# jayleicn/TVRetrieval

Hardware: AMD Instinct MI355X
Metric: queries/sec VCMR over 21.8K-video corpus (higher is better)
Workload: dtype bf16

## Files before the change

### tvretrieval_amd/csrc/convse.hip

```cpp
#include "band.h"
#include "gemm.h"

static constexpr int TM = dispatch::CONVSE_TM;
static constexpr int LP = 128 + 8;
static constexpr int LH = 4;

using dispatch::CONVSE_SUB_MAX;
using dispatch::convse_sub;

struct ConvseWs {
  int32_t* counts;
  int32_t* offsets;
  int32_t* pos;
  int32_t* chunk_off;
  int32_t* bucket;
  int32_t* chunk_vid;
};

static size_t convse_ws_layout(const xml_convse_desc* d, ConvseWs* w, char* base) {
  size_t off = 0;
  auto take = [&](size_t bytes) {
    char* p = base ? base + off : nullptr;
    off += align_up(bytes, 256);
    return p;
  };
  const size_t nv = (size_t)d->nv, P = (size_t)d->nq * d->kpairs;
  char* counts = take(nv * CONVSE_SUB_MAX * 4);
  char* offsets = take((nv * CONVSE_SUB_MAX + 1) * 4);
  char* chunk_off = take((nv + 1) * 4);
  char* bucket = take(P * 4);
  char* pos = take(P * 4);
  char* chunk_vid = take(((size_t)dispatch::convse_max_chunks((int64_t)P, (int)nv, TM) + 1) * 4);
  if (w) {
    w->chunk_vid = (int32_t*)chunk_vid;
    w->counts = (int32_t*)counts; w->pos = (int32_t*)pos; w->offsets = (int32_t*)offsets;
    w->chunk_off = (int32_t*)chunk_off; w->bucket = (int32_t*)bucket;
  }
  return off;
}

extern "C" size_t xml_convse_rerank_workspace_bytes(const xml_convse_desc* d) {
  if (!d) return 0;
  return convse_ws_layout(d, nullptr, nullptr);
}

__global__ void convse_count_kernel(const int32_t* __restrict__ pair_vid, int32_t* __restrict__ counts,
                                    int32_t* __restrict__ pos, int64_t P, int nv, int sub) {
  const int64_t p = (int64_t)blockIdx.x * blockDim.x + threadIdx.x;
  if (p >= P) return;
  const int v = pair_vid[p];
  pos[p] = (v >= 0 && v < nv) ? atomicAdd(&counts[(int64_t)v * sub + (int)(p & (sub - 1))], 1) : -1;
}

__global__ void convse_zero_skipped_kernel(const int32_t* __restrict__ pair_vid, float* __restrict__ st_out,
                                           float* __restrict__ ed_out, int64_t P, int nv, int lpad4) {
  const int64_t p = (int64_t)blockIdx.x * blockDim.x + threadIdx.x;
  if (p >= P) return;
  const int v = pair_vid[p];
  if (v >= 0 && v < nv) return;
  const float4 z = make_float4(0.f, 0.f, 0.f, 0.f);
  float4* s4 = reinterpret_cast<float4*>(st_out) + p * lpad4;
  float4* e4 = reinterpret_cast<float4*>(ed_out) + p * lpad4;
  for (int i = 0; i < lpad4; ++i) { s4[i] = z; e4[i] = z; }
}

__global__ __launch_bounds__(1024) void convse_scan_kernel(const int32_t* __restrict__ counts,
                                                           int32_t* __restrict__ offsets,
                                                           int32_t* __restrict__ chunk_off,
                                                           int32_t* __restrict__ chunk_vid, int nv, int TM, int sub) {
  __shared__ int32_t wa[16], wb[16];
  const int tid = threadIdx.x, lane = tid & 63, wave = tid >> 6;
  const int per = (nv + 1023) / 1024;
  const int r0 = min(nv, tid * per), r1 = min(nv, r0 + per);
  int sa = 0, sb = 0;
  for (int i = r0; i < r1; ++i) {
    int c = 0;
    for (int j = 0; j < sub; ++j) c += counts[(int64_t)i * sub + j];
    sa += c; sb += (c + TM - 1) / TM;
  }
  int ia = sa, ib = sb;
#pragma unroll
  for (int o = 1; o < 64; o <<= 1) {
    const int va = __shfl_up(ia, o, 64), vb = __shfl_up(ib, o, 64);
    if (lane >= o) { ia += va; ib += vb; }
  }
  if (lane == 63) { wa[wave] = ia; wb[wave] = ib; }
  __syncthreads();
  int a = ia - sa, b = ib - sb;
  for (int w = 0; w < wave; ++w) { a += wa[w]; b += wb[w]; }
  for (int i = r0; i < r1; ++i) {
    int c = 0;
    for (int j = 0; j < sub; ++j) {
      const int cj = counts[(int64_t)i * sub + j];
      offsets[(int64_t)i * sub + j] = a + c;
      c += cj;
    }
    const int ch = (c + TM - 1) / TM;
    chunk_off[i] = b;
    for (int j = 0; j < ch; ++j) chunk_vid[b + j] = i;
    a += c; b += ch;
  }
  if (tid == 1023) { offsets[(int64_t)nv * sub] = a; chunk_off[nv] = b; }
}

__global__ void convse_fill_kernel(const int32_t* __restrict__ pair_vid, const int32_t* __restrict__ offsets,
                                   const int32_t* __restrict__ pos, int32_t* __restrict__ bucket, int64_t P, int sub) {
  const int64_t p = (int64_t)blockIdx.x * blockDim.x + threadIdx.x;
  if (p >= P) return;
  const int r = pos[p];
  if (r >= 0) bucket[offsets[(int64_t)pair_vid[p] * sub + (int)(p & (sub - 1))] + r] = (int32_t)p;
}

using dispatch::CONVSE_SMALL_NV;
__global__ __launch_bounds__(1024) void convse_invert_small_kernel(const int32_t* __restrict__ pair_vid,
                                                                   int32_t* __restrict__ offsets, int32_t* __restrict__ chunk_off,
                                                                   int32_t* __restrict__ chunk_vid, int32_t* __restrict__ pos,
                                                                   int32_t* __restrict__ bucket, float* __restrict__ st_out,
                                                                   float* __restrict__ ed_out, int P, int nv, int TM, int lpad4,
                                                                   int zero_skipped) {
  __shared__ int32_t s_cnt[CONVSE_SMALL_NV], s_off[CONVSE_SMALL_NV];
  __shared__ int32_t wa[16], wb[16];
  const int tid = threadIdx.x, lane = tid & 63, wave = tid >> 6;
  for (int i = tid; i < nv; i += 1024) s_cnt[i] = 0;
  const bool in_regs = P <= 8 * 1024;
  int v_r[8], pos_r[8];
#pragma unroll
  for (int j = 0; j < 8; ++j) {
    const int p = tid + j * 1024;
    v_r[j] = (in_regs && p < P) ? pair_vid[p] : -1;
  }
  __syncthreads();
  if (in_regs) {
#pragma unroll
    for (int j = 0; j < 8; ++j) {
      const int p = tid + j * 1024;
      const bool ok = v_r[j] >= 0 && v_r[j] < nv;
      pos_r[j] = ok ? atomicAdd(&s_cnt[v_r[j]], 1) : -1;
      if (p < P && !ok && zero_skipped) {
        const float4 z = make_float4(0.f, 0.f, 0.f, 0.f);
        float4* s4 = reinterpret_cast<float4*>(st_out) + (int64_t)p * lpad4;
        float4* e4 = reinterpret_cast<float4*>(ed_out) + (int64_t)p * lpad4;
        for (int i = 0; i < lpad4; ++i) { s4[i] = z; e4[i] = z; }
      }
    }
  } else {
  for (int p = tid; p < P; p += 1024) {
    const int v = pair_vid[p];
    const bool ok = v >= 0 && v < nv;
    pos[p] = ok ? atomicAdd(&s_cnt[v], 1) : -1;
    if (!ok && zero_skipped) {
      const float4 z = make_float4(0.f, 0.f, 0.f, 0.f);
      float4* s4 = reinterpret_cast<float4*>(st_out) + (int64_t)p * lpad4;
      float4* e4 = reinterpret_cast<float4*>(ed_out) + (int64_t)p * lpad4;
      for (int i = 0; i < lpad4; ++i) { s4[i] = z; e4[i] = z; }
    }
  }
  }
  __syncthreads();
  const int per = (nv + 1023) / 1024;
  const int r0 = min(nv, tid * per), r1 = min(nv, r0 + per);
  int sa = 0, sb = 0;
  for (int i = r0; i < r1; ++i) { const int c = s_cnt[i]; sa += c; sb += (c + TM - 1) / TM; }
  int ia = sa, ib = sb;
#pragma unroll
  for (int o = 1; o < 64; o <<= 1) {
    const int va = __shfl_up(ia, o, 64), vb = __shfl_up(ib, o, 64);
    if (lane >= o) { ia += va; ib += vb; }
  }
  if (lane == 63) { wa[wave] = ia; wb[wave] = ib; }
  __syncthreads();
  int a = ia - sa, b = ib - sb;
  for (int w = 0; w < wave; ++w) { a += wa[w]; b += wb[w]; }
  for (int i = r0; i < r1; ++i) {
    const int c = s_cnt[i], ch = (c + TM - 1) / TM;
    offsets[i] = a; s_off[i] = a;
    chunk_off[i] = b;
    for (int j = 0; j < ch; ++j) chunk_vid[b + j] = i;
    a += c; b += ch;
  }
  if (tid == 1023) { offsets[nv] = a; chunk_off[nv] = b; }
  __syncthreads();
  if (in_regs) {
#pragma unroll
    for (int j = 0; j < 8; ++j)
      if (pos_r[j] >= 0) bucket[s_off[v_r[j]] + pos_r[j]] = tid + j * 1024;
    return;
  }
  for (int p = tid; p < P; p += 1024) {
    const int r = pos[p];
    if (r >= 0) bucket[s_off[pair_vid[p]] + r] = p;
  }
}

struct ConvseArgs {
  const void* q_lin[2];
  const void* feat2[2];
  const float* mask[2];
  const float* conv_w;
  float* st_out;
  float* ed_out;
  const int32_t* offsets;
  const int32_t* chunk_off;
  const int32_t* bucket;
  const int32_t* chunk_vid;
  int nv, kpairs, lpad, l_ref, hidden, n_mod, merged, ksize, softmax;
  int sub;
  int dbg;
  int dma;
  const float* q_inv[2];
  const float* c_inv[2];
  const float* pair_w;
  float* summ;
  int min_l, max_l;
  const int32_t* vid_len;
  const int32_t* pair_q;
  float* ev_sim[2];
  float* ev_merged;
};

template <typename T, bool EV = false>
__global__ __launch_bounds__(256, IsSplit16<T>::value ? 2 : 3) void convse_kernel(ConvseArgs a) {
  using Cfg = GemmCfg<T, TM, 128, 1, 4>;
  extern __shared__ __attribute__((aligned(16))) char smem[];
  __shared__ int32_t s_pair[TM];
  const int n_sim_l = a.merged ? 1 : a.n_mod;
  float (*sim)[TM][LP] = reinterpret_cast<float (*)[TM][LP]>(n_sim_l == 1 ? smem : smem + Cfg::LDS_BYTES);
  const int tid = threadIdx.x;
  const int chunk = blockIdx.x;
  if (chunk >= a.chunk_off[a.nv]) return;
  const int v = a.chunk_vid[chunk];
  const int first = a.offsets[(int64_t)v * a.sub] + (chunk - a.chunk_off[v]) * TM;
  const int cnt = min(TM, a.offsets[(int64_t)(v + 1) * a.sub] - first);
  const int vlen = a.vid_len ? max(0, min(a.vid_len[v], a.l_ref)) : a.l_ref;
  const int b_rows = a.vid_len ? max(1, min(a.lpad, vlen + (a.ksize >> 1))) : a.lpad;
  constexpr bool SPLIT = IsSplit16<T>::value;
  __shared__ float s_qinv[SPLIT ? 2 : 1][SPLIT ? TM : 1];
  auto q_of = [&](int p) -> int {
    if constexpr (EV) return a.pair_q[p];
    else return p / a.kpairs;
  };
  if (tid < TM) {
    const int p = tid < cnt ? a.bucket[first + tid] : -1;
    s_pair[tid] = p;
    if constexpr (SPLIT) {
#pragma unroll
      for (int m = 0; m < 2; ++m) s_qinv[m][tid] = (p >= 0 && m < a.n_mod) ? a.q_inv[m][q_of(p)] : 1.f;
    }
  }
  __syncthreads();

  const int lane = tid & 63, wn = tid >> 6;
  const int fr = lane & 15, fg = lane >> 4;
  const int n_sim = a.merged ? 1 : a.n_mod;
  const int mt_used = (cnt + 15) >> 4;
  f32x4 acc[Cfg::MT][Cfg::NT];
  auto ev_store = [&](float* dst, int mt, int nt, int r, float x) {
    const int row = mt * 16 + fg * 4 + r, col = wn * 32 + nt * 16 + fr;
    if (row < cnt && col < a.lpad) dst[(int64_t)s_pair[row] * a.lpad + col] = col < a.l_ref ? x : 0.f;
  };
  for (int pass = (EV && a.merged) ? -1 : 0; pass < a.n_mod; ++pass) {
    const bool pre = EV && pass < 0;
    const int m = pre ? 1 : pass;
    float cinv[Cfg::NT];
#pragma unroll
    for (int nt = 0; nt < Cfg::NT; ++nt) {
      cinv[nt] = 1.f;
      if constexpr (SPLIT) cinv[nt] = a.c_inv[m][(int64_t)v * a.lpad + min(wn * 32 + nt * 16 + fr, a.lpad - 1)];
    }
    const T* ql = reinterpret_cast<const T*>(a.q_lin[m]);
    const T* f2 = reinterpret_cast<const T*>(a.feat2[m]);
    auto a_row = [&](int r) -> const char* {
      const int p = s_pair[r];
      return p >= 0 ? reinterpret_cast<const char*>(ql + (int64_t)q_of(p) * a.hidden) : nullptr;
    };
    auto b_row = [&](int r) -> const char* {
      return r < b_rows ? reinterpret_cast<const char*>(f2 + ((int64_t)v * a.lpad + r) * a.hidden) : nullptr;
    };
    const int k_bytes = a.hidden * (int)sizeof(T);
    auto a_off = [&](int r) -> uint32_t {
      const int p = s_pair[r] >= 0 ? s_pair[r] : s_pair[0];
      return (uint32_t)q_of(p) * (uint32_t)k_bytes;
    };
    auto b_off = [&](int r) -> uint32_t { return (uint32_t)min(r, b_rows - 1) * (uint32_t)k_bytes; };
    const char* b_base = reinterpret_cast<const char*>(f2 + (int64_t)v * a.lpad * a.hidden);
    if (a.dbg == 1) {
#pragma unroll
      for (int mt = 0; mt < Cfg::MT; ++mt)
#pragma unroll
        for (int nt = 0; nt < Cfg::NT; ++nt) acc[mt][nt] = f32x4{0.f, 0.f, 0.f, 0.f};
    } else if (a.dma) {
      if (m > 0) __syncthreads();
      if (a.merged && m > 0 && !pre)
        gemm_mainloop_dma<T, Cfg, false, 2>(acc, reinterpret_cast<const char*>(ql), a_off, b_base, b_off, k_bytes, smem, mt_used);
      else
        gemm_mainloop_dma<T, Cfg, true, 2>(acc, reinterpret_cast<const char*>(ql), a_off, b_base, b_off, k_bytes, smem, mt_used);
    } else if (a.merged && m > 0 && !pre)
      gemm_mainloop<T, Cfg, false>(acc, a_row, b_row, a.hidden * (int)sizeof(T), smem, mt_used);
    else
      gemm_mainloop<T, Cfg, true>(acc, a_row, b_row, a.hidden * (int)sizeof(T), smem, mt_used);
    if constexpr (EV) {
      if (a.merged && (pre || m == 0)) {
#pragma unroll
        for (int mt = 0; mt < Cfg::MT; ++mt)
#pragma unroll
          for (int nt = 0; nt < Cfg::NT; ++nt)
#pragma unroll
            for (int r = 0; r < 4; ++r) {
              float x = acc[mt][nt][r];
              if constexpr (SPLIT) x *= s_qinv[m][mt * 16 + fg * 4 + r] * cinv[nt];
              ev_store(a.ev_sim[m], mt, nt, r, x);
            }
      }
      if (pre) {
        __syncthreads();
        continue;
      }
    }
    if constexpr (SPLIT) {
      if (a.merged && m + 1 < a.n_mod) {
        float cnext[Cfg::NT];
#pragma unroll
        for (int nt = 0; nt < Cfg::NT; ++nt)
          cnext[nt] = cinv[nt] / a.c_inv[m + 1][(int64_t)v * a.lpad + min(wn * 32 + nt * 16 + fr, a.lpad - 1)];
#pragma unroll
        for (int mt = 0; mt < Cfg::MT; ++mt)
#pragma unroll
          for (int r = 0; r < 4; ++r) {
            const int row = mt * 16 + fg * 4 + r;
            const float qr = s_qinv[m][row] / s_qinv[m + 1][row];
#pragma unroll
            for (int nt = 0; nt < Cfg::NT; ++nt) acc[mt][nt][r] *= qr * cnext[nt];
          }
      }
    }
    if (!a.merged || m == a.n_mod - 1) {
      const float scale = (a.merged && a.n_mod == 2) ? 0.5f : 1.f;
      const int si = a.merged ? 0 : m;
      if (n_sim_l == 1) __syncthreads();
#pragma unroll
      for (int mt = 0; mt < Cfg::MT; ++mt)
#pragma unroll
        for (int nt = 0; nt < Cfg::NT; ++nt)
#pragma unroll
          for (int r = 0; r < 4; ++r) {
            float x = acc[mt][nt][r] * scale;
            if constexpr (SPLIT) x *= s_qinv[m][mt * 16 + fg * 4 + r] * cinv[nt];
            sim[si][mt * 16 + fg * 4 + r][LH + wn * 32 + nt * 16 + fr] = x;
            if constexpr (EV) {
              if (a.merged) {
                ev_store(a.ev_merged, mt, nt, r, x);
              } else {
                ev_store(a.ev_sim[m], mt, nt, r, x);
                if (m == a.n_mod - 1)
                  ev_store(a.ev_merged, mt, nt, r,
                           m ? (sim[0][mt * 16 + fg * 4 + r][LH + wn * 32 + nt * 16 + fr] + x) * 0.5f : x);
              }
            }
          }
    }
  }
  __syncthreads();

  if (a.dbg == 2) return;
  const int half = a.ksize >> 1;
  const float inv_mod = 1.f / (float)n_sim;
  __shared__ float s_taps[2 * 2 * 16];
  if (tid < 2 * n_sim * a.ksize) {
    const int which = tid / (n_sim * a.ksize), rest = tid - which * n_sim * a.ksize;
    const int si = rest / a.ksize, t = rest - si * a.ksize;
    s_taps[(which * 2 + si) * 16 + t] = a.conv_w[(which * n_sim + si) * a.ksize + t];
  }
  float mk_r[2][2];
#pragma unroll
  for (int si = 0; si < 2; ++si)
#pragma unroll
    for (int h = 0; h < 2; ++h) {
      const int l = lane + h * 64;
      mk_r[si][h] = (si < n_sim && l < a.l_ref) ? a.mask[a.merged ? 0 : si][(int64_t)v * a.lpad + l] : 0.f;
    }
  __syncthreads();
  if (XML_CONVSE_FAST_EPILOGUE(a.ksize, a.summ)) {
    const int hsel = lane >> 5, l4 = (lane & 31) * 4;
    float tw[2][2][5];
#pragma unroll
    for (int w2 = 0; w2 < 2; ++w2)
#pragma unroll
      for (int si = 0; si < 2; ++si)
#pragma unroll
        for (int t = 0; t < 5; ++t) tw[w2][si][t] = si < n_sim ? s_taps[(w2 * 2 + si) * 16 + t] : 0.f;
    float mk4[2][4];
#pragma unroll
    for (int si = 0; si < 2; ++si)
#pragma unroll
      for (int c = 0; c < 4; ++c)
        mk4[si][c] = (si < n_sim && l4 + c < a.l_ref) ? a.mask[a.merged ? 0 : si][(int64_t)v * a.lpad + l4 + c] : 0.f;
    const int store_end = a.vid_len ? ((vlen + 3) & ~3) : a.lpad;
    for (int row = wn * 2 + hsel; row < ((cnt + 7) & ~7); row += 8) {
      const bool live = row < cnt;
      const int rr = live ? row : 0;
      const int p = s_pair[rr];
      float sv[4] = {0.f, 0.f, 0.f, 0.f}, ev[4] = {0.f, 0.f, 0.f, 0.f};
#pragma unroll
      for (int si = 0; si < 2; ++si) {
        if (si < n_sim) {
          float x[8];
          const float2* px = reinterpret_cast<const float2*>(&sim[si][rr][LH + l4 - 2]);
#pragma unroll
          for (int i = 0; i < 4; ++i) { const float2 t2 = px[i]; x[2 * i] = t2.x; x[2 * i + 1] = t2.y; }
#pragma unroll
          for (int i = 0; i < 8; ++i) { const int j = l4 - 2 + i; x[i] = (j >= 0 && j < a.l_ref) ? x[i] : 0.f; }
#pragma unroll
          for (int c = 0; c < 4; ++c) {
            float cs = 0.f, ce = 0.f;
#pragma unroll
            for (int t = 0; t < 5; ++t) { cs += tw[0][si][t] * x[c + t]; ce += tw[1][si][t] * x[c + t]; }
            const float fill = (1.f - mk4[si][c]) * -1e10f;
            sv[c] += cs * mk4[si][c] + fill;
            ev[c] += ce * mk4[si][c] + fill;
          }
        }
      }
#pragma unroll
      for (int c = 0; c < 4; ++c) {
        if (n_sim > 1) { sv[c] *= inv_mod; ev[c] *= inv_mod; }
        if (l4 + c >= a.l_ref) { sv[c] = -INFINITY; ev[c] = -INFINITY; }
      }
      if (a.softmax) {
        float ms = fmaxf(fmaxf(sv[0], sv[1]), fmaxf(sv[2], sv[3])), me = fmaxf(fmaxf(ev[0], ev[1]), fmaxf(ev[2], ev[3]));
        ms = lane16_max_dpp(ms); me = lane16_max_dpp(me);
        ms = fmaxf(ms, __shfl_xor(ms, 16, 64)); me = fmaxf(me, __shfl_xor(me, 16, 64));
        float ss = 0.f, se = 0.f;
#pragma unroll
        for (int c = 0; c < 4; ++c) { sv[c] = expf(sv[c] - ms); ev[c] = expf(ev[c] - me); ss += sv[c]; se += ev[c]; }
        ss = lane16_sum_dpp(ss); se = lane16_sum_dpp(se);
        ss += __shfl_xor(ss, 16, 64); se += __shfl_xor(se, 16, 64);
#pragma unroll
        for (int c = 0; c < 4; ++c) { sv[c] /= ss; ev[c] /= se; }
      }
      if (live && l4 < store_end) {
#pragma unroll
        for (int c = 0; c < 4; ++c)
          if (l4 + c >= a.l_ref) { sv[c] = 0.f; ev[c] = 0.f; }
        *reinterpret_cast<float4*>(a.st_out + (int64_t)p * a.lpad + l4) = make_float4(sv[0], sv[1], sv[2], sv[3]);
        *reinterpret_cast<float4*>(a.ed_out + (int64_t)p * a.lpad + l4) = make_float4(ev[0], ev[1], ev[2], ev[3]);
      }
    }
    return;
  }
  for (int row = wn; row < cnt; row += 4) {
    const int p = s_pair[row];
    float st[2], ed[2];
#pragma unroll
    for (int h = 0; h < 2; ++h) {
      const int l = lane + h * 64;
      float s_acc = 0.f, e_acc = 0.f;
      if (l < a.l_ref) {
#pragma unroll
        for (int si = 0; si < 2; ++si) {
          if (si < n_sim) {
            const float* wst = s_taps + si * 16;
            const float* wed = s_taps + (2 + si) * 16;
            float cs = 0.f, ce = 0.f;
            for (int t = 0; t < a.ksize; ++t) {
              const int j = l + t - half;
              const float x = (j >= 0 && j < a.l_ref) ? sim[si][row][LH + j] : 0.f;
              cs += wst[t] * x;
              ce += wed[t] * x;
            }
            const float mk = mk_r[si][h];
            const float fill = (1.f - mk) * -1e10f;
            s_acc += cs * mk + fill;
            e_acc += ce * mk + fill;
          }
        }
        if (n_sim > 1) { s_acc *= inv_mod; e_acc *= inv_mod; }
      } else {
        s_acc = -INFINITY; e_acc = -INFINITY;
      }
      st[h] = s_acc; ed[h] = e_acc;
    }
    if (a.softmax) {
      const float ms = wave_max(fmaxf(st[0], st[1])), me = wave_max(fmaxf(ed[0], ed[1]));
      float es[2], ee[2];
#pragma unroll
      for (int h = 0; h < 2; ++h) { es[h] = expf(st[h] - ms); ee[h] = expf(ed[h] - me); }
      const float ss = wave_sum(es[0] + es[1]), se = wave_sum(ee[0] + ee[1]);
#pragma unroll
      for (int h = 0; h < 2; ++h) { st[h] = es[h] / ss; ed[h] = ee[h] / se; }
    }
#pragma unroll
    for (int h = 0; h < 2; ++h) {
      const int l = lane + h * 64;
      if (a.vid_len ? l < vlen : l < a.lpad) {
        const bool in = l < a.l_ref;
        a.st_out[(int64_t)p * a.lpad + l] = in ? st[h] : 0.f;
        a.ed_out[(int64_t)p * a.lpad + l] = in ? ed[h] : 0.f;
      }
    }
    if (a.summ) {
      const float wv = a.pair_w ? a.pair_w[p] : 1.f;
      const bool in0 = lane < a.l_ref, in1 = lane + 64 < a.l_ref;
      float e_lo = in0 ? ed[0] : 0.f, e_hi = in1 ? ed[1] : 0.f;
      band_window_max(e_lo, e_hi, a.max_l - a.min_l, a.min_l, lane);
      const float m_lo = fmaxf((in0 ? st[0] : 0.f) * wv * e_lo, 0.f), m_hi = fmaxf((in1 ? st[1] : 0.f) * wv * e_hi, 0.f);
      float mg = fmaxf(m_lo, m_hi);
      mg = fmaxf(mg, __int_as_float(__builtin_amdgcn_update_dpp(0, __float_as_int(mg), 0xB1, 0xf, 0xf, false)));
      mg = fmaxf(mg, __int_as_float(__builtin_amdgcn_update_dpp(0, __float_as_int(mg), 0x4E, 0xf, 0xf, false)));
      mg = fmaxf(mg, __int_as_float(__builtin_amdgcn_update_dpp(0, __float_as_int(mg), 0x141, 0xf, 0xf, false)));
      if ((lane & 7) == 0) a.summ[(int64_t)p * XML_MOMENT_SUMM + (lane >> 3)] = mg;
    }
  }
}

struct RescoreArgs {
  const void* qn[2];
  const void* cn[2];
  const float* mask[2];
  float* out;
  const int32_t* offsets;
  const int32_t* chunk_off;
  const int32_t* bucket;
  const int32_t* chunk_vid;
  int nv, kpairs, lpad, hidden, n_mod;
  int sub;
  int dma;
};

static constexpr int RS_STAGES = 2;
template <typename T, int TM = 64>
__global__ __launch_bounds__(256, TM == 64 ? 3 : 2) void rescore_kernel(RescoreArgs a) {
  using Cfg = GemmCfg<T, TM, 128, 1, 4>;
  extern __shared__ __attribute__((aligned(16))) char smem[];
  __shared__ int32_t s_pair[TM];
  __shared__ float s_max[4][TM];
  const int tid = threadIdx.x;
  const int chunk = blockIdx.x;
  if (chunk >= a.chunk_off[a.nv]) return;
  const int v = a.chunk_vid[chunk];
  const int first = a.offsets[(int64_t)v * a.sub] + (chunk - a.chunk_off[v]) * TM;
  const int cnt = min(TM, a.offsets[(int64_t)(v + 1) * a.sub] - first);
  if (tid < TM) s_pair[tid] = tid < cnt ? a.bucket[first + tid] : -1;
  __syncthreads();
  const int lane = tid & 63, wn = tid >> 6;
  const int fr = lane & 15, fg = lane >> 4;
  float tot = 0.f;
  f32x4 acc[Cfg::MT][Cfg::NT];
  for (int m = 0; m < a.n_mod; ++m) {
    const T* qn = reinterpret_cast<const T*>(a.qn[m]);
    const T* cn = reinterpret_cast<const T*>(a.cn[m]);
    auto a_row = [&](int r) -> const char* {
      const int p = s_pair[r];
      return p >= 0 ? reinterpret_cast<const char*>(qn + (int64_t)(p / a.kpairs) * a.hidden) : nullptr;
    };
    auto b_row = [&](int r) -> const char* {
      return r < a.lpad ? reinterpret_cast<const char*>(cn + ((int64_t)v * a.lpad + r) * a.hidden) : nullptr;
    };
    float mk[Cfg::NT];
#pragma unroll
    for (int nt = 0; nt < Cfg::NT; ++nt) {
      const int c = wn * 32 + nt * 16 + fr;
      mk[nt] = c < a.lpad ? a.mask[m][(int64_t)v * a.lpad + c] : 0.f;
    }
    if (a.dma) {
      const int k_bytes = a.hidden * (int)sizeof(T);
      auto a_off = [&](int r) -> uint32_t {
        const int p = s_pair[r] >= 0 ? s_pair[r] : s_pair[0];
        return (uint32_t)(p / a.kpairs) * (uint32_t)k_bytes;
      };
      auto b_off = [&](int r) -> uint32_t { return (uint32_t)min(r, a.lpad - 1) * (uint32_t)k_bytes; };
      gemm_mainloop_dma<T, Cfg, true, RS_STAGES>(acc, reinterpret_cast<const char*>(qn), a_off,
                                                 reinterpret_cast<const char*>(cn + (int64_t)v * a.lpad * a.hidden), b_off,
                                                 k_bytes, smem, (cnt + 15) >> 4);
    } else {
      gemm_mainloop<T, Cfg, true>(acc, a_row, b_row, a.hidden * (int)sizeof(T), smem, (cnt + 15) >> 4);
    }
#pragma unroll
    for (int mt = 0; mt < Cfg::MT; ++mt)
#pragma unroll
      for (int r = 0; r < 4; ++r) {
        float best = -INFINITY;
#pragma unroll
        for (int nt = 0; nt < Cfg::NT; ++nt) {
          float x = acc[mt][nt][r];
          if constexpr (IsSplit16<T>::value) x *= 1.f / (float)(1u << (2 * XML_F16_UNIT_LOG2));
          best = fmaxf(best, x * mk[nt] + (1.f - mk[nt]) * -1e10f);
        }
        best = lane16_max_dpp(best);
        if (fr == 0) s_max[wn][mt * 16 + fg * 4 + r] = best;
      }
    __syncthreads();
    if (tid < TM) tot += fmaxf(fmaxf(s_max[0][tid], s_max[1][tid]), fmaxf(s_max[2][tid], s_max[3][tid]));
  }
  if (tid < cnt) a.out[s_pair[tid]] = a.n_mod == 2 ? tot * 0.5f : tot;
}

__global__ void rescore_fill_skipped_kernel(const int32_t* __restrict__ pair_vid, float* __restrict__ out, int64_t P,
                                            int nv) {
  const int64_t p = (int64_t)blockIdx.x * blockDim.x + threadIdx.x;
  if (p >= P) return;
  const int v = pair_vid[p];
  if (v < 0 || v >= nv) out[p] = -INFINITY;
}

__global__ void convse_zero_words_kernel(uint32_t* __restrict__ p, int64_t n) {
  const int64_t i = (int64_t)blockIdx.x * 256 + threadIdx.x;
  if (i < n) p[i] = 0u;
}

struct ConvseSumm {
  const float* pair_w;
  float* summ;
  int min_l, max_l;
  const int32_t* vid_len;
};
struct ConvseEv {
  const int32_t* pair_q;
  int64_t n_pairs;
  float* sim[2];
  float* merged;
};
static int convse_rerank_impl(const xml_convse_desc* d, const void* q_lin0, const void* q_lin1, const void* feat2_0,
                              const void* feat2_1, const float* mask0, const float* mask1, const int32_t* pair_vid,
                              const float* conv_w, float* st_out, float* ed_out, void* ws, size_t ws_bytes,
                              const float* q_inv0, const float* q_inv1, const float* c_inv0, const float* c_inv1,
                              xml_stream_t stream, ConvseSumm sm = ConvseSumm{nullptr, nullptr, 0, 0, nullptr},
                              ConvseEv ev = ConvseEv{nullptr, 0, {nullptr, nullptr}, nullptr});

extern "C" int xml_convse_rerank_ex(const xml_convse_desc* d, const void* q_lin0, const void* q_lin1, const float* q_inv0,
                                    const float* q_inv1, const void* feat2_0, const void* feat2_1, const float* c_inv0,
                                    const float* c_inv1, const float* mask0, const float* mask1, const int32_t* pair_vid,
                                    const float* conv_w, const float* pair_w, int min_l, int max_l,
                                    const int32_t* vid_len, float* st_out, float* ed_out, float* summ_out, void* ws,
                                    size_t ws_bytes, xml_stream_t stream) {
  XML_ENTER();
  if (!d || !q_lin0 || !feat2_0 || !mask0 || !pair_vid || !conv_w || !st_out || !ed_out || !ws) return XML_ERR_BAD_ARG;
  if (!summ_out && !vid_len) return XML_ERR_BAD_ARG;
  if (d->nq <= 0 || d->nv <= 0 || d->kpairs <= 0 || d->hidden <= 0) return XML_ERR_BAD_ARG;
  if (d->n_mod < 1 || d->n_mod > 2 || (d->n_mod == 2 && (!q_lin1 || !feat2_1))) return XML_ERR_BAD_ARG;
  if (d->n_mod == 2 && !d->merged && !mask1) return XML_ERR_BAD_ARG;
  if (d->merged && d->n_mod != 2) return XML_ERR_BAD_ARG;
  if (!dispatch::convse_shape_ok(d->lpad, d->l_ref, d->hidden, d->ksize, XML_F32)) return XML_ERR_UNSUPPORTED;
  if (summ_out && (min_l < 0 || max_l <= min_l)) return XML_ERR_BAD_ARG;
  if (!(d->softmax & 1)) return XML_ERR_BAD_ARG;
  if (d->dt == XML_F16S) {
    if (!q_inv0 || !c_inv0 || (d->n_mod == 2 && (!q_inv1 || !c_inv1))) return XML_ERR_BAD_ARG;
    if (!dispatch::rescore_shape_ok(d->lpad, d->hidden, XML_F16S)) return XML_ERR_UNSUPPORTED;
  } else if (d->dt != XML_F32 && d->dt != XML_BF16) {
    return XML_ERR_BAD_ARG;
  }
  return convse_rerank_impl(d, q_lin0, q_lin1, feat2_0, feat2_1, mask0, mask1, pair_vid, conv_w, st_out, ed_out, ws, ws_bytes,
                            d->dt == XML_F16S ? q_inv0 : nullptr, d->dt == XML_F16S ? q_inv1 : nullptr,
                            d->dt == XML_F16S ? c_inv0 : nullptr, d->dt == XML_F16S ? c_inv1 : nullptr, stream,
                            ConvseSumm{pair_w, summ_out, min_l, max_l, vid_len});
}

extern "C" int xml_convse_rerank(const xml_convse_desc* d, const void* q_lin0, const void* q_lin1,
                                 const void* feat2_0, const void* feat2_1, const float* mask0, const float* mask1,
                                 const int32_t* pair_vid, const float* conv_w, float* st_out, float* ed_out, void* ws,
                                 size_t ws_bytes, xml_stream_t stream) {
  XML_ENTER();
  if (!d || !q_lin0 || !feat2_0 || !mask0 || !pair_vid || !conv_w || !st_out || !ed_out || !ws) return XML_ERR_BAD_ARG;
  if (d->nq <= 0 || d->nv <= 0 || d->kpairs <= 0 || d->hidden <= 0) return XML_ERR_BAD_ARG;
  if (d->n_mod < 1 || d->n_mod > 2 || (d->n_mod == 2 && (!q_lin1 || !feat2_1))) return XML_ERR_BAD_ARG;
  if (d->n_mod == 2 && !d->merged && !mask1) return XML_ERR_BAD_ARG;
  if (d->merged && d->n_mod != 2) return XML_ERR_BAD_ARG;
  if (!dispatch::convse_shape_ok(d->lpad, d->l_ref, d->hidden, d->ksize, XML_F32)) return XML_ERR_UNSUPPORTED;
  if (d->dt != XML_F32 && d->dt != XML_BF16) return XML_ERR_BAD_ARG;
  return convse_rerank_impl(d, q_lin0, q_lin1, feat2_0, feat2_1, mask0, mask1, pair_vid, conv_w, st_out, ed_out, ws, ws_bytes,
                            nullptr, nullptr, nullptr, nullptr, stream);
}

extern "C" int xml_convse_rerank_f16s(const xml_convse_desc* d, const void* q_lin0, const void* q_lin1, const float* q_inv0,
                                      const float* q_inv1, const void* feat2_0, const void* feat2_1, const float* c_inv0,
                                      const float* c_inv1, const float* mask0, const float* mask1, const int32_t* pair_vid,
                                      const float* conv_w, float* st_out, float* ed_out, void* ws, size_t ws_bytes,
                                      xml_stream_t stream) {
  XML_ENTER();
  if (!d || !q_lin0 || !feat2_0 || !mask0 || !pair_vid || !conv_w || !st_out || !ed_out || !ws || !q_inv0 || !c_inv0)
    return XML_ERR_BAD_ARG;
  if (d->nq <= 0 || d->nv <= 0 || d->kpairs <= 0 || d->hidden <= 0) return XML_ERR_BAD_ARG;
  if (d->n_mod < 1 || d->n_mod > 2 || (d->n_mod == 2 && (!q_lin1 || !feat2_1 || !q_inv1 || !c_inv1))) return XML_ERR_BAD_ARG;
  if (d->n_mod == 2 && !d->merged && !mask1) return XML_ERR_BAD_ARG;
  if (d->merged && d->n_mod != 2) return XML_ERR_BAD_ARG;
  if (!dispatch::convse_shape_ok(d->lpad, d->l_ref, d->hidden, d->ksize, XML_F16S)) return XML_ERR_UNSUPPORTED;
  if (d->dt != XML_F16S) return XML_ERR_BAD_ARG;
  return convse_rerank_impl(d, q_lin0, q_lin1, feat2_0, feat2_1, mask0, mask1, pair_vid, conv_w, st_out, ed_out, ws, ws_bytes,
                            q_inv0, q_inv1, c_inv0, c_inv1, stream);
}

static int convse_rerank_impl(const xml_convse_desc* d, const void* q_lin0, const void* q_lin1, const void* feat2_0,
                              const void* feat2_1, const float* mask0, const float* mask1, const int32_t* pair_vid,
                              const float* conv_w, float* st_out, float* ed_out, void* ws, size_t ws_bytes,
                              const float* q_inv0, const float* q_inv1, const float* c_inv0, const float* c_inv1,
                              xml_stream_t stream, ConvseSumm sm, ConvseEv ev) {
  xml_convse_desc dl = *d;
  if (ev.pair_q) { dl.nq = (int)ev.n_pairs; dl.kpairs = 1; }
  if (!ev.pair_q && ws_bytes < xml_convse_rerank_workspace_bytes(d)) return XML_ERR_WORKSPACE;
  hipStream_t st = (hipStream_t)stream;
  ConvseWs w;
  convse_ws_layout(&dl, &w, (char*)ws);
  const int64_t P = (int64_t)dl.nq * dl.kpairs;
  int sub = 1;
  if (dispatch::convse_small_inversion(P, d->nv)) {
    hipLaunchKernelGGL(convse_invert_small_kernel, dim3(1), dim3(1024), 0, st, pair_vid, w.offsets, w.chunk_off, w.chunk_vid,
                       w.pos, w.bucket, st_out, ed_out, (int)P, d->nv, TM, d->lpad / 4, (d->softmax & 2) ? 0 : 1);
    XML_CHECK_LAUNCH();
  } else {
    {
      const int64_t nwords = (int64_t)((char*)w.offsets - (char*)w.counts) / 4;
      hipLaunchKernelGGL(convse_zero_words_kernel, dim3(cdiv(nwords, 256)), dim3(256), 0, st, (uint32_t*)w.counts, nwords);
      XML_CHECK_LAUNCH();
    }
    sub = convse_sub(P, d->nv);
    hipLaunchKernelGGL(convse_count_kernel, dim3(cdiv(P, 256)), dim3(256), 0, st, pair_vid, w.counts, w.pos, P, d->nv, sub);
    XML_CHECK_LAUNCH();
    if (!(d->softmax & 2)) {
      hipLaunchKernelGGL(convse_zero_skipped_kernel, dim3(cdiv(P, 256)), dim3(256), 0, st, pair_vid, st_out, ed_out, P,
                         d->nv, d->lpad / 4);
      XML_CHECK_LAUNCH();
    }
    hipLaunchKernelGGL(convse_scan_kernel, dim3(1), dim3(1024), 0, st, w.counts, w.offsets, w.chunk_off, w.chunk_vid,
                       d->nv, TM, sub);
    XML_CHECK_LAUNCH();
    hipLaunchKernelGGL(convse_fill_kernel, dim3(cdiv(P, 256)), dim3(256), 0, st, pair_vid, w.offsets, w.pos, w.bucket, P, sub);
    XML_CHECK_LAUNCH();
  }
  ConvseArgs a;
  a.sub = sub;
  a.q_lin[0] = q_lin0; a.q_lin[1] = q_lin1;
  a.feat2[0] = feat2_0; a.feat2[1] = feat2_1;
  a.mask[0] = mask0; a.mask[1] = mask1 ? mask1 : mask0;
  a.conv_w = conv_w; a.st_out = st_out; a.ed_out = ed_out;
  a.offsets = w.offsets; a.chunk_off = w.chunk_off; a.bucket = w.bucket; a.chunk_vid = w.chunk_vid;
  a.pair_q = ev.pair_q; a.ev_sim[0] = ev.sim[0]; a.ev_sim[1] = ev.sim[1]; a.ev_merged = ev.merged;
  a.nv = d->nv; a.kpairs = dl.kpairs; a.lpad = d->lpad; a.l_ref = d->l_ref; a.hidden = d->hidden;
  a.n_mod = d->n_mod; a.merged = d->merged; a.ksize = d->ksize; a.softmax = d->softmax & 1;
  a.dbg = g_q2c_ablation;
  a.pair_w = sm.pair_w; a.summ = sm.summ; a.min_l = sm.min_l; a.max_l = sm.max_l; a.vid_len = sm.vid_len;
  a.q_inv[0] = q_inv0; a.q_inv[1] = q_inv1 ? q_inv1 : q_inv0;
  a.c_inv[0] = c_inv0; a.c_inv[1] = c_inv1 ? c_inv1 : c_inv0;
  {
    a.dma = dispatch::convse_dma(d->nq, d->lpad, d->hidden, d->dt) ? 1 : 0;
    if (g_q2c_ablation == 40) a.dma = 0;
  }
  const int64_t max_chunks = dispatch::convse_max_chunks(P, d->nv, TM);
  const int n_sim = d->merged ? 1 : d->n_mod;
  const size_t patch = (size_t)TM * LP * 4;
  if (d->dt == XML_F16S) {
    if (!a.dma) return XML_ERR_UNSUPPORTED;
    using Cfg = GemmCfg<f16s_t, TM, 128, 1, 4>;
    constexpr size_t stg = Cfg::LDS_BYTES;
    const size_t lds = n_sim == 1 ? (stg > patch ? stg : patch) : stg + 2 * patch;
    if (ev.pair_q) {
      if (!xml_lds_attr_once<convse_kernel<f16s_t, true>>((int)(stg + 2 * patch))) return XML_ERR_LAUNCH;
      hipLaunchKernelGGL((convse_kernel<f16s_t, true>), dim3((unsigned)max_chunks), dim3(256), lds, st, a);
    } else {
      if (!xml_lds_attr_once<convse_kernel<f16s_t>>((int)(stg + 2 * patch))) return XML_ERR_LAUNCH;
      hipLaunchKernelGGL(convse_kernel<f16s_t>, dim3((unsigned)max_chunks), dim3(256), lds, st, a);
    }
  } else if (d->dt == XML_F32) {
    using Cfg = GemmCfg<float, TM, 128, 1, 4>;
    constexpr size_t stg = Cfg::LDS_BYTES;
    const size_t lds = n_sim == 1 ? (stg > patch ? stg : patch) : stg + 2 * patch;
    if (ev.pair_q) {
      if (!xml_lds_attr_once<convse_kernel<float, true>>((int)(stg + 2 * patch))) return XML_ERR_LAUNCH;
      hipLaunchKernelGGL((convse_kernel<float, true>), dim3((unsigned)max_chunks), dim3(256), lds, st, a);
    } else {
      if (!xml_lds_attr_once<convse_kernel<float>>((int)(stg + 2 * patch))) return XML_ERR_LAUNCH;
      hipLaunchKernelGGL(convse_kernel<float>, dim3((unsigned)max_chunks), dim3(256), lds, st, a);
    }
  } else {
    using Cfg = GemmCfg<bf16_t, TM, 128, 1, 4>;
    constexpr size_t stg = Cfg::LDS_BYTES;
    const size_t lds = n_sim == 1 ? (stg > patch ? stg : patch) : stg + 2 * patch;
    if (ev.pair_q) {
      if (!xml_lds_attr_once<convse_kernel<bf16_t, true>>((int)(stg + 2 * patch))) return XML_ERR_LAUNCH;
      hipLaunchKernelGGL((convse_kernel<bf16_t, true>), dim3((unsigned)max_chunks), dim3(256), lds, st, a);
    } else {
      if (!xml_lds_attr_once<convse_kernel<bf16_t>>((int)(stg + 2 * patch))) return XML_ERR_LAUNCH;
      hipLaunchKernelGGL(convse_kernel<bf16_t>, dim3((unsigned)max_chunks), dim3(256), lds, st, a);
    }
  }
  XML_CHECK_LAUNCH();
  return XML_OK;
}

__global__ void evidence_pairs_kernel(const int32_t* __restrict__ pair_q, const int32_t* __restrict__ pair_vid,
                                      int32_t* __restrict__ vid_ok, int64_t P, int nq, int nv) {
  const int64_t p = (int64_t)blockIdx.x * blockDim.x + threadIdx.x;
  if (p >= P) return;
  const int q = pair_q[p], v = pair_vid[p];
  vid_ok[p] = (q >= 0 && q < nq && v >= 0 && v < nv) ? v : -1;
}

static size_t evidence_ws_layout(const xml_convse_desc* d, int64_t n_pairs, size_t* vid_off) {
  xml_convse_desc dl = *d;
  dl.nq = (int)n_pairs; dl.kpairs = 1;
  const size_t base = convse_ws_layout(&dl, nullptr, nullptr);
  if (vid_off) *vid_off = base;
  return base + align_up((size_t)n_pairs * 4, 256);
}

extern "C" size_t xml_span_evidence_workspace_bytes(const xml_convse_desc* d, int64_t n_pairs) {
  if (!d || n_pairs <= 0 || n_pairs > INT32_MAX) return 0;
  return evidence_ws_layout(d, n_pairs, nullptr);
}

extern "C" int xml_span_evidence(const xml_convse_desc* d, const void* q_lin0, const void* q_lin1, const float* q_inv0,
                                 const float* q_inv1, const void* feat2_0, const void* feat2_1, const float* c_inv0,
                                 const float* c_inv1, const float* mask0, const float* mask1, const int32_t* pair_q,
                                 const int32_t* pair_vid, int64_t n_pairs, const float* conv_w, float* sim0_out,
                                 float* sim1_out, float* sim_out, float* st_out, float* ed_out, void* ws, size_t ws_bytes,
                                 xml_stream_t stream) {
  XML_ENTER();
  if (!d || !q_lin0 || !feat2_0 || !mask0 || !pair_q || !pair_vid || !conv_w || !sim0_out || !sim_out || !st_out ||
      !ed_out || !ws)
    return XML_ERR_BAD_ARG;
  if (d->nq <= 0 || d->nv <= 0 || n_pairs <= 0 || n_pairs > INT32_MAX || d->hidden <= 0) return XML_ERR_BAD_ARG;
  if (d->n_mod < 1 || d->n_mod > 2 || (d->n_mod == 2 && (!q_lin1 || !feat2_1 || !sim1_out))) return XML_ERR_BAD_ARG;
  if (d->n_mod == 2 && !d->merged && !mask1) return XML_ERR_BAD_ARG;
  if (d->merged && d->n_mod != 2) return XML_ERR_BAD_ARG;
  if (!dispatch::convse_shape_ok(d->lpad, d->l_ref, d->hidden, d->ksize, XML_F32)) return XML_ERR_UNSUPPORTED;
  const bool split = d->dt == XML_F16S;
  if (split) {
    if (!q_inv0 || !c_inv0 || (d->n_mod == 2 && (!q_inv1 || !c_inv1))) return XML_ERR_BAD_ARG;
    if (!dispatch::rescore_shape_ok(d->lpad, d->hidden, XML_F16S)) return XML_ERR_UNSUPPORTED;
  } else if (d->dt != XML_F32 && d->dt != XML_BF16) {
    return XML_ERR_BAD_ARG;
  }
  size_t vid_off = 0;
  if (ws_bytes < evidence_ws_layout(d, n_pairs, &vid_off)) return XML_ERR_WORKSPACE;
  hipStream_t st = (hipStream_t)stream;
  int32_t* vid_ok = (int32_t*)((char*)ws + vid_off);
  hipLaunchKernelGGL(evidence_pairs_kernel, dim3(cdiv(n_pairs, 256)), dim3(256), 0, st, pair_q, pair_vid, vid_ok, n_pairs,
                     d->nq, d->nv);
  XML_CHECK_LAUNCH();
  hipLaunchKernelGGL(convse_zero_skipped_kernel, dim3(cdiv(n_pairs, 256)), dim3(256), 0, st, vid_ok, sim0_out, sim_out,
                     n_pairs, d->nv, d->lpad / 4);
  XML_CHECK_LAUNCH();
  if (d->n_mod == 2) {
    hipLaunchKernelGGL(convse_zero_skipped_kernel, dim3(cdiv(n_pairs, 256)), dim3(256), 0, st, vid_ok, sim1_out, sim1_out,
                       n_pairs, d->nv, d->lpad / 4);
    XML_CHECK_LAUNCH();
  }
  xml_convse_desc dd = *d;
  dd.softmax = 0;
  return convse_rerank_impl(&dd, q_lin0, q_lin1, feat2_0, feat2_1, mask0, mask1, vid_ok, conv_w, st_out, ed_out, ws, ws_bytes,
                            split ? q_inv0 : nullptr, split ? q_inv1 : nullptr, split ? c_inv0 : nullptr,
                            split ? c_inv1 : nullptr, stream, ConvseSumm{nullptr, nullptr, 0, 0, nullptr},
                            ConvseEv{pair_q, n_pairs, {sim0_out, d->n_mod == 2 ? sim1_out : nullptr}, sim_out});
}

extern "C" size_t xml_q2c_rescore_workspace_bytes(int nq, int nv, int kpairs) {
  xml_convse_desc d{};
  d.nq = nq; d.nv = nv; d.kpairs = kpairs;
  return convse_ws_layout(&d, nullptr, nullptr);
}

extern "C" int xml_q2c_rescore(int n_mod, const void* qn0, const void* qn1, const void* cn0, const void* cn1,
                               const float* mask0, const float* mask1, const int32_t* pair_vid, float* out, int nq, int nv,
                               int kpairs, int lpad, int hidden, int dt, void* ws, size_t ws_bytes, xml_stream_t stream) {
  XML_ENTER();
  if (!qn0 || !cn0 || !mask0 || !pair_vid || !out || !ws) return XML_ERR_BAD_ARG;
  if (n_mod < 1 || n_mod > 2 || (n_mod == 2 && (!qn1 || !cn1 || !mask1))) return XML_ERR_BAD_ARG;
  if (nq <= 0 || nv <= 0 || kpairs <= 0 || hidden <= 0) return XML_ERR_BAD_ARG;
  if (!dispatch::rescore_shape_ok(lpad, hidden, XML_F32)) return XML_ERR_UNSUPPORTED;
  if (!dispatch::convse_dt_ok(dt)) return XML_ERR_BAD_ARG;
  if (!dispatch::rescore_shape_ok(lpad, hidden, dt)) return XML_ERR_UNSUPPORTED;
  if (dispatch::convse_mainloop(nq, lpad, hidden, dt) == XML_CONVSE_REFUSED) return XML_ERR_UNSUPPORTED;
  if (ws_bytes < xml_q2c_rescore_workspace_bytes(nq, nv, kpairs)) return XML_ERR_WORKSPACE;
  hipStream_t st = (hipStream_t)stream;
  xml_convse_desc d{};
  d.nq = nq; d.nv = nv; d.kpairs = kpairs;
  ConvseWs w;
  convse_ws_layout(&d, &w, (char*)ws);
  const int64_t P = (int64_t)nq * kpairs;
  {
    const int64_t nwords = (int64_t)((char*)w.offsets - (char*)w.counts) / 4;
    hipLaunchKernelGGL(convse_zero_words_kernel, dim3(cdiv(nwords, 256)), dim3(256), 0, st, (uint32_t*)w.counts, nwords);
    XML_CHECK_LAUNCH();
  }
  const int sub = convse_sub(P, nv);
  hipLaunchKernelGGL(convse_count_kernel, dim3(cdiv(P, 256)), dim3(256), 0, st, pair_vid, w.counts, w.pos, P, nv, sub);
  XML_CHECK_LAUNCH();
  hipLaunchKernelGGL(rescore_fill_skipped_kernel, dim3(cdiv(P, 256)), dim3(256), 0, st, pair_vid, out, P, nv);
  XML_CHECK_LAUNCH();
  const int tm = dispatch::rescore_chunk_pairs(P, nv, dt);
  const bool big = tm == dispatch::RESCORE_TM_BIG;
  hipLaunchKernelGGL(convse_scan_kernel, dim3(1), dim3(1024), 0, st, w.counts, w.offsets, w.chunk_off, w.chunk_vid, nv,
                     tm, sub);
  XML_CHECK_LAUNCH();
  hipLaunchKernelGGL(convse_fill_kernel, dim3(cdiv(P, 256)), dim3(256), 0, st, pair_vid, w.offsets, w.pos, w.bucket, P, sub);
  XML_CHECK_LAUNCH();
  RescoreArgs a;
  a.sub = sub;
  a.qn[0] = qn0; a.qn[1] = qn1; a.cn[0] = cn0; a.cn[1] = cn1;
  a.mask[0] = mask0; a.mask[1] = mask1 ? mask1 : mask0;
  a.out = out;
  a.offsets = w.offsets; a.chunk_off = w.chunk_off; a.bucket = w.bucket; a.chunk_vid = w.chunk_vid;
  a.nv = nv; a.kpairs = kpairs; a.lpad = lpad; a.hidden = hidden; a.n_mod = n_mod;
  {
    a.dma = dispatch::convse_dma(nq, lpad, hidden, dt) ? 1 : 0;
    if (g_q2c_ablation == 40) a.dma = 0;
  }
  const int64_t max_chunks = dispatch::convse_max_chunks(P, nv, tm);
  if (dt == XML_F16S && big) {
    if (!a.dma) return XML_ERR_UNSUPPORTED;
    using Cfg = GemmCfg<f16s_t, dispatch::RESCORE_TM_BIG, 128, 1, 4>;
    constexpr int lds = GemmDma<Cfg, RS_STAGES>::LDS_BYTES;
    if (!xml_lds_attr_once<rescore_kernel<f16s_t, dispatch::RESCORE_TM_BIG>>(lds)) return XML_ERR_LAUNCH;
    hipLaunchKernelGGL((rescore_kernel<f16s_t, dispatch::RESCORE_TM_BIG>), dim3((unsigned)max_chunks), dim3(256), lds, st, a);
  } else if (dt == XML_F16S) {
    if (!a.dma) return XML_ERR_UNSUPPORTED;
    using Cfg = GemmCfg<f16s_t, TM, 128, 1, 4>;
    constexpr int lds = GemmDma<Cfg, RS_STAGES>::LDS_BYTES;
    if (!xml_lds_attr_once<rescore_kernel<f16s_t>>(lds)) return XML_ERR_LAUNCH;
    hipLaunchKernelGGL(rescore_kernel<f16s_t>, dim3((unsigned)max_chunks), dim3(256), lds, st, a);
  } else if (dt == XML_F32) {
    using Cfg = GemmCfg<float, TM, 128, 1, 4>;
    constexpr int lds = GemmDma<Cfg, RS_STAGES>::LDS_BYTES;
    if (!xml_lds_attr_once<rescore_kernel<float>>(lds)) return XML_ERR_LAUNCH;
    hipLaunchKernelGGL(rescore_kernel<float>, dim3((unsigned)max_chunks), dim3(256), lds, st, a);
  } else {
    using Cfg = GemmCfg<bf16_t, TM, 128, 1, 4>;
    constexpr int lds = GemmDma<Cfg, RS_STAGES>::LDS_BYTES;
    if (!xml_lds_attr_once<rescore_kernel<bf16_t>>(lds)) return XML_ERR_LAUNCH;
    hipLaunchKernelGGL(rescore_kernel<bf16_t>, dim3((unsigned)max_chunks), dim3(256), lds, st, a);
  }
  XML_CHECK_LAUNCH();
  return XML_OK;
}
```

### tvretrieval_amd/csrc/dispatch.h

```cpp
#pragma once
#include <stddef.h>
#include <stdint.h>

#include "../../include/xmlhip.h"

namespace dispatch {

constexpr int cdiv(int64_t a, int64_t b) { return (int)((a + b - 1) / b); }
constexpr size_t dt_size(int dt) { return (dt == XML_F32 || dt == XML_F16S) ? 4 : 2; }
constexpr size_t max_of(size_t a, size_t b) { return a > b ? a : b; }

constexpr int LDS_BYTES = 160 * 1024;
constexpr int SLICE_BYTES = 64;
constexpr int RING_SLOTS = 4;
constexpr int RING_SLOTS_NOMASK = 5;
constexpr int RING_LEAD = 5;
constexpr int RING_ROWS = 256;

constexpr int GEMM_FEW_TILES = 64;
constexpr int GEMM256P_MIN_TILES = 3072;
constexpr int64_t GEMM_LN_MIN_ROWS = 2048;
constexpr int GEMM_MIN_K_BYTES = 256;
constexpr int GEMM256_MIN_M = 256, GEMM256_MIN_N = 128;
constexpr int GEMM_TILE128_MIN_WG = 512, GEMM_TILE64_MIN_WG = 192;
constexpr int GEMM_SMALL_STEP_BYTES = 128;

constexpr int64_t gemm_tiles(int64_t M, int N) { return (int64_t)cdiv(M, 256) * cdiv(N, 256); }
constexpr bool gemm_few(int64_t M, int N) { return gemm_tiles(M, N) < GEMM_FEW_TILES; }
constexpr bool gemm_ring_k(size_t k_bytes) { return k_bytes % (2 * SLICE_BYTES) == 0 && k_bytes >= GEMM_MIN_K_BYTES; }
constexpr bool gemm256_ok(int64_t M, int N, int K, int dt) {
  return M >= GEMM256_MIN_M && N >= GEMM256_MIN_N && gemm_ring_k((size_t)K * dt_size(dt));
}
constexpr bool gemm256_f16s_ok(int64_t M, int N, int K3) {
  return M >= GEMM256_MIN_M && N >= GEMM256_MIN_N && N % 8 == 0 && gemm_ring_k((size_t)K3 * 2);
}
constexpr bool gemm256p_ok(int64_t M, int N, int K, int dt) {
  return gemm_ring_k((size_t)K * dt_size(dt)) && N >= GEMM256_MIN_N && N % 8 == 0 && gemm_tiles(M, N) >= GEMM256P_MIN_TILES;
}
constexpr bool gemm_ln_fused(int64_t M, int N, int K, int dt) {
  return (dt == XML_F32 || dt == XML_BF16) && gemm_ring_k((size_t)K * dt_size(dt)) && N % 256 == 0 && N / 256 <= 3 &&
         M >= GEMM_LN_MIN_ROWS;
}
constexpr xml_gemm_kernel gemm_kernel(int64_t M, int N, int K, int dt) {
  if (dt == XML_F16S) return gemm256_f16s_ok(M, N, 3 * K) ? XML_GEMM_256 : XML_GEMM_SMALL;
  if (!gemm_few(M, N) && gemm256p_ok(M, N, K, dt)) return XML_GEMM_256P;
  if (!gemm_few(M, N) && gemm256_ok(M, N, K, dt)) return XML_GEMM_256;
  return XML_GEMM_SMALL;
}
constexpr int gemm_small_tile(int64_t M, int N) {
  const int64_t wg128 = (int64_t)cdiv(N, 128) * cdiv(M, 128);
  return wg128 >= GEMM_TILE128_MIN_WG ? 128 : wg128 * 4 >= GEMM_TILE64_MIN_WG ? 64 : 32;
}
constexpr bool gemm_small_deep(int tile, bool f16_operands) { return tile < 128 && !f16_operands; }
template <typename D3, typename D2, typename P>
constexpr void gemm_small_kloop_run(int k_bytes, D3&& deep3, D2&& deep2, P&& plain) {
  const int nsteps = (k_bytes + GEMM_SMALL_STEP_BYTES - 1) / GEMM_SMALL_STEP_BYTES;
  if (nsteps % 3 == 0) deep3();
  else if (nsteps % 2 == 0) deep2();
  else plain();
}
constexpr xml_gemm_kloop gemm_small_kloop(int k_bytes) {
  xml_gemm_kloop r = XML_KLOOP_PLAIN;
  gemm_small_kloop_run(k_bytes, [&] { r = XML_KLOOP_DEEP3; }, [&] { r = XML_KLOOP_DEEP2; }, [] {});
  return r;
}

constexpr int Q2C_PERSIST_MIN_K_BYTES = 384;
constexpr bool q2c_dt_ok(int dt) { return dt == XML_F32 || dt == XML_BF16 || dt == XML_F16; }
constexpr bool q2c_shape_ok(int lpad, int hidden) { return lpad % 16 == 0 && lpad <= 128 && hidden % 8 == 0; }
constexpr bool q2c_tiled_ok(int lpad, int hidden, int dt) {
  const size_t kb = (size_t)hidden * dt_size(dt);
  return q2c_dt_ok(dt) && lpad == 128 && kb % (2 * SLICE_BYTES) == 0 && kb >= Q2C_PERSIST_MIN_K_BYTES;
}
constexpr bool q2c_persist_ok(int lpad, int hidden, int dt) { return dt != XML_F16 && q2c_tiled_ok(lpad, hidden, dt); }
constexpr bool q2c_ring_ok(int hidden, int dt) { return dt != XML_F16 && ((size_t)hidden * dt_size(dt)) % (2 * SLICE_BYTES) == 0; }
constexpr xml_q2c_kernel q2c_kernel(int lpad, int hidden, int dt, bool combine) {
  if (!q2c_shape_ok(lpad, hidden)) return XML_Q2C_UNSUPPORTED;
  if (q2c_persist_ok(lpad, hidden, dt) && !combine) return XML_Q2C_PERSIST;
  return q2c_ring_ok(hidden, dt) ? XML_Q2C_RING : XML_Q2C_STAGED;
}
constexpr xml_q2c_kernel q2c_fused_kernel(int n_mod, int lpad, int hidden, int dt, int launch) {
  if (!q2c_shape_ok(lpad, hidden)) return launch == 0 ? XML_Q2C_UNSUPPORTED : XML_Q2C_NONE;
  if (q2c_persist_ok(lpad, hidden, dt)) return launch == 0 ? XML_Q2C_PERSIST : XML_Q2C_NONE;
  return launch < n_mod ? q2c_kernel(lpad, hidden, dt, launch > 0) : XML_Q2C_NONE;
}
constexpr int q2c_tq(int nq) { return cdiv(nq, 256); }
constexpr int q2c_tc(int nv) { return cdiv(nv, 2); }
constexpr int64_t q2c_walk_slots(int tq, int tc, int qsh) {
  const int64_t qg = (tq + (1 << qsh) - 1) >> qsh, per = 8ll << (5 - qsh);
  return (qg << qsh) * ((tc + per - 1) / per * per);
}
constexpr int q2c_qsh(int tq, int tc) {
  const int qsh = tq >= 5 ? 3 : tq >= 3 ? 2 : tq == 2 ? 1 : 0;
  return qsh == 3 && q2c_walk_slots(tq, tc, 2) * 100 < q2c_walk_slots(tq, tc, 3) * 97 ? 2 : qsh;
}
constexpr int q2c_tiles_per_workgroup(int tq, int tc) {
  const int qsh = q2c_qsh(tq, tc);
  return cdiv(tq, 1 << qsh) * cdiv(tc, 8 << (5 - qsh));
}
constexpr int q2c_ring_slots(bool tiled, int mask_mode) {
  return tiled && (mask_mode == 1 || mask_mode == 2) ? RING_SLOTS_NOMASK : RING_SLOTS;
}

constexpr int CONVSE_TM = 64;
constexpr int RESCORE_TM_BIG = 128;
constexpr int CONVSE_SUB_MAX = 16;
constexpr int CONVSE_SUB_MIN_PAIRS_PER_VIDEO = 128;
constexpr int CONVSE_SMALL_NV = 4096, CONVSE_SMALL_P = 32768;
constexpr int CONVSE_MAX_KSIZE = 15, CONVSE_FAST_KSIZE = 5, CONVSE_MAX_LPAD = 128;
constexpr int CONVSE_STEP_BYTES = GEMM_SMALL_STEP_BYTES;

constexpr bool convse_dt_ok(int dt) { return dt == XML_F32 || dt == XML_BF16 || dt == XML_F16S; }
constexpr bool rescore_shape_ok(int lpad, int hidden, int dt) {
  return lpad > 0 && lpad % 16 == 0 && lpad <= CONVSE_MAX_LPAD && hidden % 8 == 0 && (dt != XML_F16S || hidden % 32 == 0);
}
constexpr bool convse_shape_ok(int lpad, int l_ref, int hidden, int ksize, int dt) {
  return rescore_shape_ok(lpad, hidden, dt) && l_ref > 0 && l_ref <= lpad && (ksize & 1) && ksize >= 1 && ksize <= CONVSE_MAX_KSIZE;
}
constexpr bool convse_dma(int64_t nq, int lpad, int hidden, int dt) {
  const int64_t kb = (int64_t)hidden * (int64_t)dt_size(dt);
  return kb % CONVSE_STEP_BYTES == 0 && nq * kb < (1ll << 32) && (int64_t)lpad * kb < (1ll << 32);
}
constexpr xml_convse_mainloop convse_mainloop(int64_t nq, int lpad, int hidden, int dt) {
  return convse_dma(nq, lpad, hidden, dt) ? XML_CONVSE_DMA : dt == XML_F16S ? XML_CONVSE_REFUSED : XML_CONVSE_STAGED;
}
constexpr int convse_sub(int64_t P, int nv) { return P >= CONVSE_SUB_MIN_PAIRS_PER_VIDEO * (int64_t)nv ? CONVSE_SUB_MAX : 1; }
constexpr bool convse_small_inversion(int64_t P, int nv) { return P <= CONVSE_SMALL_P && nv <= CONVSE_SMALL_NV; }
constexpr xml_convse_inversion convse_inversion(int64_t P, int nv, bool rescore) {
  if (!rescore && convse_small_inversion(P, nv)) return XML_CONVSE_INV_SMALL;
  return convse_sub(P, nv) > 1 ? XML_CONVSE_INV_SUB : XML_CONVSE_INV_GLOBAL;
}
constexpr int rescore_chunk_pairs(int64_t P, int nv, int dt) {
  return dt == XML_F16S && P > CONVSE_TM * (int64_t)nv ? RESCORE_TM_BIG : CONVSE_TM;
}
constexpr int64_t convse_max_chunks(int64_t P, int nv, int tm) { return P / tm + (P < nv ? P : nv); }
#define XML_CONVSE_FAST_EPILOGUE(ksize, summ) ((ksize) == dispatch::CONVSE_FAST_KSIZE && !(summ))
constexpr bool convse_fast_epilogue(int ksize, bool summ) { return XML_CONVSE_FAST_EPILOGUE(ksize, summ); }

constexpr int L2N_MAXJ = 8, L2N_LANES = 32;
constexpr bool l2n_vec_ok(int d, int dt) {
  const int vec = 16 / (int)dt_size(dt);
  return (dt == XML_F32 || dt == XML_BF16) && d % vec == 0 && d / vec <= L2N_LANES * L2N_MAXJ;
}
constexpr bool tile_rows_l2norm_ok(int hidden, int dt) {
  return hidden > 0 && l2n_vec_ok(hidden, dt) && (hidden * (int)dt_size(dt)) % SLICE_BYTES == 0;
}

#define XML_ATTN_HEAD_SIZES(X) X(32) X(64) X(96) X(128) X(192)
#define XML_ATTN_LIST(D) D,
constexpr int ATTN_HEAD_SIZES[] = {XML_ATTN_HEAD_SIZES(XML_ATTN_LIST)};
#undef XML_ATTN_LIST
constexpr int ATTN_N_HEAD_SIZES = sizeof(ATTN_HEAD_SIZES) / sizeof(ATTN_HEAD_SIZES[0]);
constexpr int ATTN_MAX_L = 128;
constexpr int ATTN_SMALL_MAX_L = 32;
constexpr int ATTN_SMALL_UNITS = 4;
constexpr bool attn_head_size_ok(int dh) {
  for (int i = 0; i < ATTN_N_HEAD_SIZES; ++i)
    if (ATTN_HEAD_SIZES[i] == dh) return true;
  return false;
}
constexpr size_t attn_small_lds_bytes(int lk, int dh, int dt) {
  const int es = (int)dt_size(dt), ce = 64 / es;
  const int lkp = (lk + ce - 1) / ce * ce;
  const size_t k_stride = (size_t)dh * es + 16, vt_stride = (size_t)lkp * es + 16;
  const size_t kvb = es == 2 ? (size_t)32 * k_stride : max_of((size_t)32 * k_stride, (size_t)dh * vt_stride);
  return ATTN_SMALL_UNITS * (kvb + 16 * vt_stride);
}
constexpr size_t attn_lds_bytes(int lk, int dh, int dt) {
  const int es = (int)dt_size(dt), ce = 64 / es;
  const int lkp = (lk + ce - 1) / ce * ce;
  const size_t k_stride = (size_t)dh * es + 16, vt_stride = (size_t)lkp * es + 16;
  const size_t kvb = es == 2 ? (size_t)lkp * k_stride
                             : max_of((size_t)((lk + 15) / 16 * 16) * k_stride, (size_t)dh * vt_stride);
  return kvb + 4 * 16 * vt_stride;
}
constexpr xml_attn_kernel attn_kernel(int lq, int lk, int hidden, int n_heads, int dt) {
  if (n_heads <= 0 || hidden % n_heads) return XML_ATTN_REFUSED_HEADS;
  const int dh = hidden / n_heads;
  if (lq > ATTN_MAX_L || lk > ATTN_MAX_L) return XML_ATTN_REFUSED_LENGTH;
  if (attn_lds_bytes(lk, dh, dt) > (size_t)LDS_BYTES) return XML_ATTN_REFUSED_LDS;
  if (!attn_head_size_ok(dh)) return XML_ATTN_REFUSED_DH;
  const bool small = lq <= ATTN_SMALL_MAX_L && lk <= ATTN_SMALL_MAX_L && attn_small_lds_bytes(lk, dh, dt) <= (size_t)LDS_BYTES;
  return small ? XML_ATTN_SMALL : XML_ATTN_LARGE;
}
constexpr bool attn_train_ok(int lq, int lk, int hidden, int n_heads, int dt) {
  return dt == XML_BF16 && n_heads > 0 && hidden % n_heads == 0 && lq > 0 && lk > 0 && lq <= ATTN_MAX_L && lk <= ATTN_MAX_L &&
         attn_head_size_ok(hidden / n_heads);
}

}
```

### tvretrieval_amd/csrc/gemm256.hip

```cpp
#include <type_traits>

#include "internal.h"
#include "ring256.h"

__device__ __forceinline__ void g256_dma4(uint32_t va0, uint32_t va1, uint32_t vb0, uint32_t vb1, const char* sa,
                                          const char* sb, uint32_t lds_dst) {
  asm volatile(
      "s_mov_b32 m0, %4\n\ts_nop 0\n\tglobal_load_lds_dwordx4 %0, %5\n\t"
      "s_add_u32 m0, m0, 0x400\n\ts_nop 0\n\tglobal_load_lds_dwordx4 %1, %5\n\t"
      "s_add_u32 m0, m0, 0x3c00\n\ts_nop 0\n\tglobal_load_lds_dwordx4 %2, %6\n\t"
      "s_add_u32 m0, m0, 0x400\n\ts_nop 0\n\tglobal_load_lds_dwordx4 %3, %6"
      :
      : "v"(va0), "v"(va1), "v"(vb0), "v"(vb1), "s"(lds_dst), "s"(sa), "s"(sb)
      : "memory", "scc");
}
template <typename T, typename OutT, typename AddT, bool RAGGED_N = false>
__global__ __launch_bounds__(512, 2) void gemm256_kernel(const T* __restrict__ A, const T* __restrict__ W,
                                                         const float* __restrict__ bias,
                                                         const AddT* __restrict__ addend, OutT* __restrict__ out,
                                                         int64_t M, int N, int K, int relu, int add_mode, int seq_len,
                                                         int tm, int tn, const float* __restrict__ row_scale) {
  constexpr bool SCALED = std::is_same<T, f16_t>::value;
  using namespace ring256;
  constexpr int NSLOT = dispatch::RING_SLOTS;
  static_assert((NSLOT & (NSLOT - 1)) == 0, "slots are addressed by masking the slice number");
  extern __shared__ __attribute__((aligned(16))) char smem[];

  const int b = blockIdx.x;
  const int xcd = b & 7, local = b >> 3;
  const int sup = (local >> 5) * 8 + xcd;
  const int w32 = local & 31;
  const int sm = (tm + 7) >> 3;
  const int mt_ = (sup % sm) * 8 + (w32 & 7);
  const int nt_ = (sup / sm) * 4 + (w32 >> 3);
  if (mt_ >= tm || nt_ >= tn) return;

  const int tid = threadIdx.x, lane = tid & 63;
  const int wave = __builtin_amdgcn_readfirstlane(tid >> 6);
  const int wm = wave >> 1, wn = wave & 1;
  const int fr = lane & 15, fg = lane >> 4;
  const int64_t m0 = (int64_t)mt_ * 256;
  const int n0 = nt_ * 256;
  const int k_bytes = K * (int)sizeof(T);
  const int n_slices = k_bytes / ROWB;

  uint32_t voff_a[2], voff_b[2];
  {
    const int rsub = lane >> 2, pslot = lane & 3;
#pragma unroll
    for (int i = 0; i < 2; ++i) {
      const int row = (wave * 2 + i) * 16 + rsub;
      const int slot = pslot ^ ring_swz(row);
      voff_a[i] = (uint32_t)((m0 + row < M) ? row : 0) * k_bytes + slot * 16;
      voff_b[i] = (uint32_t)((n0 + row < N) ? row : 0) * k_bytes + slot * 16;
    }
  }
  const char* sbase_a = reinterpret_cast<const char*>(A) + m0 * k_bytes;
  const char* sbase_b = reinterpret_cast<const char*>(W) + (int64_t)n0 * k_bytes;
  const uint32_t lds_wave = (uint32_t)(uintptr_t)(__attribute__((address_space(3))) char*)smem + wave * 2048;
  int i_slice = 0;
  auto issue_slice = [&]() {
    const int koff = i_slice * ROWB;
    const uint32_t dst = lds_wave + (i_slice & (NSLOT - 1)) * SLOT_BYTES;
    g256_dma4(voff_a[0], voff_a[1], voff_b[0], voff_b[1], sbase_a + koff, sbase_b + koff, dst);
    ++i_slice;
  };

  const int a_off = (wm * 64 + fr) * ROWB + ((fg ^ ring_swz(fr)) << 4);
  constexpr bool DIRECT = !RAGGED_N;
  constexpr bool PAIRED = DIRECT && sizeof(OutT) == 2;
  const int rb_e = PAIRED ? (fr >> 2) * 8 + (fr & 3) : fr;
  const int b_off = OPER_BYTES + (wn * 128 + rb_e) * ROWB + ((fg ^ ring_swz(rb_e)) << 4);
  const int b_off_o = OPER_BYTES + (wn * 128 + rb_e + 4) * ROWB + ((fg ^ ring_swz(rb_e + 4)) << 4);
  auto b_frag = [&](const char* slot, int n) -> uint4 {
    if constexpr (PAIRED) return *reinterpret_cast<const uint4*>(slot + ((n & 1) ? b_off_o : b_off) + (n >> 1) * 32 * ROWB);
    else return *reinterpret_cast<const uint4*>(slot + b_off + n * 16 * ROWB);
  };

  issue_slice(); issue_slice(); issue_slice(); issue_slice();
  asm volatile("s_waitcnt vmcnt(12)" ::: "memory");
  __builtin_amdgcn_s_barrier();

  f32x4 acc[4][8];
  uint4 faA[4], faB[4], fbL[4], fbH[4];
#pragma unroll
  for (int m = 0; m < 4; ++m) faA[m] = *reinterpret_cast<const uint4*>(smem + a_off + m * 16 * ROWB);
#pragma unroll
  for (int n = 0; n < 4; ++n) fbL[n] = b_frag(smem, n);

  int c_slice = 0;
  auto run = [&](auto grp_tag) {
    constexpr bool GRP1 = decltype(grp_tag)::value;
    auto slice_step = [&](uint4 (&fc)[4], uint4 (&fn)[4], auto mode_tag, auto init_tag) {
      constexpr int MODE = decltype(mode_tag)::value;
      constexpr bool INIT = decltype(init_tag)::value;
      const char* slot = smem + (c_slice & (NSLOT - 1)) * SLOT_BYTES;
#pragma unroll
      for (int n = 0; n < 4; ++n) fbH[n] = b_frag(slot, n + 4);
#pragma unroll
      for (int m = 0; m < 4; ++m)
#pragma unroll
        for (int n = 0; n < 4; ++n) {
          if constexpr (DIRECT) {
            if constexpr (INIT) RingInit<T>::chunk(acc[m][n], fbL[n], fc[m]);
            else Mma<T>::chunk(acc[m][n], fbL[n], fc[m]);
          } else {
            if constexpr (INIT) RingInit<T>::chunk(acc[m][n], fc[m], fbL[n]);
            else Mma<T>::chunk(acc[m][n], fc[m], fbL[n]);
          }
        }
      if constexpr (MODE <= 1) __builtin_amdgcn_s_waitcnt(0x0078);
      else if constexpr (MODE == 2) __builtin_amdgcn_s_waitcnt(0x0074);
      else if constexpr (MODE == 3) __builtin_amdgcn_s_waitcnt(0x0070);
      if constexpr (MODE <= 3) __builtin_amdgcn_s_barrier();
      ++c_slice;
      auto preamble = [&]() {
        if constexpr (MODE <= 3) {
          const char* nslot = smem + (c_slice & (NSLOT - 1)) * SLOT_BYTES;
#pragma unroll
          for (int m = 0; m < 4; ++m) fn[m] = *reinterpret_cast<const uint4*>(nslot + a_off + m * 16 * ROWB);
#pragma unroll
          for (int n = 0; n < 4; ++n) fbL[n] = b_frag(nslot, n);
        }
        if constexpr (MODE == 0) issue_slice();
      };
      if (!GRP1) preamble();
      __builtin_amdgcn_sched_barrier(0);
#pragma unroll
      for (int m = 0; m < 4; ++m)
#pragma unroll
        for (int n = 0; n < 4; ++n) {
          if constexpr (DIRECT) {
            if constexpr (INIT) RingInit<T>::chunk(acc[m][n + 4], fbH[n], fc[m]);
            else Mma<T>::chunk(acc[m][n + 4], fbH[n], fc[m]);
          } else {
            if constexpr (INIT) RingInit<T>::chunk(acc[m][n + 4], fc[m], fbH[n]);
            else Mma<T>::chunk(acc[m][n + 4], fc[m], fbH[n]);
          }
        }
      __builtin_amdgcn_sched_barrier(0);
      if (GRP1) preamble();
    };
    using M0 = std::integral_constant<int, 0>;
    using M1 = std::integral_constant<int, 1>;
    using M2 = std::integral_constant<int, 2>;
    using M3 = std::integral_constant<int, 3>;
    using M4 = std::integral_constant<int, 4>;
    const int n_main = n_slices - 4;
    if (n_main > 0) {
      slice_step(faA, faB, M0{}, std::true_type{});
      slice_step(faB, faA, M0{}, std::false_type{});
      for (int s2 = 2; s2 < n_main; s2 += 2) {
        slice_step(faA, faB, M0{}, std::false_type{});
        slice_step(faB, faA, M0{}, std::false_type{});
      }
      slice_step(faA, faB, M1{}, std::false_type{});
    } else {
      slice_step(faA, faB, M1{}, std::true_type{});
    }
    slice_step(faB, faA, M2{}, std::false_type{});
    slice_step(faA, faB, M3{}, std::false_type{});
    slice_step(faB, faA, M4{}, std::false_type{});
  };
  if (wave >> 2) run(std::true_type{});
  else run(std::false_type{});

  if constexpr (DIRECT) {
    constexpr int GC = PAIRED ? 8 : 4;
    constexpr int NGRP = 128 / (4 * GC);
    static_assert(GC * sizeof(AddT) <= 16, "addend group wider than one 16-byte load");
    int gcol[NGRP], pcol[NGRP / 2];
    bool gok[NGRP];
    float gb[NGRP][GC];
#pragma unroll
    for (int q = 0; q < NGRP; ++q) {
      gcol[q] = n0 + wn * 128 + q * (4 * GC) + fg * GC;
      gok[q] = gcol[q] + GC <= N;
#pragma unroll
      for (int e = 0; e < GC; e += 4) {
        float4 b4 = make_float4(0.f, 0.f, 0.f, 0.f);
        if (bias && gok[q]) b4 = *reinterpret_cast<const float4*>(bias + gcol[q] + e);
        gb[q][e] = b4.x; gb[q][e + 1] = b4.y; gb[q][e + 2] = b4.z; gb[q][e + 3] = b4.w;
      }
    }
#pragma unroll
    for (int pq = 0; pq < NGRP / 2; ++pq) pcol[pq] = n0 + wn * 128 + pq * (8 * GC) + (fr & 1) * (4 * GC) + fg * GC;
    const uint32_t m0_mod = add_mode == 1 ? (uint32_t)(m0 % seq_len) : 0u;
    const bool odd = (fr & 1) != 0;
#pragma unroll
    for (int m4 = 0; m4 < 4; ++m4) {
      const int lrow = wm * 64 + m4 * 16 + fr;
      const int64_t m = m0 + lrow;
      const bool rok = m < M;
      float rsc = 1.f;
      if constexpr (SCALED) rsc = rok ? row_scale[m] : 0.f;
      float v[NGRP][GC];
#pragma unroll
      for (int q = 0; q < NGRP; ++q)
#pragma unroll
        for (int e = 0; e < GC; ++e) {
          float x = (PAIRED ? acc[m4][2 * q + (e >> 2)][e & 3] : acc[m4][q][e & 3]);
          if constexpr (SCALED) x *= rsc;
          x += gb[q][e];
          if (relu) x = fmaxf(x, 0.f);
          v[q][e] = x;
        }
      if (add_mode) {
        const int64_t arow = add_mode == 1 ? (int64_t)((m0_mod + (uint32_t)lrow) % (uint32_t)seq_len) : m;
        constexpr int AB = GC * (int)sizeof(AddT);
#pragma unroll
        for (int qb = 0; qb < NGRP; qb += 4) {
          uint4 ad[4];
#pragma unroll
          for (int qi = 0; qi < 4; ++qi) {
            const int q = qb + qi;
            ad[qi] = make_uint4(0u, 0u, 0u, 0u);
            if (rok && gok[q]) {
              if constexpr (AB == 16) ad[qi] = ld_global16(addend + arow * N + gcol[q]);
              else { const uint2 u = *reinterpret_cast<const uint2*>(addend + arow * N + gcol[q]); ad[qi].x = u.x; ad[qi].y = u.y; }
            }
          }
#pragma unroll
          for (int qi = 0; qi < 4; ++qi) {
            float av[8];
            if constexpr (sizeof(AddT) == 2) unpack16<bf16_t>(ad[qi], av);
            else unpack16<float>(ad[qi], av);
#pragma unroll
            for (int e = 0; e < GC; ++e) v[qb + qi][e] += av[e];
          }
        }
      }
      uint4 pk[NGRP];
#pragma unroll
      for (int q = 0; q < NGRP; ++q) pk[q] = pack16<OutT>(v[q]);
      const int64_t m_even = m0 + wm * 64 + m4 * 16 + (fr & ~1);
#pragma unroll
      for (int pq = 0; pq < NGRP / 2; ++pq) {
        const uint4 own_e = pk[2 * pq], own_o = pk[2 * pq + 1];
        const uint4 dn = ring_dpp_u4<0x111>(own_o);
        const uint4 up = ring_dpp_u4<0x101>(own_e);
        const uint4 d_even = make_uint4(odd ? dn.x : own_e.x, odd ? dn.y : own_e.y, odd ? dn.z : own_e.z, odd ? dn.w : own_e.w);
        const uint4 d_odd = make_uint4(odd ? own_o.x : up.x, odd ? own_o.y : up.y, odd ? own_o.z : up.z, odd ? own_o.w : up.w);
        if (pcol[pq] + GC <= N) {
          if (m_even < M) st_global16(out + m_even * N + pcol[pq], d_even);
          if (m_even + 1 < M) st_global16(out + (m_even + 1) * N + pcol[pq], d_odd);
        }
      }
    }
    return;
  }
  __syncthreads();
  constexpr int PLD = 132;
  float* patch = reinterpret_cast<float*>(smem) + wave * (32 * PLD);
  constexpr bool F32O = sizeof(OutT) == 4;
  const int orow = lane >> 4;
  const int oc0 = (lane & 15) * (F32O ? 4 : 8);
  const int oc1 = F32O ? oc0 + 64 : oc0 + 4;
  const int nc0 = n0 + wn * 128 + oc0, nc1 = n0 + wn * 128 + oc1;
  const bool ok0 = nc0 + 4 <= N, ok1 = nc1 + 4 <= N;
  float bv[8];
#pragma unroll
  for (int j = 0; j < 4; ++j) {
    bv[j] = (bias && nc0 + j < N) ? bias[nc0 + j] : 0.f;
    bv[4 + j] = (bias && nc1 + j < N) ? bias[nc1 + j] : 0.f;
  }
#pragma unroll
  for (int j = 0; j < 8; ++j) asm volatile("" : "+v"(bv[j]));
  const uint32_t m0_mod = add_mode == 1 ? (uint32_t)(m0 % seq_len) : 0u;
#pragma unroll
  for (int half = 0; half < 2; ++half) {
#pragma unroll
    for (int mt = 0; mt < 2; ++mt)
#pragma unroll
      for (int nt = 0; nt < 8; ++nt)
#pragma unroll
        for (int r = 0; r < 4; ++r) patch[(mt * 16 + fg * 4 + r) * PLD + nt * 16 + fr] = acc[half * 2 + mt][nt][r];
    __builtin_amdgcn_wave_barrier();
#pragma unroll
    for (int it = 0; it < 8; ++it) {
      const int prow = it * 4 + orow;
      const int lrow = wm * 64 + half * 32 + prow;
      const int64_t m = m0 + lrow;
      const float4 v0 = *reinterpret_cast<const float4*>(patch + prow * PLD + oc0);
      const float4 v1 = *reinterpret_cast<const float4*>(patch + prow * PLD + oc1);
      float v[8] = {v0.x, v0.y, v0.z, v0.w, v1.x, v1.y, v1.z, v1.w};
      if (m >= M) continue;
      if constexpr (SCALED) {
        const float rsc = row_scale[m];
#pragma unroll
        for (int j = 0; j < 8; ++j) v[j] *= rsc;
      }
#pragma unroll
      for (int j = 0; j < 8; ++j) {
        v[j] += bv[j];
        if (relu) v[j] = fmaxf(v[j], 0.f);
      }
      const int64_t arow = add_mode == 1 ? (int64_t)((m0_mod + (uint32_t)lrow) % (uint32_t)seq_len) : m;
      if (!RAGGED_N) {
        if (add_mode) {
          float av[8] = {0.f, 0.f, 0.f, 0.f, 0.f, 0.f, 0.f, 0.f};
          if (sizeof(AddT) == 2) {
            uint2 u0 = make_uint2(0u, 0u), u1 = u0;
            if (ok0) u0 = *reinterpret_cast<const uint2*>(addend + arow * N + nc0);
            if (ok1) u1 = *reinterpret_cast<const uint2*>(addend + arow * N + nc1);
            av[0] = __uint_as_float(u0.x << 16); av[1] = __uint_as_float(u0.x & 0xffff0000u);
            av[2] = __uint_as_float(u0.y << 16); av[3] = __uint_as_float(u0.y & 0xffff0000u);
            av[4] = __uint_as_float(u1.x << 16); av[5] = __uint_as_float(u1.x & 0xffff0000u);
            av[6] = __uint_as_float(u1.y << 16); av[7] = __uint_as_float(u1.y & 0xffff0000u);
          } else {
            if (ok0) unpack16<float>(ld_global16(addend + arow * N + nc0), av);
            if (ok1) unpack16<float>(ld_global16(addend + arow * N + nc1), av + 4);
          }
#pragma unroll
          for (int j = 0; j < 8; ++j) v[j] += av[j];
        }
        if (F32O) {
          if (ok0) st_global16(out + m * N + nc0, pack16<float>(v));
          if (ok1) st_global16(out + m * N + nc1, pack16<float>(v + 4));
        } else if (ok1) {
          st_global16(out + m * N + nc0, pack16<bf16_t>(v));
        }
      } else {
#pragma unroll
        for (int j = 0; j < 8; ++j) {
          const int n = (j < 4 ? nc0 : nc1 - 4) + j;
          if (n >= N) continue;
          float x = v[j];
          if (add_mode) x += DT<AddT>::ld(addend + arow * N + n);
          DT<OutT>::st(out + m * N + n, x);
        }
      }
    }
    __builtin_amdgcn_wave_barrier();
  }
}

template <typename T, typename OutT, typename AddT>
static int launch_gemm256(const void* A, const void* W, const float* bias, const void* addend, void* out, int64_t M,
                          int N, int K, int relu, int add_mode, int seq_len, hipStream_t st,
                          const float* row_scale = nullptr) {
  const int tm = cdiv(M, 256), tn = cdiv(N, 256);
  const int64_t nsup = (int64_t)((tm + 7) / 8) * ((tn + 3) / 4);
  const unsigned grid = (unsigned)(((nsup + 7) / 8) * 8 * 32);
  const int lds = 8 * 32 * 132 * 4;
  auto kern = (N & 7) ? gemm256_kernel<T, OutT, AddT, true> : gemm256_kernel<T, OutT, AddT, false>;
  if (!((N & 7) ? xml_lds_attr_once<gemm256_kernel<T, OutT, AddT, true>>(lds)
                : xml_lds_attr_once<gemm256_kernel<T, OutT, AddT, false>>(lds)))
    return XML_ERR_LAUNCH;
  hipLaunchKernelGGL(kern, dim3(grid), dim3(512), lds, st, (const T*)A, (const T*)W, bias, (const AddT*)addend,
                     (OutT*)out, M, N, K, relu, add_mode, seq_len, tm, tn, row_scale);
  XML_CHECK_LAUNCH();
  return XML_OK;
}

int xmli_gemm256_f16s(const void* A, const void* W, const float* bias, const void* addend, void* out,
                      const float* row_scale, int64_t M, int N, int K3, int relu, int add_mode, int seq_len,
                      hipStream_t st) {
  return launch_gemm256<f16_t, float, float>(A, W, bias, addend, out, M, N, K3, relu, add_mode, seq_len, st, row_scale);
}

int xmli_gemm256(const void* A, const void* W, const float* bias, const void* addend, void* out, int64_t M, int N,
                 int K, int relu, int add_mode, int seq_len, int out_f32, int dt, hipStream_t st) {
  if (dt == XML_F32)
    return launch_gemm256<float, float, float>(A, W, bias, addend, out, M, N, K, relu, add_mode, seq_len, st);
  if (out_f32)
    return launch_gemm256<bf16_t, float, bf16_t>(A, W, bias, addend, out, M, N, K, relu, add_mode, seq_len, st);
  return launch_gemm256<bf16_t, bf16_t, bf16_t>(A, W, bias, addend, out, M, N, K, relu, add_mode, seq_len, st);
}
```

### tvretrieval_amd/csrc/gemm256p.hip

```cpp
#include <type_traits>

#include "internal.h"
#include "ring256.h"

struct G256pArgs {
  const void* A;
  const void* W;
  const float* bias;
  const void* addend;
  void* out;
  int64_t M, n_tiles;
  int N, K, relu, add_mode, seq_len, tn;
  float* ln_scratch;
  const float* ln_g;
  const float* ln_b;
  float ln_eps;
  int probe;
};

#ifdef XML_DEBUG_VARIANTS
__device__ unsigned long long g_g256p_probe[8 * 8];
__device__ unsigned int g_g256p_steps[8 * 64];
extern "C" int xml_debug_read_gemm_steps(unsigned int* host_out) {
  return hipMemcpyFromSymbol(host_out, HIP_SYMBOL(g_g256p_steps), sizeof(unsigned int) * 512) == hipSuccess ? 0 : -4;
}
extern "C" int xml_debug_read_gemm_probe(unsigned long long* host_out) {
  return hipMemcpyFromSymbol(host_out, HIP_SYMBOL(g_g256p_probe), sizeof(unsigned long long) * 64) == hipSuccess ? 0 : -4;
}
#define G256P_T() ((a.probe & 1) ? __builtin_amdgcn_s_memtime() : 0ull)
#else
#define G256P_T() 0ull
#endif
template <typename T, typename OutT, typename AddT, bool LNE = false, bool DIRECT = true>
__global__ __launch_bounds__(512) void gemm256p_kernel(G256pArgs a) {
  static_assert(!LNE || DIRECT, "the LayerNorm epilogue works on the DIRECT accumulator layout");
  using namespace ring256;
  constexpr int NSLOT = dispatch::RING_SLOTS;
  constexpr int RING_BYTES = NSLOT * SLOT_BYTES;
  extern __shared__ __attribute__((aligned(16))) char smem[];

  const int tid = threadIdx.x, lane = tid & 63;
  const int wave = __builtin_amdgcn_readfirstlane(tid >> 6);
  const int wm = wave >> 1, wn = wave & 1;
  const int grp = wave >> 2;
  const int fr = lane & 15, fg = lane >> 4;
  const int xcd = blockIdx.x & 7, loc = blockIdx.x >> 3;
  const int k_bytes = a.K * (int)sizeof(T);
  const int n_slices = k_bytes / ROWB;
  const T* A = reinterpret_cast<const T*>(a.A);
  const T* W = reinterpret_cast<const T*>(a.W);
  const AddT* addend = reinterpret_cast<const AddT*>(a.addend);
  OutT* out = reinterpret_cast<OutT*>(a.out);
  const int64_t M = a.M;
  const int N = a.N;

  const int tn_s = __builtin_amdgcn_readfirstlane(a.tn);
  const int64_t n_rb = a.n_tiles / tn_s;
  auto lne_split = [&](int k, int& r, int& nt) {
    r = tn_s == 1 ? k : tn_s == 2 ? (k >> 1) : (int)(((uint32_t)k * 43691u) >> 17);
    nt = k - r * tn_s;
  };
  auto tile_of = [&](int k) -> int64_t {
    if constexpr (LNE) {
      int r, nt;
      lne_split(k, r, nt);
      const int64_t rb = ((int64_t)r * 8 + xcd) * 32 + loc;
      return rb < n_rb ? rb * tn_s + nt : a.n_tiles;
    }
    return ((int64_t)k * 8 + xcd) * 32 + loc;
  };
  auto tile_mt_nt = [&](int k, int64_t& mt, int& nt) {
    if constexpr (LNE) {
      int r;
      lne_split(k, r, nt);
      mt = ((int64_t)r * 8 + xcd) * 32 + loc;
    } else {
      const int64_t lin = tile_of(k);
      mt = lin / a.tn;
      nt = (int)(lin - mt * a.tn);
    }
  };

  const uint32_t lds0 = (uint32_t)(uintptr_t)(__attribute__((address_space(3))) char*)smem;
  int i_k = 0, i_slice = 0, i_slot = 0, i_left = n_slices, i_inc = 1;
  uint32_t va[4] = {}, vb[2] = {};
  const char* sbase_a = nullptr;
  const char* sbase_b = nullptr;
  auto setup_issue_tile = [&]() {
    int64_t mt; int nt;
    tile_mt_nt(i_k, mt, nt);
    const int64_t m0 = mt * 256;
    const int n0 = nt * 256;
    const int lane_o = ring_lane_now();
    const int rsub = lane_o >> 2, pslot = lane_o & 3;
    auto off_a = [&](int piece) -> uint32_t {
      const int row = piece * 16 + rsub;
      return (uint32_t)((m0 + row < M) ? row : 0) * k_bytes + (pslot ^ ring_swz(row)) * 16;
    };
    auto off_b = [&](int piece) -> uint32_t {
      const int row = piece * 16 + rsub;
      return (uint32_t)((n0 + row < N) ? row : 0) * k_bytes + (pslot ^ ring_swz(row)) * 16;
    };
    if (grp == 0) {
      va[0] = off_a(wave * 4); va[1] = off_a(wave * 4 + 1); va[2] = off_a(wave * 4 + 2); va[3] = off_a(wave * 4 + 3);
      vb[0] = off_b(wave * 2); vb[1] = off_b(wave * 2 + 1);
    } else {
      vb[0] = off_b(8 + (wave - 4) * 2); vb[1] = off_b(9 + (wave - 4) * 2);
    }
    sbase_a = reinterpret_cast<const char*>(A) + ((a.probe & 2) ? (int64_t)(blockIdx.x & 31) * 256 : m0) * k_bytes;
    sbase_b = reinterpret_cast<const char*>(W) + (int64_t)n0 * k_bytes;
  };
  auto issue_slice = [&]() {
    const int koff = i_slice * ROWB;
    const uint32_t slot0 = lds0 + i_slot * SLOT_BYTES;
    if (grp == 0) {
      ring_dma_quad(va[0], va[1], va[2], va[3], sbase_a + koff, slot0 + wave * 4096);
      ring_dma_pair(vb[0], vb[1], sbase_b + koff, slot0 + OPER_BYTES + wave * 2048);
    } else {
      ring_dma_pair(vb[0], vb[1], sbase_b + koff, slot0 + OPER_BYTES + 8192 + (wave - 4) * 2048);
    }
    if (++i_slot == NSLOT) i_slot = 0;
    i_slice += i_inc;
    if (--i_left == 0) {
      i_slice = 0;
      i_left = n_slices;
      ++i_k;
      if (tile_of(i_k) < a.n_tiles) setup_issue_tile();
      else { i_left = 0x7fffffff; i_inc = 0; }
    }
  };
  if (tile_of(0) >= a.n_tiles) return;
  setup_issue_tile();

  const int a_off = (wm * 64 + fr) * ROWB + ((fg ^ ring_swz(fr)) << 4);
  constexpr bool PAIRED = DIRECT && sizeof(OutT) == 2;
  const int rb_e = PAIRED ? (fr >> 2) * 8 + (fr & 3) : fr;
  const int b_off = OPER_BYTES + (wn * 128 + rb_e) * ROWB + ((fg ^ ring_swz(rb_e)) << 4);
  const int b_off_o = OPER_BYTES + (wn * 128 + rb_e + 4) * ROWB + ((fg ^ ring_swz(rb_e + 4)) << 4);
  auto b_frag = [&](const char* slot, int n) -> uint4 {
    if constexpr (PAIRED) return *reinterpret_cast<const uint4*>(slot + ((n & 1) ? b_off_o : b_off) + (n >> 1) * 32 * ROWB);
    else return *reinterpret_cast<const uint4*>(slot + b_off + n * 16 * ROWB);
  };
  int c_k = 0, c_slot = 0;
  issue_slice(); issue_slice(); issue_slice(); issue_slice();
  if (grp == 0) asm volatile("s_waitcnt vmcnt(18)" ::: "memory");
  else asm volatile("s_waitcnt vmcnt(6)" ::: "memory");
  __builtin_amdgcn_s_barrier();

  uint4 faA[4], faB[4], fbL[4], fbH[4];

  auto run = [&](auto grp_tag) {
  constexpr bool GRP1 = decltype(grp_tag)::value;
  unsigned long long pr[8] = {};
  const unsigned long long pr_t0 = G256P_T();
  const unsigned long long pr_r0 = (a.probe & 1) ? __builtin_amdgcn_s_memrealtime() : 0ull;
#ifdef XML_DEBUG_VARIANTS
  unsigned int* sp = reinterpret_cast<unsigned int*>(smem + RING_BYTES + wave * 4096 + 2048);
  if ((a.probe & 1) && lane < 64) sp[lane] = 0;
  int pstep = 0;
  unsigned long long pst = 0;
#endif
  for (;;) {
    unsigned long long pt = G256P_T();
#ifdef XML_DEBUG_VARIANTS
    pstep = 0; pst = pt;
#endif
    f32x4 acc[4][8];
    {
      const char* slot0 = smem + c_slot * SLOT_BYTES;
#pragma unroll
      for (int m = 0; m < 4; ++m) faA[m] = *reinterpret_cast<const uint4*>(slot0 + a_off + m * 16 * ROWB);
#pragma unroll
      for (int n = 0; n < 4; ++n) fbL[n] = b_frag(slot0, n);
    }
    auto slice_step = [&](uint4 (&fc)[4], uint4 (&fn)[4], auto init_tag) {
      constexpr bool INIT = decltype(init_tag)::value;
      const char* slot = smem + c_slot * SLOT_BYTES;
#pragma unroll
      for (int n = 0; n < 4; ++n) fbH[n] = b_frag(slot, n + 4);
#pragma unroll
      for (int m = 0; m < 4; ++m)
#pragma unroll
        for (int n = 0; n < 4; ++n) {
          if constexpr (DIRECT) {
            if constexpr (INIT) RingInit<T>::chunk(acc[m][n], fbL[n], fc[m]);
            else Mma<T>::chunk(acc[m][n], fbL[n], fc[m]);
          } else {
            if constexpr (INIT) RingInit<T>::chunk(acc[m][n], fc[m], fbL[n]);
            else Mma<T>::chunk(acc[m][n], fc[m], fbL[n]);
          }
        }
      if (!GRP1) __builtin_amdgcn_s_waitcnt(0x007c);
      else __builtin_amdgcn_s_waitcnt(0x0074);
      __builtin_amdgcn_s_barrier();
      if (++c_slot == NSLOT) c_slot = 0;
      auto next_reads = [&]() {
        const char* nslot = smem + c_slot * SLOT_BYTES;
#pragma unroll
        for (int m = 0; m < 4; ++m) fn[m] = *reinterpret_cast<const uint4*>(nslot + a_off + m * 16 * ROWB);
#pragma unroll
        for (int n = 0; n < 4; ++n) fbL[n] = b_frag(nslot, n);
      };
      if (!GRP1) { next_reads(); issue_slice(); }
      __builtin_amdgcn_sched_barrier(0);
#pragma unroll
      for (int m = 0; m < 4; ++m)
#pragma unroll
        for (int n = 0; n < 4; ++n) {
          if constexpr (DIRECT) {
            if constexpr (INIT) RingInit<T>::chunk(acc[m][n + 4], fbH[n], fc[m]);
            else Mma<T>::chunk(acc[m][n + 4], fbH[n], fc[m]);
          } else {
            if constexpr (INIT) RingInit<T>::chunk(acc[m][n + 4], fc[m], fbH[n]);
            else Mma<T>::chunk(acc[m][n + 4], fc[m], fbH[n]);
          }
        }
      __builtin_amdgcn_sched_barrier(0);
      if (GRP1) { next_reads(); issue_slice(); }
#ifdef XML_DEBUG_VARIANTS
      if (a.probe & 1) {
        const unsigned long long t = __builtin_amdgcn_s_memtime();
        if (lane == 0 && pstep < 64) sp[pstep] += (unsigned int)(t - pst);
        pst = t; ++pstep;
      }
#endif
    };
    slice_step(faA, faB, std::true_type{});
    slice_step(faB, faA, std::false_type{});
    for (int s2 = 2; s2 < n_slices; s2 += 2) {
      slice_step(faA, faB, std::false_type{});
      slice_step(faB, faA, std::false_type{});
    }

    { const unsigned long long t = G256P_T(); pr[0] += t - pt; pt = t; }
    {
      int64_t mt; int nt;
      tile_mt_nt(c_k, mt, nt);
      const int64_t m0 = mt * 256;
      const int n0 = nt * 256;
      const uint32_t m0_mod = a.add_mode == 1 ? (uint32_t)(m0 % a.seq_len) : 0u;
      const int lane_e = ring_lane_now();
      const int fr_e = lane_e & 15, fg_e = lane_e >> 4;
      const int tid_e = wave * 64 + lane_e;
      float* patch = reinterpret_cast<float*>(smem + RING_BYTES) + wave * 1024;
      constexpr bool F32O = sizeof(OutT) == 4;
      const int orow = lane_e >> 4;
      const int oc0 = (lane_e & 15) * (F32O ? 4 : 8);
      const int oc1 = F32O ? oc0 + 64 : oc0 + 4;
      const int nc0 = n0 + wn * 128 + oc0, nc1 = n0 + wn * 128 + oc1;
      const bool ok0 = nc0 + 4 <= N, ok1 = nc1 + 4 <= N;
      constexpr int GC = PAIRED ? 8 : 4;
      constexpr int NGRP = 128 / (4 * GC);
      static_assert(GC * sizeof(AddT) <= 16, "addend group wider than one 16-byte load");
      int gcol[DIRECT ? NGRP : 1];
      bool gok[DIRECT ? NGRP : 1];
      int pcol[DIRECT ? NGRP / 2 : 1];
      auto store_rows = [&](int m4, auto& v, int dcol = 0) {
        uint4 pk[NGRP];
#pragma unroll
        for (int q = 0; q < NGRP; ++q) pk[q] = pack16<OutT>(v[q]);
        const bool odd = (fr_e & 1) != 0;
        const int64_t m_even = m0 + wm * 64 + m4 * 16 + (fr_e & ~1);
#pragma unroll
        for (int pq = 0; pq < NGRP / 2; ++pq) {
          const uint4 dn = ring_dpp_u4<0x111>(pk[2 * pq + 1]);
          const uint4 up = ring_dpp_u4<0x101>(pk[2 * pq]);
          const uint4 own_e = pk[2 * pq], own_o = pk[2 * pq + 1];
          const uint4 d_even = make_uint4(odd ? dn.x : own_e.x, odd ? dn.y : own_e.y, odd ? dn.z : own_e.z, odd ? dn.w : own_e.w);
          const uint4 d_odd = make_uint4(odd ? own_o.x : up.x, odd ? own_o.y : up.y, odd ? own_o.z : up.z, odd ? own_o.w : up.w);
          const int col = pcol[pq] + dcol;
          if (col + GC <= N) {
            if (!(a.probe & 8)) {
              typedef unsigned int g_u4 __attribute__((ext_vector_type(4)));
              if (m_even < M && !(a.probe & 4)) __builtin_nontemporal_store(g_u4{d_even.x, d_even.y, d_even.z, d_even.w}, reinterpret_cast<g_u4*>(out + m_even * N + col));
              if (m_even + 1 < M && !(a.probe & 4)) __builtin_nontemporal_store(g_u4{d_odd.x, d_odd.y, d_odd.z, d_odd.w}, reinterpret_cast<g_u4*>(out + (m_even + 1) * N + col));
            } else {
              if (m_even < M && !(a.probe & 4)) st_global16(out + m_even * N + col, d_even);
              if (m_even + 1 < M && !(a.probe & 4)) st_global16(out + (m_even + 1) * N + col, d_odd);
            }
          }
        }
      };
      if constexpr (DIRECT) {
#pragma unroll
        for (int q = 0; q < NGRP; ++q) {
          gcol[q] = n0 + wn * 128 + q * (4 * GC) + fg_e * GC;
          gok[q] = gcol[q] + GC <= N;
        }
#pragma unroll
        for (int pq = 0; pq < NGRP / 2; ++pq) pcol[pq] = n0 + wn * 128 + pq * (8 * GC) + (fr_e & 1) * (4 * GC) + fg_e * GC;
        {
          float4 b4 = make_float4(0.f, 0.f, 0.f, 0.f);
          const int bc = n0 + wn * 128 + (lane_e & 31) * 4;
          if (a.bias && bc + 4 <= N) b4 = *reinterpret_cast<const float4*>(a.bias + bc);
          if (lane_e < 32) *reinterpret_cast<float4*>(patch + 256 + lane_e * 4) = b4;
          __builtin_amdgcn_s_waitcnt(0xc07f);
          __builtin_amdgcn_wave_barrier();
        }
        { const unsigned long long t = G256P_T(); pr[1] += t - pt; pt = t; }
#pragma unroll
        for (int m4 = 0; m4 < 4; ++m4) {
          const int lrow = wm * 64 + m4 * 16 + fr_e;
          const int64_t m = m0 + lrow;
          const bool rok = m < M;
          float v[NGRP][GC];
          int boff = fg_e * GC;
          asm volatile("" : "+v"(boff));
#pragma unroll
          for (int q = 0; q < NGRP; ++q) {
            float gb[GC];
#pragma unroll
            for (int e = 0; e < GC; e += 4) {
              const float4 b4 = *reinterpret_cast<const float4*>(patch + 256 + q * (4 * GC) + boff + e);
              gb[e] = b4.x; gb[e + 1] = b4.y; gb[e + 2] = b4.z; gb[e + 3] = b4.w;
            }
#pragma unroll
            for (int e = 0; e < GC; ++e) {
              float x = (PAIRED ? acc[m4][2 * q + (e >> 2)][e & 3] : acc[m4][q][e & 3]) + gb[e];
              if (a.relu) x = fmaxf(x, 0.f);
              v[q][e] = x;
            }
          }
          if (a.add_mode) {
            const int64_t arow = a.add_mode == 1 ? (int64_t)((m0_mod + (uint32_t)lrow) % (uint32_t)a.seq_len) : m;
            constexpr int AB = GC * (int)sizeof(AddT);
#pragma unroll
            for (int qb = 0; qb < NGRP; qb += 4) {
              uint4 ad[4];
#pragma unroll
              for (int qi = 0; qi < 4; ++qi) {
                const int q = qb + qi;
                ad[qi] = make_uint4(0u, 0u, 0u, 0u);
                if (rok && gok[q]) {
                  if constexpr (AB == 16) ad[qi] = ld_global16(addend + arow * N + gcol[q]);
                  else { const uint2 u = *reinterpret_cast<const uint2*>(addend + arow * N + gcol[q]); ad[qi].x = u.x; ad[qi].y = u.y; }
                }
              }
#pragma unroll
              for (int qi = 0; qi < 4; ++qi) {
                float av[8];
                if constexpr (sizeof(AddT) == 2) unpack16<bf16_t>(ad[qi], av);
                else unpack16<float>(ad[qi], av);
#pragma unroll
                for (int e = 0; e < GC; ++e) v[qb + qi][e] += av[e];
              }
            }
          }
          if constexpr (LNE) {
            float s = 0.f;
#pragma unroll
            for (int q = 0; q < NGRP; ++q)
#pragma unroll
              for (int e = 0; e < GC; ++e) s += v[q][e];
            s += __shfl_xor(s, 16, 64);
            s += __shfl_xor(s, 32, 64);
            const float seg_mean = s * (1.0f / 128.0f);
            float c2 = 0.f;
#pragma unroll
            for (int q = 0; q < NGRP; ++q)
#pragma unroll
              for (int e = 0; e < GC; ++e) { const float c = v[q][e] - seg_mean; c2 += c * c; }
            c2 += __shfl_xor(c2, 16, 64);
            c2 += __shfl_xor(c2, 32, 64);
            if (fg_e == 0) {
              float* ps = patch + 640 + ((m4 * 16 + fr_e) * tn_s + nt) * 2;
              ps[0] = s;
              ps[1] = c2;
            }
          }
          if constexpr (LNE) {
            if (nt == tn_s - 1) {
#pragma unroll
              for (int q = 0; q < NGRP; ++q)
#pragma unroll
                for (int e = 0; e < GC; ++e) {
                  if constexpr (PAIRED) acc[m4][2 * q + (e >> 2)][e & 3] = v[q][e];
                  else acc[m4][q][e & 3] = v[q][e];
                }
            } else {
              float4* sc = reinterpret_cast<float4*>(a.ln_scratch) + (int64_t)blockIdx.x * (tn_s - 1) * 16384 +
                           (int64_t)((nt * 4 + m4) * 8) * 512 + tid_e;
#pragma unroll
              for (int j = 0; j < 8; ++j) {
                const float* vf = &v[0][0] + j * 4;
                typedef float xml_nt4 __attribute__((ext_vector_type(4)));
                __builtin_nontemporal_store(xml_nt4{vf[0], vf[1], vf[2], vf[3]}, reinterpret_cast<xml_nt4*>(sc + j * 512));
              }
            }
          } else {
            store_rows(m4, v);
          }
        }
      } else {
      float bv[8];
      {
        float4 b0 = make_float4(0.f, 0.f, 0.f, 0.f), b1 = b0;
        if (a.bias && ok0) b0 = *reinterpret_cast<const float4*>(a.bias + nc0);
        if (a.bias && ok1) b1 = *reinterpret_cast<const float4*>(a.bias + nc1);
        bv[0] = b0.x; bv[1] = b0.y; bv[2] = b0.z; bv[3] = b0.w; bv[4] = b1.x; bv[5] = b1.y; bv[6] = b1.z; bv[7] = b1.w;
      }
#pragma unroll
      for (int j = 0; j < 8; ++j) asm volatile("" : "+v"(bv[j]));
#pragma unroll
      for (int p = 0; p < 8; ++p) {
        if ((fg_e >> 1) == (p & 1)) {
          const int prow0 = (fg_e & 1) * 4;
#pragma unroll
          for (int n = 0; n < 8; ++n)
#pragma unroll
            for (int r = 0; r < 4; ++r)
              patch[(prow0 + r) * 128 + ((n * 16 + fr_e) ^ ((fg_e & 1) << 4))] = acc[p >> 1][n][r];
        }
        __builtin_amdgcn_s_waitcnt(0xc07f);
        __builtin_amdgcn_wave_barrier();
#pragma unroll
        for (int it = 0; it < 2; ++it) {
          const int prow = it * 4 + orow;
          const int lrow = wm * 64 + p * 8 + prow;
          const int64_t m = m0 + lrow;
          const float4 v0 = *reinterpret_cast<const float4*>(patch + prow * 128 + (oc0 ^ (it << 4)));
          const float4 v1 = *reinterpret_cast<const float4*>(patch + prow * 128 + (oc1 ^ (it << 4)));
          float v[8] = {v0.x, v0.y, v0.z, v0.w, v1.x, v1.y, v1.z, v1.w};
          if (m >= M) continue;
#pragma unroll
          for (int j = 0; j < 8; ++j) {
            v[j] += bv[j];
            if (a.relu) v[j] = fmaxf(v[j], 0.f);
          }
          if (a.add_mode) {
            const int64_t arow = a.add_mode == 1 ? (int64_t)((m0_mod + (uint32_t)lrow) % (uint32_t)a.seq_len) : m;
            float av[8] = {0.f, 0.f, 0.f, 0.f, 0.f, 0.f, 0.f, 0.f};
            if (sizeof(AddT) == 2) {
              uint2 u0 = make_uint2(0u, 0u), u1 = u0;
              if (ok0) u0 = *reinterpret_cast<const uint2*>(addend + arow * N + nc0);
              if (ok1) u1 = *reinterpret_cast<const uint2*>(addend + arow * N + nc1);
              av[0] = __uint_as_float(u0.x << 16); av[1] = __uint_as_float(u0.x & 0xffff0000u);
              av[2] = __uint_as_float(u0.y << 16); av[3] = __uint_as_float(u0.y & 0xffff0000u);
              av[4] = __uint_as_float(u1.x << 16); av[5] = __uint_as_float(u1.x & 0xffff0000u);
              av[6] = __uint_as_float(u1.y << 16); av[7] = __uint_as_float(u1.y & 0xffff0000u);
            } else {
              if (ok0) unpack16<float>(ld_global16(addend + arow * N + nc0), av);
              if (ok1) unpack16<float>(ld_global16(addend + arow * N + nc1), av + 4);
            }
#pragma unroll
            for (int j = 0; j < 8; ++j) v[j] += av[j];
          }
          if (F32O) {
            if (ok0) st_global16(out + m * N + nc0, pack16<float>(v));
            if (ok1) st_global16(out + m * N + nc1, pack16<float>(v + 4));
          } else if (ok1) {
            st_global16(out + m * N + nc0, pack16<bf16_t>(v));
          }
        }
        __builtin_amdgcn_s_waitcnt(0xc07f);
        __builtin_amdgcn_wave_barrier();
      }
      }
      { const unsigned long long t = G256P_T(); pr[2] += t - pt; pt = t; }
      if constexpr (LNE) {
        if (nt == tn_s - 1) {
          __builtin_amdgcn_s_waitcnt(0xc07f);
          __builtin_amdgcn_s_barrier();
          {
            const float* p0 = reinterpret_cast<const float*>(smem + RING_BYTES) + (wm * 2) * 1024 + 640 + lane_e * tn_s * 2;
            const float* p1 = p0 + 1024;
            typedef float xml_f4 __attribute__((ext_vector_type(4)));
            xml_f4 pv[3];
#pragma unroll
            for (int t = 0; t < 3; ++t)
              pv[t] = t < tn_s ? xml_f4{p0[t * 2], p0[t * 2 + 1], p1[t * 2], p1[t * 2 + 1]} : xml_f4{0.f, 0.f, 0.f, 0.f};
            float tot = 0.f;
#pragma unroll
            for (int t = 0; t < 3; ++t) tot += pv[t].x + pv[t].z;
            tot += 0.f + 0.f;
            const float mean = tot / (float)N;
            float m2 = 0.f;
#pragma unroll
            for (int t = 0; t < 3; ++t) {
              if (t < tn_s) {
                const float d0 = pv[t].x * (1.0f / 128.0f) - mean, d1 = pv[t].z * (1.0f / 128.0f) - mean;
                m2 += pv[t].y + 128.0f * d0 * d0 + pv[t].w + 128.0f * d1 * d1;
              }
            }
            const float rstd = 1.0f / sqrtf(m2 / (float)N + a.ln_eps);
            patch[lane_e * 2] = mean;
            patch[lane_e * 2 + 1] = rstd;
          }
          { const unsigned long long t = G256P_T(); pr[3] += t - pt; pt = t; }
          for (int t = tn_s - 1; t >= 0; --t) {
            __builtin_amdgcn_wave_barrier();
            {
              const int bc = t * 256 + wn * 128 + (lane_e & 31) * 4;
              const float4 g4 = *reinterpret_cast<const float4*>(a.ln_g + bc);
              const float4 b4 = *reinterpret_cast<const float4*>(a.ln_b + bc);
              if (lane_e < 32) {
                *reinterpret_cast<float4*>(patch + 384 + lane_e * 4) = g4;
                *reinterpret_cast<float4*>(patch + 512 + lane_e * 4) = b4;
              }
            }
            __builtin_amdgcn_s_waitcnt(0xc07f);
            __builtin_amdgcn_wave_barrier();
            const float4* sc = reinterpret_cast<const float4*>(a.ln_scratch) + (int64_t)blockIdx.x * (tn_s - 1) * 16384 +
                               (int64_t)(t * 32) * 512 + tid_e;
#pragma unroll
            for (int m4 = 0; m4 < 4; ++m4) {
              const int lr64 = m4 * 16 + fr_e;
              const float mean = patch[lr64 * 2], rstd = patch[lr64 * 2 + 1];
              int boff = fg_e * GC;
              asm volatile("" : "+v"(boff));
              float x[NGRP * GC];
              if (t == tn_s - 1) {
#pragma unroll
                for (int q = 0; q < NGRP; ++q)
#pragma unroll
                  for (int e = 0; e < GC; ++e)
                    x[q * GC + e] = PAIRED ? acc[m4][2 * q + (e >> 2)][e & 3] : acc[m4][q][e & 3];
              } else {
#pragma unroll
                for (int j = 0; j < 8; ++j) {
                  typedef float xml_nt4 __attribute__((ext_vector_type(4)));
                  const xml_nt4 f = __builtin_nontemporal_load(reinterpret_cast<const xml_nt4*>(sc + (m4 * 8 + j) * 512));
                  x[j * 4] = f.x; x[j * 4 + 1] = f.y; x[j * 4 + 2] = f.z; x[j * 4 + 3] = f.w;
                }
              }
              float v[NGRP][GC];
#pragma unroll
              for (int q = 0; q < NGRP; ++q)
#pragma unroll
                for (int e = 0; e < GC; e += 4) {
                  const float4 g4 = *reinterpret_cast<const float4*>(patch + 384 + q * (4 * GC) + boff + e);
                  const float4 b4 = *reinterpret_cast<const float4*>(patch + 512 + q * (4 * GC) + boff + e);
                  const float gq[4] = {g4.x, g4.y, g4.z, g4.w}, bq[4] = {b4.x, b4.y, b4.z, b4.w};
#pragma unroll
                  for (int j = 0; j < 4; ++j) v[q][e + j] = (x[q * GC + e + j] - mean) * rstd * gq[j] + bq[j];
                }
              store_rows(m4, v, (t - nt) * 256);
            }
          }
          __builtin_amdgcn_s_waitcnt(0xc07f);
          __builtin_amdgcn_wave_barrier();
        }
      }
    }
    { const unsigned long long t = G256P_T(); pr[4] += t - pt; pt = t; }
    ++pr[6];
    ++c_k;
    if (tile_of(c_k) >= a.n_tiles) break;
  }
#ifdef XML_DEBUG_VARIANTS
  if ((a.probe & 1) && blockIdx.x == 0 && lane == 0) {
    pr[5] = __builtin_amdgcn_s_memtime() - pr_t0;
    pr[7] = __builtin_amdgcn_s_memrealtime() - pr_r0;
    for (int i = 0; i < 8; ++i) g_g256p_probe[wave * 8 + i] = pr[i];
    for (int i = 0; i < 64; ++i) g_g256p_steps[wave * 64 + i] = sp[i];
  }
#endif
  };
  if (grp) run(std::true_type{});
  else run(std::false_type{});
  asm volatile("s_waitcnt vmcnt(0)" ::: "memory");
  __builtin_amdgcn_s_barrier();
}

template <typename T, typename OutT, typename AddT, bool LNE = false, bool DIRECT = true>
static int launch_gemm256p(const void* A, const void* W, const float* bias, const void* addend, void* out, int64_t M,
                           int N, int K, int relu, int add_mode, int seq_len, hipStream_t st, const float* ln_g = nullptr,
                           const float* ln_b = nullptr, void* ln_ws = nullptr) {
  G256pArgs a;
  a.A = A; a.W = W; a.bias = bias; a.addend = addend; a.out = out;
  a.M = M; a.N = N; a.K = K; a.relu = relu; a.add_mode = add_mode; a.seq_len = seq_len;
  a.tn = cdiv(N, 256);
  a.n_tiles = (int64_t)cdiv(M, 256) * a.tn;
  a.ln_scratch = (float*)ln_ws; a.ln_g = ln_g; a.ln_b = ln_b; a.ln_eps = 1e-5f;
  a.probe = g_q2c_ablation == 9 ? 1 : g_q2c_ablation == 21 ? 2 : g_q2c_ablation == 22 ? 4 : g_q2c_ablation == 23 ? 6 : g_q2c_ablation == 24 ? 8 : 0;
  const int lds = dispatch::RING_SLOTS * ring256::SLOT_BYTES + 8 * 4096;
#ifdef XML_DEBUG_VARIANTS
  if (!LNE && DIRECT && g_gemm_variant == 3)
    return launch_gemm256p<T, OutT, AddT, false, false>(A, W, bias, addend, out, M, N, K, relu, add_mode, seq_len, st);
#endif
  auto kern = gemm256p_kernel<T, OutT, AddT, LNE, DIRECT>;
  if (!xml_lds_attr_once<gemm256p_kernel<T, OutT, AddT, LNE, DIRECT>>(lds)) return XML_ERR_LAUNCH;
  hipLaunchKernelGGL(kern, dim3(256), dim3(512), lds, st, a);
  XML_CHECK_LAUNCH();
  return XML_OK;
}

size_t xmli_gemm_ln_workspace_bytes(int64_t M, int N) {
  (void)M;
  return align_up((size_t)256 * (size_t)(N / 256 > 1 ? N / 256 - 1 : 0) * 256 * 256 * 4 + 256, 256);
}
int xmli_gemm_ln(const void* A, const void* W, const float* bias, const void* addend, const float* ln_g, const float* ln_b,
                 void* y, int64_t M, int N, int K, int relu, int add_mode, int seq_len, int dt, void* ln_ws,
                 hipStream_t st) {
  if (!ln_ws) return XML_ERR_WORKSPACE;
  if (dt == XML_F32)
    return launch_gemm256p<float, float, float, true>(A, W, bias, addend, y, M, N, K, relu, add_mode, seq_len, st, ln_g,
                                                      ln_b, ln_ws);
  return launch_gemm256p<bf16_t, bf16_t, bf16_t, true>(A, W, bias, addend, y, M, N, K, relu, add_mode, seq_len, st, ln_g,
                                                        ln_b, ln_ws);
}

template <typename OutT, int TN>
__global__ __launch_bounds__(64) void ln_lne_order_kernel(const float* __restrict__ pre, const float* __restrict__ ln_g,
                                                           const float* __restrict__ ln_b, OutT* __restrict__ y,
                                                           int64_t rows, int N, float ln_eps) {
#pragma clang fp contract(off)
  constexpr int GC = sizeof(OutT) == 2 ? 8 : 4;
  constexpr int NGRP = 128 / (4 * GC);
  constexpr int LPR = TN == 1 ? 8 : TN == 2 ? 16 : 32;
  const int lane = threadIdx.x & 63;
  const int sub = lane & (LPR - 1);
  const int base = lane - sub;
  const int64_t row = ((int64_t)blockIdx.x * 64 + threadIdx.x) / LPR;
  if (row >= rows || sub >= 8 * TN) return;
  const int seg = sub >> 2, fg = sub & 3;
  const int c0 = (seg >> 1) * 256 + (seg & 1) * 128 + fg * GC;
  const float* pr = pre + row * N;
  float v[NGRP][GC], gv[NGRP][GC], bv[NGRP][GC];
#pragma unroll
  for (int q = 0; q < NGRP; ++q)
#pragma unroll
    for (int e = 0; e < GC; e += 4) {
      const float4 f = *reinterpret_cast<const float4*>(pr + c0 + q * (4 * GC) + e);
      const float4 g4 = *reinterpret_cast<const float4*>(ln_g + c0 + q * (4 * GC) + e);
      const float4 b4 = *reinterpret_cast<const float4*>(ln_b + c0 + q * (4 * GC) + e);
      v[q][e] = f.x; v[q][e + 1] = f.y; v[q][e + 2] = f.z; v[q][e + 3] = f.w;
      gv[q][e] = g4.x; gv[q][e + 1] = g4.y; gv[q][e + 2] = g4.z; gv[q][e + 3] = g4.w;
      bv[q][e] = b4.x; bv[q][e + 1] = b4.y; bv[q][e + 2] = b4.z; bv[q][e + 3] = b4.w;
    }
#pragma unroll
  for (int q = 0; q < NGRP; ++q)
#pragma unroll
    for (int e = 0; e < GC; ++e) asm volatile("" : "+v"(v[q][e]), "+v"(gv[q][e]), "+v"(bv[q][e]));
  float s = 0.f;
#pragma unroll
  for (int q = 0; q < NGRP; ++q)
#pragma unroll
    for (int e = 0; e < GC; ++e) s += v[q][e];
  s += __shfl_xor(s, 1, 64);
  s += __shfl_xor(s, 2, 64);
  const float* vf = &v[0][0];
  const float cs0 = __builtin_fmaf(s, -1.0f / 128.0f, vf[0]), cs1 = __builtin_fmaf(s, -1.0f / 128.0f, vf[1]);
  float c2 = __builtin_fmaf(cs0, cs0, cs1 * cs1);
#pragma unroll
  for (int k = 2; k < NGRP * GC; ++k) {
    const float c = __builtin_fmaf(s, -1.0f / 128.0f, vf[k]);
    c2 = __builtin_fmaf(c, c, c2);
  }
  c2 += __shfl_xor(c2, 1, 64);
  c2 += __shfl_xor(c2, 2, 64);
  typedef float xml_f4 __attribute__((ext_vector_type(4)));
  xml_f4 pv[3];
#pragma unroll
  for (int t = 0; t < 3; ++t)
    pv[t] = t < TN ? xml_f4{__shfl(s, base + t * 8, 64), __shfl(c2, base + t * 8, 64), __shfl(s, base + t * 8 + 4, 64),
                            __shfl(c2, base + t * 8 + 4, 64)}
                   : xml_f4{0.f, 0.f, 0.f, 0.f};
  float tot = 0.f;
#pragma unroll
  for (int t = 0; t < 3; ++t) tot += pv[t].x + pv[t].z;
  const float mean = tot / (float)N;
  float m2 = 0.f;
#pragma unroll
  for (int t = 0; t < TN; ++t) {
    const float d0 = __builtin_fmaf(pv[t].x, 1.0f / 128.0f, -mean), d1 = __builtin_fmaf(pv[t].z, 1.0f / 128.0f, -mean);
    float u = __builtin_fmaf(d0, 128.0f * d0, pv[t].y);
    u = pv[t].w + u;
    u = __builtin_fmaf(d1, 128.0f * d1, u);
    m2 = u + m2;
  }
  const float rstd = 1.0f / sqrtf(m2 / (float)N + ln_eps);
#pragma unroll
  for (int q = 0; q < NGRP; ++q) {
    float o[GC];
#pragma unroll
    for (int e = 0; e < GC; ++e) o[e] = __builtin_fmaf((v[q][e] - mean) * rstd, gv[q][e], bv[q][e]);
    st_global16(y + row * N + c0 + q * (4 * GC), pack16<OutT>(o));
  }
}

int xmli_gemm_ln_tail(const float* pre, const float* ln_g, const float* ln_b, void* y, int64_t M, int N, int dt,
                      hipStream_t st) {
  const int tn = N / 256;
  if ((dt != XML_F32 && dt != XML_BF16) || N % 256 || tn < 1 || tn > 3 || M <= 0)
    return xmli_add_layernorm(pre, XML_F32, nullptr, ln_g, ln_b, y, M, N, N, xmli_act_dt(dt), st);
  const int lpr = tn == 1 ? 8 : tn == 2 ? 16 : 32;
  const dim3 grid((unsigned)cdiv(M * lpr, (int64_t)64)), blk(64);
#define XML_LNT(OT, TN)                                                                                                 \
  hipLaunchKernelGGL((ln_lne_order_kernel<OT, TN>), grid, blk, 0, st, pre, ln_g, ln_b, (OT*)y, M, N, 1e-5f)
  if (dt == XML_F32) {
    if (tn == 1) XML_LNT(float, 1); else if (tn == 2) XML_LNT(float, 2); else XML_LNT(float, 3);
  } else {
    if (tn == 1) XML_LNT(bf16_t, 1); else if (tn == 2) XML_LNT(bf16_t, 2); else XML_LNT(bf16_t, 3);
  }
#undef XML_LNT
  XML_CHECK_LAUNCH();
  return XML_OK;
}

int xmli_gemm256p(const void* A, const void* W, const float* bias, const void* addend, void* out, int64_t M, int N,
                  int K, int relu, int add_mode, int seq_len, int out_f32, int dt, hipStream_t st) {
  if (dt == XML_F32)
    return launch_gemm256p<float, float, float>(A, W, bias, addend, out, M, N, K, relu, add_mode, seq_len, st);
  if (out_f32)
    return launch_gemm256p<bf16_t, float, bf16_t>(A, W, bias, addend, out, M, N, K, relu, add_mode, seq_len, st);
  return launch_gemm256p<bf16_t, bf16_t, bf16_t>(A, W, bias, addend, out, M, N, K, relu, add_mode, seq_len, st);
}
```

### tvretrieval_amd/csrc/internal.h

```cpp
#pragma once
#include "common.h"

int xmli_gemm(const void* A, const void* W, const float* bias, const void* addend, void* out, int64_t M, int N,
              int K, int relu, int add_mode, int seq_len, int out_f32, int dt, hipStream_t st, void* split_ws = nullptr);
size_t xmli_gemm_split_ws_bytes(int64_t M, int K, int dt);
static inline int xmli_act_dt(int dt) { return dt == XML_F16S ? XML_F32 : dt; }
static inline bool xmli_model_dt_ok(int dt) { return dt == XML_F32 || dt == XML_BF16 || dt == XML_F16S; }
size_t xmli_gemm_ln_workspace_bytes(int64_t M, int N);
int xmli_gemm_ln(const void* A, const void* W, const float* bias, const void* addend, const float* ln_g, const float* ln_b,
                 void* y, int64_t M, int N, int K, int relu, int add_mode, int seq_len, int dt, void* ln_ws,
                 hipStream_t st);
int xmli_gemm_ln_tail(const float* pre, const float* ln_g, const float* ln_b, void* y, int64_t M, int N, int dt,
                      hipStream_t st);
int xmli_add_layernorm(const void* a, int a_dt, const void* b, const float* g, const float* beta, void* y,
                       int64_t rows, int d, int ld_out, int dt, hipStream_t st);
int xmli_attention_core(const void* q, int ldq, const void* k, int ldk, const void* v, int ldv,
                        const float* q_mask, const float* k_mask, void* out, int out_f32, int64_t n, int lq, int lk,
                        int hidden, int n_heads, int dt, hipStream_t st);
int xmli_modular_pool_bwd_vec(const void* enc, const float* mask, const float* w_m, const void* dout, void* denc, float* dw_m,
                              int64_t n, int lq, int hidden, int n_mod, int dt, hipStream_t st);
```

### tvretrieval_amd/csrc/linear.hip

```cpp
#include "gemm.h"
#include "internal.h"
#include "l2norm.h"

template <typename T, typename OutT, typename AddT, int BMN = 128>
__global__ __launch_bounds__(256) void gemm_bias_act_kernel(const T* __restrict__ A, const T* __restrict__ W,
                                                            const float* __restrict__ bias,
                                                            const AddT* __restrict__ addend, OutT* __restrict__ out,
                                                            int64_t M, int N, int K, int relu, int add_mode,
                                                            int seq_len, const float* __restrict__ row_scale) {
  using Cfg = GemmCfg<T, BMN, BMN, 2, 2>;
  __shared__ __attribute__((aligned(16))) char smem[Cfg::LDS_BYTES];
  const int64_t m0 = (int64_t)blockIdx.y * Cfg::BM;
  const int n0 = blockIdx.x * Cfg::BN;
  f32x4 acc[Cfg::MT][Cfg::NT];
  auto a_row = [&](int r) -> const char* {
    const int64_t m = m0 + r;
    return m < M ? reinterpret_cast<const char*>(A + m * K) : nullptr;
  };
  auto b_row = [&](int r) -> const char* {
    const int n = n0 + r;
    return n < N ? reinterpret_cast<const char*>(W + (int64_t)n * K) : nullptr;
  };
  if constexpr (dispatch::gemm_small_deep(BMN, IsSplit16<T>::value || std::is_same<T, f16_t>::value)) {
    dispatch::gemm_small_kloop_run(
        K * (int)sizeof(T), [&] { gemm_mainloop_deep<T, Cfg, 3>(acc, a_row, b_row, K * (int)sizeof(T), smem); },
        [&] { gemm_mainloop_deep<T, Cfg, 2>(acc, a_row, b_row, K * (int)sizeof(T), smem); },
        [&] { gemm_mainloop<T, Cfg>(acc, a_row, b_row, K * (int)sizeof(T), smem); });
  } else {
    gemm_mainloop<T, Cfg>(acc, a_row, b_row, K * (int)sizeof(T), smem);
  }

  const int lane = threadIdx.x & 63, wave = threadIdx.x >> 6;
  const int wm = wave / Cfg::WN, wn = wave % Cfg::WN;
#pragma unroll
  for (int mt = 0; mt < Cfg::MT; ++mt) {
#pragma unroll
    for (int nt = 0; nt < Cfg::NT; ++nt) {
      const int n = n0 + wn * (Cfg::BN / Cfg::WN) + nt * 16 + (lane & 15);
      if (n >= N) continue;
      const float b = bias ? bias[n] : 0.f;
#pragma unroll
      for (int r = 0; r < 4; ++r) {
        const int64_t m = m0 + wm * (Cfg::BM / Cfg::WM) + mt * 16 + (lane >> 4) * 4 + r;
        if (m >= M) continue;
        float v = acc[mt][nt][r];
        if constexpr (std::is_same<T, f16_t>::value) v *= row_scale[m];
        v += b;
        if (relu) v = fmaxf(v, 0.f);
        if (add_mode == 1) v += DT<AddT>::ld(addend + (int64_t)(m % seq_len) * N + n);
        else if (add_mode == 2) v += DT<AddT>::ld(addend + m * N + n);
        DT<OutT>::st(out + m * N + n, v);
      }
    }
  }
}

template <typename T, typename OutT, typename AddT>
static int launch_gemm(const void* A, const void* W, const float* bias, const void* addend, void* out, int64_t M,
                       int N, int K, int relu, int add_mode, int seq_len, hipStream_t st,
                       const float* row_scale = nullptr) {
  const int bmn = dispatch::gemm_small_tile(M, N);
  dim3 grid(cdiv(N, bmn), cdiv(M, bmn));
  if (bmn == 128)
    hipLaunchKernelGGL((gemm_bias_act_kernel<T, OutT, AddT, 128>), grid, dim3(256), 0, st, (const T*)A, (const T*)W, bias,
                       (const AddT*)addend, (OutT*)out, M, N, K, relu, add_mode, seq_len, row_scale);
  else if (bmn == 64)
    hipLaunchKernelGGL((gemm_bias_act_kernel<T, OutT, AddT, 64>), grid, dim3(256), 0, st, (const T*)A, (const T*)W, bias,
                       (const AddT*)addend, (OutT*)out, M, N, K, relu, add_mode, seq_len, row_scale);
  else
    hipLaunchKernelGGL((gemm_bias_act_kernel<T, OutT, AddT, 32>), grid, dim3(256), 0, st, (const T*)A, (const T*)W, bias,
                       (const AddT*)addend, (OutT*)out, M, N, K, relu, add_mode, seq_len, row_scale);
  XML_CHECK_LAUNCH();
  return XML_OK;
}

int xmli_gemm256(const void* A, const void* W, const float* bias, const void* addend, void* out, int64_t M, int N,
                 int K, int relu, int add_mode, int seq_len, int out_f32, int dt, hipStream_t st);
int xmli_gemm256p(const void* A, const void* W, const float* bias, const void* addend, void* out, int64_t M, int N,
                  int K, int relu, int add_mode, int seq_len, int out_f32, int dt, hipStream_t st);
#ifdef XML_DEBUG_VARIANTS
int g_gemm_variant = 0;
extern "C" void xml_debug_set_gemm_variant(int v) { g_gemm_variant = v; }
#endif

int xmli_gemm256_f16s(const void* A, const void* W, const float* bias, const void* addend, void* out,
                      const float* row_scale, int64_t M, int N, int K3, int relu, int add_mode, int seq_len,
                      hipStream_t st);
int xmli_split_f16_kcat(const float* x, void* a_cat, float* inv_scale, const float* w_trailer, int64_t rows, int k,
                        hipStream_t st);

size_t xmli_gemm_split_ws_bytes(int64_t M, int K, int dt) {
  if (dt != XML_F16S) return 0;
  return align_up((size_t)M * K * 6, 256) + align_up((size_t)M * 4, 256);
}

int xmli_gemm(const void* A, const void* W, const float* bias, const void* addend, void* out, int64_t M, int N,
              int K, int relu, int add_mode, int seq_len, int out_f32, int dt, hipStream_t st, void* split_ws) {
  XML_ENTER();
  if (M <= 0 || N <= 0 || K <= 0) return XML_ERR_BAD_ARG;
  if (dt == XML_F16S) {
    if (!split_ws) return XML_ERR_WORKSPACE;
    if (K % 8 || N % 8) return XML_ERR_UNSUPPORTED;
    char* a_cat = (char*)split_ws;
    float* rs = reinterpret_cast<float*>(a_cat + align_up((size_t)M * K * 6, 256));
    const float* trailer = reinterpret_cast<const float*>((const char*)W + align_up((size_t)N * K * 6, 16));
    const int rc = xmli_split_f16_kcat((const float*)A, a_cat, rs, trailer, M, K, st);
    if (rc) return rc;
    if (dispatch::gemm_kernel(M, N, K, dt) == XML_GEMM_256)
      return xmli_gemm256_f16s(a_cat, W, bias, addend, out, rs, M, N, 3 * K, relu, add_mode, seq_len, st);
    return launch_gemm<f16_t, float, float>(a_cat, W, bias, addend, out, M, N, 3 * K, relu, add_mode, seq_len, st, rs);
  }
  if (dt != XML_F32 && dt != XML_BF16) return XML_ERR_BAD_ARG;
  int kernel = dispatch::gemm_kernel(M, N, K, dt);
  if (g_gemm_variant != 0) {
    const bool few = dispatch::gemm_few(M, N) && g_gemm_variant != 3;
    kernel = !few && g_gemm_variant != 1 && dispatch::gemm256_ok(M, N, K, dt) ? XML_GEMM_256 : XML_GEMM_SMALL;
  }
  if (kernel == XML_GEMM_256P)
    return xmli_gemm256p(A, W, bias, addend, out, M, N, K, relu, add_mode, seq_len, out_f32, dt, st);
  if (kernel == XML_GEMM_256)
    return xmli_gemm256(A, W, bias, addend, out, M, N, K, relu, add_mode, seq_len, out_f32, dt, st);
  if (dt == XML_F32) {
    if (K % 4) return XML_ERR_UNSUPPORTED;
    return launch_gemm<float, float, float>(A, W, bias, addend, out, M, N, K, relu, add_mode, seq_len, st);
  } else if (dt == XML_BF16) {
    if (K % 8) return XML_ERR_UNSUPPORTED;
    if (out_f32) return launch_gemm<bf16_t, float, bf16_t>(A, W, bias, addend, out, M, N, K, relu, add_mode, seq_len, st);
    return launch_gemm<bf16_t, bf16_t, bf16_t>(A, W, bias, addend, out, M, N, K, relu, add_mode, seq_len, st);
  }
  return XML_ERR_BAD_ARG;
}

template <typename InT, typename BT, typename OutT>
__global__ __launch_bounds__(256) void add_layernorm_kernel(const InT* __restrict__ a, const BT* __restrict__ b,
                                                            const float* __restrict__ g,
                                                            const float* __restrict__ beta, OutT* __restrict__ y,
                                                            int64_t rows, int d, int ld_out, float eps) {
  const int lane = threadIdx.x & 63;
  const int64_t row = (int64_t)blockIdx.x * 4 + (threadIdx.x >> 6);
  if (row >= rows) return;
  const InT* pa = a + row * d;
  const BT* pb = b ? b + row * d : nullptr;
  OutT* py = y + row * ld_out;
  if (d <= 64 * 16) {
    float x[16];
    float s = 0.f;
#pragma unroll
    for (int k = 0; k < 16; ++k) {
      const int i = lane + k * 64;
      x[k] = (i < d) ? DT<InT>::ld(pa + i) + (pb ? DT<BT>::ld(pb + i) : 0.f) : 0.f;
      s += x[k];
    }
    const float mean = wave_sum(s) / (float)d;
    float v = 0.f;
#pragma unroll
    for (int k = 0; k < 16; ++k) {
      const float c = (lane + k * 64 < d) ? x[k] - mean : 0.f;
      v += c * c;
    }
    const float rstd = 1.0f / sqrtf(wave_sum(v) / (float)d + eps);
#pragma unroll
    for (int k = 0; k < 16; ++k) {
      const int i = lane + k * 64;
      if (i < d) DT<OutT>::st(py + i, (x[k] - mean) * rstd * g[i] + beta[i]);
    }
  } else {
    float s = 0.f;
    for (int i = lane; i < d; i += 64) s += DT<InT>::ld(pa + i) + (pb ? DT<BT>::ld(pb + i) : 0.f);
    const float mean = wave_sum(s) / (float)d;
    float v = 0.f;
    for (int i = lane; i < d; i += 64) {
      const float x = DT<InT>::ld(pa + i) + (pb ? DT<BT>::ld(pb + i) : 0.f) - mean;
      v += x * x;
    }
    const float rstd = 1.0f / sqrtf(wave_sum(v) / (float)d + eps);
    for (int i = lane; i < d; i += 64) {
      const float x = DT<InT>::ld(pa + i) + (pb ? DT<BT>::ld(pb + i) : 0.f);
      DT<OutT>::st(py + i, (x - mean) * rstd * g[i] + beta[i]);
    }
  }
  for (int i = d + lane; i < ld_out; i += 64) DT<OutT>::st(py + i, 0.f);
}

template <typename InT, typename BT, typename OutT, int VPL, bool DROP = false>
__global__ __launch_bounds__(256) void add_layernorm_vec_kernel(const InT* __restrict__ a, const BT* __restrict__ b,
                                                                const float* __restrict__ g,
                                                                const float* __restrict__ beta, OutT* __restrict__ y,
                                                                int64_t rows, int d, int ld_out, float eps,
                                                                const int32_t* __restrict__ src_row,
                                                                XmlDropSite din = XmlDropSite{0u, 1.f, 0ull},
                                                                XmlDropSite dout = XmlDropSite{0u, 1.f, 0ull},
                                                                const uint64_t* __restrict__ seed_dev = nullptr) {
  const int lane = threadIdx.x & 63;
  const int64_t row = (int64_t)blockIdx.x * 4 + (threadIdx.x >> 6);
  if (row >= rows) return;
  const int nvec = d >> 3;
  const InT* pa = a + (src_row ? (int64_t)src_row[row] : row) * d;
  const BT* pb = b ? b + row * d : nullptr;
  OutT* py = y + row * ld_out;
  uint32_t si0 = 0, si1 = 0, so0 = 0, so1 = 0;
  if constexpr (DROP) {
    xml_seed_words(din.seed, seed_dev, si0, si1);
    xml_seed_words(dout.seed, seed_dev, so0, so1);
  }
  float x[VPL * 8];
  float s = 0.f;
#pragma unroll
  for (int k = 0; k < VPL; ++k) {
    const int v = lane + k * 64;
    if (v < nvec) {
      ld8<InT>(pa + v * 8, x + k * 8);
      if constexpr (DROP) {
        if (din.thresh) {
          const uint64_t i0 = (uint64_t)row * (uint64_t)d + (uint64_t)v * 8u;
          drop_mask8(i0, si0, si1, din.thresh, din.scale, x + k * 8);
        }
      }
      if (pb) {
        float t[8];
        ld8<BT>(pb + v * 8, t);
#pragma unroll
        for (int j = 0; j < 8; ++j) x[k * 8 + j] += t[j];
      }
    } else {
#pragma unroll
      for (int j = 0; j < 8; ++j) x[k * 8 + j] = 0.f;
    }
#pragma unroll
    for (int j = 0; j < 8; ++j) s += x[k * 8 + j];
  }
  const float mean = wave_sum(s) / (float)d;
  float var = 0.f;
#pragma unroll
  for (int k = 0; k < VPL; ++k)
    if (lane + k * 64 < nvec)
#pragma unroll
      for (int j = 0; j < 8; ++j) { const float c = x[k * 8 + j] - mean; var += c * c; }
  const float rstd = 1.0f / sqrtf(wave_sum(var) / (float)d + eps);
#pragma unroll
  for (int k = 0; k < VPL; ++k) {
    const int v = lane + k * 64;
    if (v < nvec) {
      float gv[8], bv[8], o[8];
      ld8<float>(g + v * 8, gv);
      ld8<float>(beta + v * 8, bv);
#pragma unroll
      for (int j = 0; j < 8; ++j) o[j] = (x[k * 8 + j] - mean) * rstd * gv[j] + bv[j];
      if constexpr (DROP) {
        if (dout.thresh) {
          const uint64_t i0 = (uint64_t)row * (uint64_t)ld_out + (uint64_t)v * 8u;
          drop_mask8(i0, so0, so1, dout.thresh, dout.scale, o);
        }
      }
      st8<OutT>(py + v * 8, o);
    }
  }
  for (int i = d + lane; i < ld_out; i += 64) DT<OutT>::st(py + i, 0.f);
}

template <typename InT, typename BT, typename OutT>
static int launch_ln_drop(const void* a, const void* b, const float* g, const float* beta, void* y, int64_t rows, int d,
                          XmlDropSite din, XmlDropSite dout, const uint64_t* seed_dev, hipStream_t st) {
  const dim3 grid(cdiv(rows, 4)), blk(256);
#define XML_LN_DROP(VPL)                                                                                                    \
  hipLaunchKernelGGL((add_layernorm_vec_kernel<InT, BT, OutT, VPL, true>), grid, blk, 0, st, (const InT*)a, (const BT*)b, g, \
                     beta, (OutT*)y, rows, d, d, 1e-5f, (const int32_t*)nullptr, din, dout, seed_dev)
  if (d <= 1024) XML_LN_DROP(2);
  else if (d <= 3072) XML_LN_DROP(6);
  else XML_LN_DROP(8);
#undef XML_LN_DROP
  XML_CHECK_LAUNCH();
  return XML_OK;
}

extern "C" int xml_add_layernorm_drop(const void* a, int a_dt, const void* b, const float* g, const float* beta, void* y,
                                      int64_t rows, int d, int dt, float p_in, uint64_t seed_in, float p_out,
                                      uint64_t seed_out, const uint64_t* seed_dev, xml_stream_t stream) {
  XML_ENTER();
  if (!a || !g || !beta || !y || rows <= 0 || d <= 0) return XML_ERR_BAD_ARG;
  if (!(p_in >= 0.f) || p_in >= 1.f || !(p_out >= 0.f) || p_out >= 1.f) return XML_ERR_BAD_ARG;
  if (d % 8 || d > 4096) return XML_ERR_UNSUPPORTED;
  const XmlDropSite din = xml_drop_site(p_in, seed_in), dout = xml_drop_site(p_out, seed_out);
  hipStream_t st = (hipStream_t)stream;
  if (dt == XML_F32) {
    if (a_dt != XML_F32) return XML_ERR_BAD_ARG;
    return launch_ln_drop<float, float, float>(a, b, g, beta, y, rows, d, din, dout, seed_dev, st);
  }
  if (dt != XML_BF16) return XML_ERR_BAD_ARG;
  if (a_dt == XML_F32) return launch_ln_drop<float, bf16_t, bf16_t>(a, b, g, beta, y, rows, d, din, dout, seed_dev, st);
  return launch_ln_drop<bf16_t, bf16_t, bf16_t>(a, b, g, beta, y, rows, d, din, dout, seed_dev, st);
}

template <typename InT, typename BT, typename OutT>
static int launch_ln(const void* a, const void* b, const float* g, const float* beta, void* y, int64_t rows, int d,
                     int ld_out, hipStream_t st, const int32_t* src_row = nullptr) {
  const dim3 grid(cdiv(rows, 4)), blk(256);
  const bool vec = (d % 8 == 0) && (ld_out % 8 == 0);
#define XML_LN_VEC(VPL)                                                                                              \
  hipLaunchKernelGGL((add_layernorm_vec_kernel<InT, BT, OutT, VPL>), grid, blk, 0, st, (const InT*)a, (const BT*)b, g, \
                     beta, (OutT*)y, rows, d, ld_out, 1e-5f, src_row)
  if (src_row && !(vec && d <= 4096)) return XML_ERR_UNSUPPORTED;
  if (vec && d <= 1024) XML_LN_VEC(2);
  else if (vec && d <= 3072) XML_LN_VEC(6);
  else if (vec && d <= 4096) XML_LN_VEC(8);
  else
    hipLaunchKernelGGL((add_layernorm_kernel<InT, BT, OutT>), grid, blk, 0, st, (const InT*)a, (const BT*)b, g, beta,
                       (OutT*)y, rows, d, ld_out, 1e-5f);
#undef XML_LN_VEC
  XML_CHECK_LAUNCH();
  return XML_OK;
}

static int add_layernorm_rows(const void* a, int a_dt, const void* b, const float* g, const float* beta, void* y,
                              int64_t rows, int d, int ld_out, int dt, hipStream_t st, const int32_t* src_row) {
  if (rows <= 0 || d <= 0) return XML_ERR_BAD_ARG;
  if (dt == XML_F32) {
    if (a_dt != XML_F32) return XML_ERR_BAD_ARG;
    return launch_ln<float, float, float>(a, b, g, beta, y, rows, d, ld_out, st, src_row);
  }
  if (a_dt == XML_F32) return launch_ln<float, bf16_t, bf16_t>(a, b, g, beta, y, rows, d, ld_out, st, src_row);
  return launch_ln<bf16_t, bf16_t, bf16_t>(a, b, g, beta, y, rows, d, ld_out, st, src_row);
}

int xmli_add_layernorm(const void* a, int a_dt, const void* b, const float* g, const float* beta, void* y,
                       int64_t rows, int d, int ld_out, int dt, hipStream_t st) {
  XML_ENTER();
  return add_layernorm_rows(a, a_dt, b, g, beta, y, rows, d, ld_out, dt, st, nullptr);
}

extern "C" int xml_add_layernorm(const void* a, int a_dt, const void* b, const float* g, const float* beta,
                                 void* y, int64_t rows, int d, int dt, xml_stream_t stream) {
  XML_ENTER();
  if (!a || !g || !beta || !y) return XML_ERR_BAD_ARG;
  return xmli_add_layernorm(a, a_dt, b, g, beta, y, rows, d, d, dt, (hipStream_t)stream);
}

template <typename T>
__global__ __launch_bounds__(256) void l2norm_rows_kernel(const T* __restrict__ x, T* __restrict__ y, int64_t rows,
                                                          int d) {
  const int lane = threadIdx.x & 63;
  const int64_t row = (int64_t)blockIdx.x * 4 + (threadIdx.x >> 6);
  if (row >= rows) return;
  const T* px = x + row * d;
  float s = 0.f;
  for (int i = lane; i < d; i += 64) {
    const float v = DT<T>::ld(px + i);
    s += v * v;
  }
  const float nrm = fmaxf(sqrtf(wave_sum(s)), 1e-12f);
  for (int i = lane; i < d; i += 64) DT<T>::st(y + row * d + i, DT<T>::ld(px + i) / nrm);
}

__global__ __launch_bounds__(256) void l2norm_add_eps_kernel(const float* __restrict__ x, float* __restrict__ y,
                                                             int64_t rows, int d, float eps) {
  const int lane = threadIdx.x & 63;
  const int64_t row = (int64_t)blockIdx.x * 4 + (threadIdx.x >> 6);
  if (row >= rows) return;
  const float* px = x + row * d;
  float s = 0.f;
  for (int i = lane; i < d; i += 64) s += px[i] * px[i];
  const float den = sqrtf(wave_sum(s)) + eps;
  for (int i = lane; i < d; i += 64) y[row * d + i] = px[i] / den;
}

extern "C" int xml_l2norm_rows_eps(const float* x, float* y, int64_t rows, int d, float eps, xml_stream_t stream) {
  XML_ENTER();
  if (!x || !y || rows <= 0 || d <= 0) return XML_ERR_BAD_ARG;
  hipLaunchKernelGGL(l2norm_add_eps_kernel, dim3(cdiv(rows, 4)), dim3(256), 0, (hipStream_t)stream, x, y, rows, d, eps);
  XML_CHECK_LAUNCH();
  return XML_OK;
}

template <typename T>
__global__ __launch_bounds__(256) void l2norm_rows_vec_kernel(const T* __restrict__ x, T* __restrict__ y, int64_t rows,
                                                              int d) {
  constexpr int VEC = 16 / (int)sizeof(T);
  const int l32 = threadIdx.x & 31;
  const int64_t row = (int64_t)blockIdx.x * 8 + (threadIdx.x >> 5);
  const bool live = row < rows;
  uint4 v[L2N_MAXJ];
  const float nrm = l2n_load_row<T>(live ? x + row * d : nullptr, d, l32, v);
  if (!live) return;
  const int chunks = d / VEC;
#pragma unroll
  for (int j = 0; j < L2N_MAXJ; ++j) {
    const int c = l32 + 32 * j;
    if (c < chunks) st_global16(y + row * d + c * VEC, l2n_scale_chunk<T>(v[j], nrm));
  }
}

extern "C" int xml_l2norm_rows(const void* x, void* y, int64_t rows, int d, int dt, xml_stream_t stream) {
  XML_ENTER();
  if (!x || !y || rows <= 0 || d <= 0) return XML_ERR_BAD_ARG;
  hipStream_t st = (hipStream_t)stream;
  const bool vec = dispatch::l2n_vec_ok(d, dt);
  if (vec && dt == XML_F32)
    hipLaunchKernelGGL(l2norm_rows_vec_kernel<float>, dim3(cdiv(rows, 8)), dim3(256), 0, st, (const float*)x, (float*)y, rows, d);
  else if (vec)
    hipLaunchKernelGGL(l2norm_rows_vec_kernel<bf16_t>, dim3(cdiv(rows, 8)), dim3(256), 0, st, (const bf16_t*)x, (bf16_t*)y, rows, d);
  else if (dt == XML_F32)
    hipLaunchKernelGGL(l2norm_rows_kernel<float>, dim3(cdiv(rows, 4)), dim3(256), 0, st, (const float*)x, (float*)y, rows, d);
  else if (dt == XML_BF16)
    hipLaunchKernelGGL(l2norm_rows_kernel<bf16_t>, dim3(cdiv(rows, 4)), dim3(256), 0, st, (const bf16_t*)x, (bf16_t*)y, rows, d);
  else
    return XML_ERR_BAD_ARG;
  XML_CHECK_LAUNCH();
  return XML_OK;
}

template <typename S, typename D>
__global__ void convert_kernel(const S* __restrict__ s, D* __restrict__ d, int64_t n) {
  for (int64_t i = (int64_t)blockIdx.x * blockDim.x + threadIdx.x; i < n; i += (int64_t)gridDim.x * blockDim.x)
    DT<D>::st(d + i, DT<S>::ld(s + i));
}

extern "C" int xml_convert(const void* src, int src_dt, void* dst, int dst_dt, int64_t n, xml_stream_t stream) {
  XML_ENTER();
  if (!src || !dst || n < 0) return XML_ERR_BAD_ARG;
  if (n == 0) return XML_OK;
  hipStream_t st = (hipStream_t)stream;
  const int grid = (int)((n + 255) / 256 < 4096 ? (n + 255) / 256 : 4096);
  if (src_dt == XML_F32 && dst_dt == XML_BF16)
    hipLaunchKernelGGL((convert_kernel<float, bf16_t>), dim3(grid), dim3(256), 0, st, (const float*)src, (bf16_t*)dst, n);
  else if (src_dt == XML_BF16 && dst_dt == XML_F32)
    hipLaunchKernelGGL((convert_kernel<bf16_t, float>), dim3(grid), dim3(256), 0, st, (const bf16_t*)src, (float*)dst, n);
  else if (src_dt == XML_F32 && dst_dt == XML_F32)
    hipLaunchKernelGGL((convert_kernel<float, float>), dim3(grid), dim3(256), 0, st, (const float*)src, (float*)dst, n);
  else if (src_dt == XML_BF16 && dst_dt == XML_BF16)
    hipLaunchKernelGGL((convert_kernel<bf16_t, bf16_t>), dim3(grid), dim3(256), 0, st, (const bf16_t*)src, (bf16_t*)dst, n);
  else
    return XML_ERR_BAD_ARG;
  XML_CHECK_LAUNCH();
  return XML_OK;
}

extern "C" int xml_pack_weights(const float* src, void* dst, int dt, int64_t n, xml_stream_t stream) {
  XML_ENTER();
  return xml_convert(src, XML_F32, dst, dt, n, stream);
}

extern "C" int xml_linear(const void* x, const void* w, const float* b, void* y, int64_t rows, int n, int k, int relu,
                          int dt, xml_stream_t stream) {
  XML_ENTER();
  if (!x || !w || !y) return XML_ERR_BAD_ARG;
  return xmli_gemm(x, w, b, nullptr, y, rows, n, k, relu, 0, 1, 0, dt, (hipStream_t)stream);
}

extern "C" int xml_linear_add(const void* x, const void* w, const float* b, const void* addend, void* y, int64_t rows, int n,
                              int k, int relu, int dt, xml_stream_t stream) {
  XML_ENTER();
  if (!x || !w || !y || !addend) return XML_ERR_BAD_ARG;
  if (dt != XML_F32 && dt != XML_BF16) return XML_ERR_UNSUPPORTED;
  return xmli_gemm(x, w, b, addend, y, rows, n, k, relu, 2, 1, 0, dt, (hipStream_t)stream);
}

extern "C" size_t xml_linear_f16s_workspace_bytes(int64_t rows, int k) { return xmli_gemm_split_ws_bytes(rows, k, XML_F16S); }
extern "C" int xml_linear_f16s(const float* x, const void* w, const float* b, float* y, int64_t rows, int n, int k, int relu,
                               void* ws, size_t ws_bytes, xml_stream_t stream) {
  XML_ENTER();
  if (!x || !w || !y || !ws) return XML_ERR_BAD_ARG;
  if (rows > 0 && ws_bytes < xmli_gemm_split_ws_bytes(rows, k, XML_F16S)) return XML_ERR_WORKSPACE;
  return xmli_gemm(x, w, b, nullptr, y, rows, n, k, relu, 0, 1, 1, XML_F16S, (hipStream_t)stream, ws);
}

static inline int k_pad8(int d_in) { return (d_in + 7) & ~7; }
extern "C" size_t xml_linear_ln_relu_pos_workspace_bytes(int64_t rows, int d_in, int hidden, int dt) {
  const size_t pre = align_up((size_t)rows * hidden * 4, 256);
  const size_t lnw = dispatch::gemm_ln_fused(rows, hidden, k_pad8(d_in), dt) ? xmli_gemm_ln_workspace_bytes(rows, hidden) : 0;
  return align_up((size_t)rows * k_pad8(d_in) * dt_size(dt), 256) + (pre > lnw ? pre : lnw) +
         xmli_gemm_split_ws_bytes(rows, k_pad8(d_in), dt);
}

extern "C" int xml_linear_ln_relu_pos(const void* x, int x_dt, const float* ln_in_g, const float* ln_in_b,
                                      const void* w, const float* b, const void* pos, const float* ln_pos_g,
                                      const float* ln_pos_b, void* y, int64_t rows, int seq_len, int d_in, int hidden,
                                      int dt, void* ws, size_t ws_bytes, xml_stream_t stream) {
  XML_ENTER();
  if (!x || !ln_in_g || !ln_in_b || !w || !b || !pos || !ln_pos_g || !ln_pos_b || !y || !ws) return XML_ERR_BAD_ARG;
  if (rows <= 0 || seq_len <= 0 || !xmli_model_dt_ok(dt)) return XML_ERR_BAD_ARG;
  if (d_in <= 0 || hidden % 8) return XML_ERR_UNSUPPORTED;
  if (ws_bytes < xml_linear_ln_relu_pos_workspace_bytes(rows, d_in, hidden, dt)) return XML_ERR_WORKSPACE;
  hipStream_t st = (hipStream_t)stream;
  const int d_pad = k_pad8(d_in);
  const int adt = xmli_act_dt(dt);
  char* xn = (char*)ws;
  char* pre = xn + align_up((size_t)rows * d_pad * dt_size(dt), 256);
  char* sws = dt == XML_F16S ? (char*)ws + xml_linear_ln_relu_pos_workspace_bytes(rows, d_in, hidden, dt) -
                                   xmli_gemm_split_ws_bytes(rows, d_pad, dt) : nullptr;
  int rc = xmli_add_layernorm(x, x_dt, nullptr, ln_in_g, ln_in_b, xn, rows, d_in, d_pad, adt, st);
  if (rc) return rc;
  if (dispatch::gemm_ln_fused(rows, hidden, d_pad, dt) &&
      xmli_gemm_ln(xn, w, b, pos, ln_pos_g, ln_pos_b, y, rows, hidden, d_pad,  1,  1, seq_len, dt, pre,
                   st) == XML_OK)
    return XML_OK;
  rc = xmli_gemm(xn, w, b, pos, pre, rows, hidden, d_pad,  1,  1, seq_len,  1, dt, st, sws);
  if (rc) return rc;
  return xmli_gemm_ln_tail((const float*)pre, ln_pos_g, ln_pos_b, y, rows, hidden, dt, st);
}

__global__ __launch_bounds__(256) void pack_len_kernel(const float* __restrict__ mask, int n, int lq, int32_t* __restrict__ cu,
                                                       int32_t* __restrict__ status) {
  const int lane = threadIdx.x & 63;
  const int r = blockIdx.x * 4 + (threadIdx.x >> 6);
  if (r >= n) return;
  const float v = lane < lq ? mask[(int64_t)r * lq + lane] : 0.f;
  const unsigned long long ones = __ballot(v == 1.f), other = __ballot(v != 1.f && v != 0.f);
  const int len = (int)__popcll(ones);
  const bool ok = other == 0 && len > 0 && ones == (len == 64 ? ~0ull : ((1ull << len) - 1ull));
  if (lane == 0) {
    cu[r + 1] = len;
    if (!ok) atomicOr(&status[1], 1);
  }
}

__global__ __launch_bounds__(1024) void pack_scan_kernel(int n, int32_t* __restrict__ cu, int32_t* __restrict__ status) {
  __shared__ int s_wave[16];
  const int tid = threadIdx.x, lane = tid & 63, wave = tid >> 6;
  const int per = (n + 1023) / 1024;
  const int r0 = min(n, tid * per), r1 = min(n, r0 + per);
  int sum = 0;
  for (int r = r0; r < r1; ++r) sum += cu[r + 1];
  int inc = sum;
#pragma unroll
  for (int o = 1; o < 64; o <<= 1) {
    const int v = __shfl_up(inc, o, 64);
    if (lane >= o) inc += v;
  }
  if (lane == 63) s_wave[wave] = inc;
  __syncthreads();
  int base = inc - sum;
  for (int w = 0; w < wave; ++w) base += s_wave[w];
  for (int r = r0; r < r1; ++r) {
    base += cu[r + 1];
    cu[r + 1] = base;
  }
  if (tid == 0) {
    cu[0] = 0;
    int total = 0;
    for (int w = 0; w < 16; ++w) total += s_wave[w];
    status[0] = status[1] ? -1 : total;
  }
}

__global__ __launch_bounds__(256) void pack_fill_kernel(int n, int lq, const int32_t* __restrict__ cu, int32_t* __restrict__ src_row) {
  const int lane = threadIdx.x & 63;
  const int r = blockIdx.x * 4 + (threadIdx.x >> 6);
  if (r >= n) return;
  const int b = cu[r], len = cu[r + 1] - b;
  if (lane < len) src_row[b + lane] = r * lq + lane;
}

extern "C" int xml_pack_plan(const float* mask, int64_t n, int lq, int32_t* cu_seqlens, int32_t* src_row, int32_t* status,
                             xml_stream_t stream) {
  XML_ENTER();
  if (!mask || !cu_seqlens || !src_row || !status || n <= 0 || lq <= 0) return XML_ERR_BAD_ARG;
  if (lq > 64 || n * lq > (int64_t)INT32_MAX) return XML_ERR_UNSUPPORTED;
  hipStream_t st = (hipStream_t)stream;
  xml_zero_async(status, 8, st);
  hipLaunchKernelGGL(pack_len_kernel, dim3(cdiv(n, 4)), dim3(256), 0, st, mask, (int)n, lq, cu_seqlens, status);
  hipLaunchKernelGGL(pack_scan_kernel, dim3(1), dim3(1024), 0, st, (int)n, cu_seqlens, status);
  hipLaunchKernelGGL(pack_fill_kernel, dim3(cdiv(n, 4)), dim3(256), 0, st, (int)n, lq, cu_seqlens, src_row);
  XML_CHECK_LAUNCH();
  return XML_OK;
}

__global__ __launch_bounds__(256) void gather_pos_rows_kernel(const uint4* __restrict__ table, const int32_t* __restrict__ src_row,
                                                              uint4* __restrict__ dst, int64_t rows, int lq, int vec_per_row) {
  const int64_t i = (int64_t)blockIdx.x * 256 + threadIdx.x;
  if (i >= rows * vec_per_row) return;
  const int64_t r = i / vec_per_row;
  const int v = (int)(i - r * vec_per_row);
  dst[i] = table[(int64_t)(src_row[r] % lq) * vec_per_row + v];
}

extern "C" size_t xml_linear_ln_relu_pos_packed_workspace_bytes(int64_t rows, int d_in, int hidden, int dt) {
  return xml_linear_ln_relu_pos_workspace_bytes(rows, d_in, hidden, dt) + align_up((size_t)rows * hidden * dt_size(dt), 256);
}

extern "C" int xml_linear_ln_relu_pos_packed(const void* x, int x_dt, const int32_t* src_row, int lq, const float* ln_in_g,
                                             const float* ln_in_b, const void* w, const float* b, const void* pos,
                                             const float* ln_pos_g, const float* ln_pos_b, void* y, int64_t rows, int d_in,
                                             int hidden, int dt, void* ws, size_t ws_bytes, xml_stream_t stream) {
  XML_ENTER();
  if (!x || !src_row || !ln_in_g || !ln_in_b || !w || !b || !pos || !ln_pos_g || !ln_pos_b || !y || !ws) return XML_ERR_BAD_ARG;
  if (rows <= 0 || rows > (int64_t)INT32_MAX || lq <= 0 || !xmli_model_dt_ok(dt)) return XML_ERR_BAD_ARG;
  if (d_in <= 0 || d_in % 8 || d_in > 4096 || hidden % 8) return XML_ERR_UNSUPPORTED;
  if (ws_bytes < xml_linear_ln_relu_pos_packed_workspace_bytes(rows, d_in, hidden, dt)) return XML_ERR_WORKSPACE;
  hipStream_t st = (hipStream_t)stream;
  const int adt = xmli_act_dt(dt);
  char* pg = (char*)ws;
  char* xn = pg + align_up((size_t)rows * hidden * dt_size(dt), 256);
  char* pre = xn + align_up((size_t)rows * d_in * dt_size(dt), 256);
  char* sws = dt == XML_F16S ? (char*)ws + xml_linear_ln_relu_pos_packed_workspace_bytes(rows, d_in, hidden, dt) -
                                   xmli_gemm_split_ws_bytes(rows, d_in, dt) : nullptr;
  const int vpr = hidden * (int)dt_size(dt) / 16;
  hipLaunchKernelGGL(gather_pos_rows_kernel, dim3(cdiv(rows * vpr, 256)), dim3(256), 0, st, (const uint4*)pos, src_row,
                     (uint4*)pg, rows, lq, vpr);
  XML_CHECK_LAUNCH();
  int rc = add_layernorm_rows(x, x_dt, nullptr, ln_in_g, ln_in_b, xn, rows, d_in, d_in, adt, st, src_row);
  if (rc) return rc;
  if (dispatch::gemm_ln_fused(rows, hidden, d_in, dt) &&
      xmli_gemm_ln(xn, w, b, pg, ln_pos_g, ln_pos_b, y, rows, hidden, d_in,  1,  1, (int)rows, dt, pre,
                   st) == XML_OK)
    return XML_OK;
  rc = xmli_gemm(xn, w, b, pg, pre, rows, hidden, d_in,  1,  1, (int)rows,  1, dt, st, sws);
  if (rc) return rc;
  return xmli_gemm_ln_tail((const float*)pre, ln_pos_g, ln_pos_b, y, rows, hidden, dt, st);
}
```

Before: 145,000.

## Fuse positional-row gather into GEMM epilogue and parallelize convse scan across workgroups

The packed linear+LN path no longer materializes a gathered positional-embedding buffer. It passes src_row as an add_map into every GEMM variant, so each epilogue indexes the pos table directly, which saves one kernel launch and a rows×hidden write and read. Separately, the single-workgroup convse scan now runs on up to 32 workgroups, each recomputing the prefix of the earlier ranges, to cut serial latency for large video counts. In exchange, the GEMM epilogues take extra per-row indirection, and the scan does redundant reads of counts.

After: 145,300, median of 6. Within noise of the previous version (+0.2%).

```diff
diff --git a/tvretrieval_amd/csrc/convse.hip b/tvretrieval_amd/csrc/convse.hip
--- a/tvretrieval_amd/csrc/convse.hip
+++ b/tvretrieval_amd/csrc/convse.hip
@@ -64,18 +64,32 @@
   for (int i = 0; i < lpad4; ++i) { s4[i] = z; e4[i] = z; }
 }
 
+using dispatch::convse_scan_wgs;
 __global__ __launch_bounds__(1024) void convse_scan_kernel(const int32_t* __restrict__ counts,
                                                            int32_t* __restrict__ offsets,
                                                            int32_t* __restrict__ chunk_off,
                                                            int32_t* __restrict__ chunk_vid, int nv, int TM, int sub) {
-  __shared__ int32_t wa[16], wb[16];
+  __shared__ int32_t wa[16], wb[16], pa[16], pb[16];
   const int tid = threadIdx.x, lane = tid & 63, wave = tid >> 6;
-  const int per = (nv + 1023) / 1024;
-  const int r0 = min(nv, tid * per), r1 = min(nv, r0 + per);
+  const int per = (nv + (int)gridDim.x * 1024 - 1) / ((int)gridDim.x * 1024);
+  const int start = min(nv, (int)blockIdx.x * per * 1024), end = min(nv, start + per * 1024);
+  auto video_count = [&](int i) {
+    int c = 0;
+    for (int j = 0; j < sub; ++j) c += counts[(int64_t)i * sub + j];
+    return c;
+  };
+  int fa = 0, fb = 0;
+  for (int i = tid; i < start; i += 1024) {
+    const int c = video_count(i);
+    fa += c; fb += (c + TM - 1) / TM;
+  }
+#pragma unroll
+  for (int o = 32; o > 0; o >>= 1) { fa += __shfl_xor(fa, o, 64); fb += __shfl_xor(fb, o, 64); }
+  if (lane == 0) { pa[wave] = fa; pb[wave] = fb; }
+  const int r0 = min(end, start + tid * per), r1 = min(end, r0 + per);
   int sa = 0, sb = 0;
   for (int i = r0; i < r1; ++i) {
-    int c = 0;
-    for (int j = 0; j < sub; ++j) c += counts[(int64_t)i * sub + j];
+    const int c = video_count(i);
     sa += c; sb += (c + TM - 1) / TM;
   }
   int ia = sa, ib = sb;
@@ -87,6 +101,7 @@
   if (lane == 63) { wa[wave] = ia; wb[wave] = ib; }
   __syncthreads();
   int a = ia - sa, b = ib - sb;
+  for (int w = 0; w < 16; ++w) { a += pa[w]; b += pb[w]; }
   for (int w = 0; w < wave; ++w) { a += wa[w]; b += wb[w]; }
   for (int i = r0; i < r1; ++i) {
     int c = 0;
@@ -100,7 +115,7 @@
     for (int j = 0; j < ch; ++j) chunk_vid[b + j] = i;
     a += c; b += ch;
   }
-  if (tid == 1023) { offsets[(int64_t)nv * sub] = a; chunk_off[nv] = b; }
+  if (blockIdx.x == gridDim.x - 1 && tid == 1023) { offsets[(int64_t)nv * sub] = a; chunk_off[nv] = b; }
 }
 
 __global__ void convse_fill_kernel(const int32_t* __restrict__ pair_vid, const int32_t* __restrict__ offsets,
@@ -719,8 +734,8 @@
                          d->nv, d->lpad / 4);
       XML_CHECK_LAUNCH();
     }
-    hipLaunchKernelGGL(convse_scan_kernel, dim3(1), dim3(1024), 0, st, w.counts, w.offsets, w.chunk_off, w.chunk_vid,
-                       d->nv, TM, sub);
+    hipLaunchKernelGGL(convse_scan_kernel, dim3(convse_scan_wgs(d->nv)), dim3(1024), 0, st, w.counts, w.offsets, w.chunk_off,
+                       w.chunk_vid, d->nv, TM, sub);
     XML_CHECK_LAUNCH();
     hipLaunchKernelGGL(convse_fill_kernel, dim3(cdiv(P, 256)), dim3(256), 0, st, pair_vid, w.offsets, w.pos, w.bucket, P, sub);
     XML_CHECK_LAUNCH();
@@ -887,8 +902,8 @@
   XML_CHECK_LAUNCH();
   const int tm = dispatch::rescore_chunk_pairs(P, nv, dt);
   const bool big = tm == dispatch::RESCORE_TM_BIG;
-  hipLaunchKernelGGL(convse_scan_kernel, dim3(1), dim3(1024), 0, st, w.counts, w.offsets, w.chunk_off, w.chunk_vid, nv,
-                     tm, sub);
+  hipLaunchKernelGGL(convse_scan_kernel, dim3(convse_scan_wgs(nv)), dim3(1024), 0, st, w.counts, w.offsets, w.chunk_off,
+                     w.chunk_vid, nv, tm, sub);
   XML_CHECK_LAUNCH();
   hipLaunchKernelGGL(convse_fill_kernel, dim3(cdiv(P, 256)), dim3(256), 0, st, pair_vid, w.offsets, w.pos, w.bucket, P, sub);
   XML_CHECK_LAUNCH();
diff --git a/tvretrieval_amd/csrc/dispatch.h b/tvretrieval_amd/csrc/dispatch.h
--- a/tvretrieval_amd/csrc/dispatch.h
+++ b/tvretrieval_amd/csrc/dispatch.h
@@ -125,6 +125,8 @@
   return convse_dma(nq, lpad, hidden, dt) ? XML_CONVSE_DMA : dt == XML_F16S ? XML_CONVSE_REFUSED : XML_CONVSE_STAGED;
 }
 constexpr int convse_sub(int64_t P, int nv) { return P >= CONVSE_SUB_MIN_PAIRS_PER_VIDEO * (int64_t)nv ? CONVSE_SUB_MAX : 1; }
+constexpr int CONVSE_SCAN_MAX_WG = 32;
+constexpr int convse_scan_wgs(int nv) { return nv > 1024 * CONVSE_SCAN_MAX_WG ? CONVSE_SCAN_MAX_WG : cdiv(nv, 1024); }
 constexpr bool convse_small_inversion(int64_t P, int nv) { return P <= CONVSE_SMALL_P && nv <= CONVSE_SMALL_NV; }
 constexpr xml_convse_inversion convse_inversion(int64_t P, int nv, bool rescore) {
   if (!rescore && convse_small_inversion(P, nv)) return XML_CONVSE_INV_SMALL;
diff --git a/tvretrieval_amd/csrc/gemm256.hip b/tvretrieval_amd/csrc/gemm256.hip
--- a/tvretrieval_amd/csrc/gemm256.hip
+++ b/tvretrieval_amd/csrc/gemm256.hip
@@ -19,7 +19,8 @@
                                                          const float* __restrict__ bias,
                                                          const AddT* __restrict__ addend, OutT* __restrict__ out,
                                                          int64_t M, int N, int K, int relu, int add_mode, int seq_len,
-                                                         int tm, int tn, const float* __restrict__ row_scale) {
+                                                         int tm, int tn, const float* __restrict__ row_scale,
+                                                         const int32_t* __restrict__ add_map) {
   constexpr bool SCALED = std::is_same<T, f16_t>::value;
   using namespace ring256;
   constexpr int NSLOT = dispatch::RING_SLOTS;
@@ -187,6 +188,14 @@
     for (int pq = 0; pq < NGRP / 2; ++pq) pcol[pq] = n0 + wn * 128 + pq * (8 * GC) + (fr & 1) * (4 * GC) + fg * GC;
     const uint32_t m0_mod = add_mode == 1 ? (uint32_t)(m0 % seq_len) : 0u;
     const bool odd = (fr & 1) != 0;
+    int amap[4] = {0, 0, 0, 0};
+    if (add_mode == 1 && add_map) {
+#pragma unroll
+      for (int m4 = 0; m4 < 4; ++m4) {
+        const int64_t mr = m0 + wm * 64 + m4 * 16 + fr;
+        if (mr < M) amap[m4] = add_map[mr] % seq_len;
+      }
+    }
 #pragma unroll
     for (int m4 = 0; m4 < 4; ++m4) {
       const int lrow = wm * 64 + m4 * 16 + fr;
@@ -206,7 +215,9 @@
           v[q][e] = x;
         }
       if (add_mode) {
-        const int64_t arow = add_mode == 1 ? (int64_t)((m0_mod + (uint32_t)lrow) % (uint32_t)seq_len) : m;
+        const int64_t arow = add_mode != 1 ? m
+                             : add_map     ? (int64_t)amap[m4]
+                                           : (int64_t)((m0_mod + (uint32_t)lrow) % (uint32_t)seq_len);
         constexpr int AB = GC * (int)sizeof(AddT);
 #pragma unroll
         for (int qb = 0; qb < NGRP; qb += 4) {
@@ -295,7 +306,9 @@
         v[j] += bv[j];
         if (relu) v[j] = fmaxf(v[j], 0.f);
       }
-      const int64_t arow = add_mode == 1 ? (int64_t)((m0_mod + (uint32_t)lrow) % (uint32_t)seq_len) : m;
+      const int64_t arow = add_mode != 1 ? m
+                           : add_map     ? (int64_t)(add_map[m] % seq_len)
+                                         : (int64_t)((m0_mod + (uint32_t)lrow) % (uint32_t)seq_len);
       if (!RAGGED_N) {
         if (add_mode) {
           float av[8] = {0.f, 0.f, 0.f, 0.f, 0.f, 0.f, 0.f, 0.f};
@@ -337,8 +350,8 @@
 
 template <typename T, typename OutT, typename AddT>
 static int launch_gemm256(const void* A, const void* W, const float* bias, const void* addend, void* out, int64_t M,
-                          int N, int K, int relu, int add_mode, int seq_len, hipStream_t st,
-                          const float* row_scale = nullptr) {
+                          int N, int K, int relu, int add_mode, int seq_len, const int32_t* add_map,
+                          hipStream_t st, const float* row_scale = nullptr) {
   const int tm = cdiv(M, 256), tn = cdiv(N, 256);
   const int64_t nsup = (int64_t)((tm + 7) / 8) * ((tn + 3) / 4);
   const unsigned grid = (unsigned)(((nsup + 7) / 8) * 8 * 32);
@@ -348,22 +361,22 @@
                 : xml_lds_attr_once<gemm256_kernel<T, OutT, AddT, false>>(lds)))
     return XML_ERR_LAUNCH;
   hipLaunchKernelGGL(kern, dim3(grid), dim3(512), lds, st, (const T*)A, (const T*)W, bias, (const AddT*)addend,
-                     (OutT*)out, M, N, K, relu, add_mode, seq_len, tm, tn, row_scale);
+                     (OutT*)out, M, N, K, relu, add_mode, seq_len, tm, tn, row_scale, add_map);
   XML_CHECK_LAUNCH();
   return XML_OK;
 }
 
 int xmli_gemm256_f16s(const void* A, const void* W, const float* bias, const void* addend, void* out,
                       const float* row_scale, int64_t M, int N, int K3, int relu, int add_mode, int seq_len,
-                      hipStream_t st) {
-  return launch_gemm256<f16_t, float, float>(A, W, bias, addend, out, M, N, K3, relu, add_mode, seq_len, st, row_scale);
+                      hipStream_t st, const int32_t* add_map) {
+  return launch_gemm256<f16_t, float, float>(A, W, bias, addend, out, M, N, K3, relu, add_mode, seq_len, add_map, st, row_scale);
 }
 
 int xmli_gemm256(const void* A, const void* W, const float* bias, const void* addend, void* out, int64_t M, int N,
-                 int K, int relu, int add_mode, int seq_len, int out_f32, int dt, hipStream_t st) {
+                 int K, int relu, int add_mode, int seq_len, int out_f32, int dt, hipStream_t st, const int32_t* add_map) {
   if (dt == XML_F32)
-    return launch_gemm256<float, float, float>(A, W, bias, addend, out, M, N, K, relu, add_mode, seq_len, st);
+    return launch_gemm256<float, float, float>(A, W, bias, addend, out, M, N, K, relu, add_mode, seq_len, add_map, st);
   if (out_f32)
-    return launch_gemm256<bf16_t, float, bf16_t>(A, W, bias, addend, out, M, N, K, relu, add_mode, seq_len, st);
-  return launch_gemm256<bf16_t, bf16_t, bf16_t>(A, W, bias, addend, out, M, N, K, relu, add_mode, seq_len, st);
-}
+    return launch_gemm256<bf16_t, float, bf16_t>(A, W, bias, addend, out, M, N, K, relu, add_mode, seq_len, add_map, st);
+  return launch_gemm256<bf16_t, bf16_t, bf16_t>(A, W, bias, addend, out, M, N, K, relu, add_mode, seq_len, add_map, st);
+}
diff --git a/tvretrieval_amd/csrc/gemm256p.hip b/tvretrieval_amd/csrc/gemm256p.hip
--- a/tvretrieval_amd/csrc/gemm256p.hip
+++ b/tvretrieval_amd/csrc/gemm256p.hip
@@ -1,3 +1,4 @@
+#include <cstddef>
 #include <type_traits>
 
 #include "internal.h"
@@ -8,6 +9,7 @@
   const void* W;
   const float* bias;
   const void* addend;
+  const int32_t* add_map;
   void* out;
   int64_t M, n_tiles;
   int N, K, relu, add_mode, seq_len, tn;
@@ -293,6 +295,18 @@
           float4 b4 = make_float4(0.f, 0.f, 0.f, 0.f);
           const int bc = n0 + wn * 128 + (lane_e & 31) * 4;
           if (a.bias && bc + 4 <= N) b4 = *reinterpret_cast<const float4*>(a.bias + bc);
+          if (a.add_mode == 1) {
+            typedef const __attribute__((address_space(4))) char* karg_p;
+            karg_p ka = (karg_p)__builtin_amdgcn_kernarg_segment_ptr();
+            asm volatile("" : "+s"(ka));
+            const int seq_len = *(const __attribute__((address_space(4))) int*)(ka + offsetof(G256pArgs, seq_len));
+            const int32_t* add_map = *(const int32_t* const __attribute__((address_space(4)))*)(ka + offsetof(G256pArgs, add_map));
+            const int lr = wm * 64 + lane_e;
+            int ar;
+            if (add_map) ar = m0 + lr < M ? add_map[m0 + lr] % seq_len : 0;
+            else ar = (int)(((uint32_t)(m0 % seq_len) + (uint32_t)lr) % (uint32_t)seq_len);
+            reinterpret_cast<int*>(patch)[128 + lane_e] = ar;
+          }
           if (lane_e < 32) *reinterpret_cast<float4*>(patch + 256 + lane_e * 4) = b4;
           __builtin_amdgcn_s_waitcnt(0xc07f);
           __builtin_amdgcn_wave_barrier();
@@ -322,7 +336,7 @@
             }
           }
           if (a.add_mode) {
-            const int64_t arow = a.add_mode == 1 ? (int64_t)((m0_mod + (uint32_t)lrow) % (uint32_t)a.seq_len) : m;
+            const int64_t arow = a.add_mode == 1 ? (int64_t)reinterpret_cast<const int*>(patch)[128 + m4 * 16 + fr_e] : m;
             constexpr int AB = GC * (int)sizeof(AddT);
 #pragma unroll
             for (int qb = 0; qb < NGRP; qb += 4) {
@@ -428,7 +442,9 @@
             if (a.relu) v[j] = fmaxf(v[j], 0.f);
           }
           if (a.add_mode) {
-            const int64_t arow = a.add_mode == 1 ? (int64_t)((m0_mod + (uint32_t)lrow) % (uint32_t)a.seq_len) : m;
+            const int64_t arow = a.add_mode != 1 ? m
+                                 : a.add_map     ? (int64_t)(a.add_map[m] % a.seq_len)
+                                                 : (int64_t)((m0_mod + (uint32_t)lrow) % (uint32_t)a.seq_len);
             float av[8] = {0.f, 0.f, 0.f, 0.f, 0.f, 0.f, 0.f, 0.f};
             if (sizeof(AddT) == 2) {
               uint2 u0 = make_uint2(0u, 0u), u1 = u0;
@@ -564,10 +580,10 @@
 
 template <typename T, typename OutT, typename AddT, bool LNE = false, bool DIRECT = true>
 static int launch_gemm256p(const void* A, const void* W, const float* bias, const void* addend, void* out, int64_t M,
-                           int N, int K, int relu, int add_mode, int seq_len, hipStream_t st, const float* ln_g = nullptr,
-                           const float* ln_b = nullptr, void* ln_ws = nullptr) {
+                           int N, int K, int relu, int add_mode, int seq_len, const int32_t* add_map, hipStream_t st,
+                           const float* ln_g = nullptr, const float* ln_b = nullptr, void* ln_ws = nullptr) {
   G256pArgs a;
-  a.A = A; a.W = W; a.bias = bias; a.addend = addend; a.out = out;
+  a.A = A; a.W = W; a.bias = bias; a.addend = addend; a.add_map = add_mode == 1 ? add_map : nullptr; a.out = out;
   a.M = M; a.N = N; a.K = K; a.relu = relu; a.add_mode = add_mode; a.seq_len = seq_len;
   a.tn = cdiv(N, 256);
   a.n_tiles = (int64_t)cdiv(M, 256) * a.tn;
@@ -576,7 +592,7 @@
   const int lds = dispatch::RING_SLOTS * ring256::SLOT_BYTES + 8 * 4096;
 #ifdef XML_DEBUG_VARIANTS
   if (!LNE && DIRECT && g_gemm_variant == 3)
-    return launch_gemm256p<T, OutT, AddT, false, false>(A, W, bias, addend, out, M, N, K, relu, add_mode, seq_len, st);
+    return launch_gemm256p<T, OutT, AddT, false, false>(A, W, bias, addend, out, M, N, K, relu, add_mode, seq_len, add_map, st);
 #endif
   auto kern = gemm256p_kernel<T, OutT, AddT, LNE, DIRECT>;
   if (!xml_lds_attr_once<gemm256p_kernel<T, OutT, AddT, LNE, DIRECT>>(lds)) return XML_ERR_LAUNCH;
@@ -591,12 +607,12 @@
 }
 int xmli_gemm_ln(const void* A, const void* W, const float* bias, const void* addend, const float* ln_g, const float* ln_b,
                  void* y, int64_t M, int N, int K, int relu, int add_mode, int seq_len, int dt, void* ln_ws,
-                 hipStream_t st) {
+                 hipStream_t st, const int32_t* add_map) {
   if (!ln_ws) return XML_ERR_WORKSPACE;
   if (dt == XML_F32)
-    return launch_gemm256p<float, float, float, true>(A, W, bias, addend, y, M, N, K, relu, add_mode, seq_len, st, ln_g,
+    return launch_gemm256p<float, float, float, true>(A, W, bias, addend, y, M, N, K, relu, add_mode, seq_len, add_map, st, ln_g,
                                                       ln_b, ln_ws);
-  return launch_gemm256p<bf16_t, bf16_t, bf16_t, true>(A, W, bias, addend, y, M, N, K, relu, add_mode, seq_len, st, ln_g,
+  return launch_gemm256p<bf16_t, bf16_t, bf16_t, true>(A, W, bias, addend, y, M, N, K, relu, add_mode, seq_len, add_map, st, ln_g,
                                                         ln_b, ln_ws);
 }
 
@@ -699,10 +715,10 @@
 }
 
 int xmli_gemm256p(const void* A, const void* W, const float* bias, const void* addend, void* out, int64_t M, int N,
-                  int K, int relu, int add_mode, int seq_len, int out_f32, int dt, hipStream_t st) {
+                  int K, int relu, int add_mode, int seq_len, int out_f32, int dt, hipStream_t st, const int32_t* add_map) {
   if (dt == XML_F32)
-    return launch_gemm256p<float, float, float>(A, W, bias, addend, out, M, N, K, relu, add_mode, seq_len, st);
+    return launch_gemm256p<float, float, float>(A, W, bias, addend, out, M, N, K, relu, add_mode, seq_len, add_map, st);
   if (out_f32)
-    return launch_gemm256p<bf16_t, float, bf16_t>(A, W, bias, addend, out, M, N, K, relu, add_mode, seq_len, st);
-  return launch_gemm256p<bf16_t, bf16_t, bf16_t>(A, W, bias, addend, out, M, N, K, relu, add_mode, seq_len, st);
-}
+    return launch_gemm256p<bf16_t, float, bf16_t>(A, W, bias, addend, out, M, N, K, relu, add_mode, seq_len, add_map, st);
+  return launch_gemm256p<bf16_t, bf16_t, bf16_t>(A, W, bias, addend, out, M, N, K, relu, add_mode, seq_len, add_map, st);
+}
diff --git a/tvretrieval_amd/csrc/internal.h b/tvretrieval_amd/csrc/internal.h
--- a/tvretrieval_amd/csrc/internal.h
+++ b/tvretrieval_amd/csrc/internal.h
@@ -2,14 +2,15 @@
 #include "common.h"
 
 int xmli_gemm(const void* A, const void* W, const float* bias, const void* addend, void* out, int64_t M, int N,
-              int K, int relu, int add_mode, int seq_len, int out_f32, int dt, hipStream_t st, void* split_ws = nullptr);
+              int K, int relu, int add_mode, int seq_len, int out_f32, int dt, hipStream_t st, void* split_ws = nullptr,
+              const int32_t* add_map = nullptr);
 size_t xmli_gemm_split_ws_bytes(int64_t M, int K, int dt);
 static inline int xmli_act_dt(int dt) { return dt == XML_F16S ? XML_F32 : dt; }
 static inline bool xmli_model_dt_ok(int dt) { return dt == XML_F32 || dt == XML_BF16 || dt == XML_F16S; }
 size_t xmli_gemm_ln_workspace_bytes(int64_t M, int N);
 int xmli_gemm_ln(const void* A, const void* W, const float* bias, const void* addend, const float* ln_g, const float* ln_b,
                  void* y, int64_t M, int N, int K, int relu, int add_mode, int seq_len, int dt, void* ln_ws,
-                 hipStream_t st);
+                 hipStream_t st, const int32_t* add_map = nullptr);
 int xmli_gemm_ln_tail(const float* pre, const float* ln_g, const float* ln_b, void* y, int64_t M, int N, int dt,
                       hipStream_t st);
 int xmli_add_layernorm(const void* a, int a_dt, const void* b, const float* g, const float* beta, void* y,
diff --git a/tvretrieval_amd/csrc/linear.hip b/tvretrieval_amd/csrc/linear.hip
--- a/tvretrieval_amd/csrc/linear.hip
+++ b/tvretrieval_amd/csrc/linear.hip
@@ -7,7 +7,8 @@
                                                             const float* __restrict__ bias,
                                                             const AddT* __restrict__ addend, OutT* __restrict__ out,
                                                             int64_t M, int N, int K, int relu, int add_mode,
-                                                            int seq_len, const float* __restrict__ row_scale) {
+                                                            int seq_len, const float* __restrict__ row_scale,
+                                                            const int32_t* __restrict__ add_map) {
   using Cfg = GemmCfg<T, BMN, BMN, 2, 2>;
   __shared__ __attribute__((aligned(16))) char smem[Cfg::LDS_BYTES];
   const int64_t m0 = (int64_t)blockIdx.y * Cfg::BM;
@@ -47,7 +48,7 @@
         if constexpr (std::is_same<T, f16_t>::value) v *= row_scale[m];
         v += b;
         if (relu) v = fmaxf(v, 0.f);
-        if (add_mode == 1) v += DT<AddT>::ld(addend + (int64_t)(m % seq_len) * N + n);
+        if (add_mode == 1) v += DT<AddT>::ld(addend + (int64_t)(add_map ? add_map[m] % seq_len : m % seq_len) * N + n);
         else if (add_mode == 2) v += DT<AddT>::ld(addend + m * N + n);
         DT<OutT>::st(out + m * N + n, v);
       }
@@ -57,27 +58,27 @@
 
 template <typename T, typename OutT, typename AddT>
 static int launch_gemm(const void* A, const void* W, const float* bias, const void* addend, void* out, int64_t M,
-                       int N, int K, int relu, int add_mode, int seq_len, hipStream_t st,
-                       const float* row_scale = nullptr) {
+                       int N, int K, int relu, int add_mode, int seq_len, const int32_t* add_map,
+                       hipStream_t st, const float* row_scale = nullptr) {
   const int bmn = dispatch::gemm_small_tile(M, N);
   dim3 grid(cdiv(N, bmn), cdiv(M, bmn));
   if (bmn == 128)
     hipLaunchKernelGGL((gemm_bias_act_kernel<T, OutT, AddT, 128>), grid, dim3(256), 0, st, (const T*)A, (const T*)W, bias,
-                       (const AddT*)addend, (OutT*)out, M, N, K, relu, add_mode, seq_len, row_scale);
+                       (const AddT*)addend, (OutT*)out, M, N, K, relu, add_mode, seq_len, row_scale, add_map);
   else if (bmn == 64)
     hipLaunchKernelGGL((gemm_bias_act_kernel<T, OutT, AddT, 64>), grid, dim3(256), 0, st, (const T*)A, (const T*)W, bias,
-                       (const AddT*)addend, (OutT*)out, M, N, K, relu, add_mode, seq_len, row_scale);
+                       (const AddT*)addend, (OutT*)out, M, N, K, relu, add_mode, seq_len, row_scale, add_map);
   else
     hipLaunchKernelGGL((gemm_bias_act_kernel<T, OutT, AddT, 32>), grid, dim3(256), 0, st, (const T*)A, (const T*)W, bias,
-                       (const AddT*)addend, (OutT*)out, M, N, K, relu, add_mode, seq_len, row_scale);
+                       (const AddT*)addend, (OutT*)out, M, N, K, relu, add_mode, seq_len, row_scale, add_map);
   XML_CHECK_LAUNCH();
   return XML_OK;
 }
 
 int xmli_gemm256(const void* A, const void* W, const float* bias, const void* addend, void* out, int64_t M, int N,
-                 int K, int relu, int add_mode, int seq_len, int out_f32, int dt, hipStream_t st);
+                 int K, int relu, int add_mode, int seq_len, int out_f32, int dt, hipStream_t st, const int32_t* add_map);
 int xmli_gemm256p(const void* A, const void* W, const float* bias, const void* addend, void* out, int64_t M, int N,
-                  int K, int relu, int add_mode, int seq_len, int out_f32, int dt, hipStream_t st);
+                  int K, int relu, int add_mode, int seq_len, int out_f32, int dt, hipStream_t st, const int32_t* add_map);
 #ifdef XML_DEBUG_VARIANTS
 int g_gemm_variant = 0;
 extern "C" void xml_debug_set_gemm_variant(int v) { g_gemm_variant = v; }
@@ -85,7 +86,7 @@
 
 int xmli_gemm256_f16s(const void* A, const void* W, const float* bias, const void* addend, void* out,
                       const float* row_scale, int64_t M, int N, int K3, int relu, int add_mode, int seq_len,
-                      hipStream_t st);
+                      hipStream_t st, const int32_t* add_map);
 int xmli_split_f16_kcat(const float* x, void* a_cat, float* inv_scale, const float* w_trailer, int64_t rows, int k,
                         hipStream_t st);
 
@@ -95,7 +96,8 @@
 }
 
 int xmli_gemm(const void* A, const void* W, const float* bias, const void* addend, void* out, int64_t M, int N,
-              int K, int relu, int add_mode, int seq_len, int out_f32, int dt, hipStream_t st, void* split_ws) {
+              int K, int relu, int add_mode, int seq_len, int out_f32, int dt, hipStream_t st, void* split_ws,
+              const int32_t* add_map) {
   XML_ENTER();
   if (M <= 0 || N <= 0 || K <= 0) return XML_ERR_BAD_ARG;
   if (dt == XML_F16S) {
@@ -107,8 +109,8 @@
     const int rc = xmli_split_f16_kcat((const float*)A, a_cat, rs, trailer, M, K, st);
     if (rc) return rc;
     if (dispatch::gemm_kernel(M, N, K, dt) == XML_GEMM_256)
-      return xmli_gemm256_f16s(a_cat, W, bias, addend, out, rs, M, N, 3 * K, relu, add_mode, seq_len, st);
-    return launch_gemm<f16_t, float, float>(a_cat, W, bias, addend, out, M, N, 3 * K, relu, add_mode, seq_len, st, rs);
+      return xmli_gemm256_f16s(a_cat, W, bias, addend, out, rs, M, N, 3 * K, relu, add_mode, seq_len, st, add_map);
+    return launch_gemm<f16_t, float, float>(a_cat, W, bias, addend, out, M, N, 3 * K, relu, add_mode, seq_len, add_map, st, rs);
   }
   if (dt != XML_F32 && dt != XML_BF16) return XML_ERR_BAD_ARG;
   int kernel = dispatch::gemm_kernel(M, N, K, dt);
@@ -117,16 +119,16 @@
     kernel = !few && g_gemm_variant != 1 && dispatch::gemm256_ok(M, N, K, dt) ? XML_GEMM_256 : XML_GEMM_SMALL;
   }
   if (kernel == XML_GEMM_256P)
-    return xmli_gemm256p(A, W, bias, addend, out, M, N, K, relu, add_mode, seq_len, out_f32, dt, st);
+    return xmli_gemm256p(A, W, bias, addend, out, M, N, K, relu, add_mode, seq_len, out_f32, dt, st, add_map);
   if (kernel == XML_GEMM_256)
-    return xmli_gemm256(A, W, bias, addend, out, M, N, K, relu, add_mode, seq_len, out_f32, dt, st);
+    return xmli_gemm256(A, W, bias, addend, out, M, N, K, relu, add_mode, seq_len, out_f32, dt, st, add_map);
   if (dt == XML_F32) {
     if (K % 4) return XML_ERR_UNSUPPORTED;
-    return launch_gemm<float, float, float>(A, W, bias, addend, out, M, N, K, relu, add_mode, seq_len, st);
+    return launch_gemm<float, float, float>(A, W, bias, addend, out, M, N, K, relu, add_mode, seq_len, add_map, st);
   } else if (dt == XML_BF16) {
     if (K % 8) return XML_ERR_UNSUPPORTED;
-    if (out_f32) return launch_gemm<bf16_t, float, bf16_t>(A, W, bias, addend, out, M, N, K, relu, add_mode, seq_len, st);
-    return launch_gemm<bf16_t, bf16_t, bf16_t>(A, W, bias, addend, out, M, N, K, relu, add_mode, seq_len, st);
+    if (out_f32) return launch_gemm<bf16_t, float, bf16_t>(A, W, bias, addend, out, M, N, K, relu, add_mode, seq_len, add_map, st);
+    return launch_gemm<bf16_t, bf16_t, bf16_t>(A, W, bias, addend, out, M, N, K, relu, add_mode, seq_len, add_map, st);
   }
   return XML_ERR_BAD_ARG;
 }
@@ -564,15 +566,6 @@
   return XML_OK;
 }
 
-__global__ __launch_bounds__(256) void gather_pos_rows_kernel(const uint4* __restrict__ table, const int32_t* __restrict__ src_row,
-                                                              uint4* __restrict__ dst, int64_t rows, int lq, int vec_per_row) {
-  const int64_t i = (int64_t)blockIdx.x * 256 + threadIdx.x;
-  if (i >= rows * vec_per_row) return;
-  const int64_t r = i / vec_per_row;
-  const int v = (int)(i - r * vec_per_row);
-  dst[i] = table[(int64_t)(src_row[r] % lq) * vec_per_row + v];
-}
-
 extern "C" size_t xml_linear_ln_relu_pos_packed_workspace_bytes(int64_t rows, int d_in, int hidden, int dt) {
   return xml_linear_ln_relu_pos_workspace_bytes(rows, d_in, hidden, dt) + align_up((size_t)rows * hidden * dt_size(dt), 256);
 }
@@ -588,22 +581,17 @@
   if (ws_bytes < xml_linear_ln_relu_pos_packed_workspace_bytes(rows, d_in, hidden, dt)) return XML_ERR_WORKSPACE;
   hipStream_t st = (hipStream_t)stream;
   const int adt = xmli_act_dt(dt);
-  char* pg = (char*)ws;
-  char* xn = pg + align_up((size_t)rows * hidden * dt_size(dt), 256);
+  char* xn = (char*)ws;
   char* pre = xn + align_up((size_t)rows * d_in * dt_size(dt), 256);
-  char* sws = dt == XML_F16S ? (char*)ws + xml_linear_ln_relu_pos_packed_workspace_bytes(rows, d_in, hidden, dt) -
+  char* sws = dt == XML_F16S ? (char*)ws + xml_linear_ln_relu_pos_workspace_bytes(rows, d_in, hidden, dt) -
                                    xmli_gemm_split_ws_bytes(rows, d_in, dt) : nullptr;
-  const int vpr = hidden * (int)dt_size(dt) / 16;
-  hipLaunchKernelGGL(gather_pos_rows_kernel, dim3(cdiv(rows * vpr, 256)), dim3(256), 0, st, (const uint4*)pos, src_row,
-                     (uint4*)pg, rows, lq, vpr);
-  XML_CHECK_LAUNCH();
   int rc = add_layernorm_rows(x, x_dt, nullptr, ln_in_g, ln_in_b, xn, rows, d_in, d_in, adt, st, src_row);
   if (rc) return rc;
   if (dispatch::gemm_ln_fused(rows, hidden, d_in, dt) &&
-      xmli_gemm_ln(xn, w, b, pg, ln_pos_g, ln_pos_b, y, rows, hidden, d_in,  1,  1, (int)rows, dt, pre,
-                   st) == XML_OK)
+      xmli_gemm_ln(xn, w, b, pos, ln_pos_g, ln_pos_b, y, rows, hidden, d_in,  1,  1, lq, dt, pre, st,
+                   src_row) == XML_OK)
     return XML_OK;
-  rc = xmli_gemm(xn, w, b, pg, pre, rows, hidden, d_in,  1,  1, (int)rows,  1, dt, st, sws);
+  rc = xmli_gemm(xn, w, b, pos, pre, rows, hidden, d_in,  1,  1, lq,  1, dt, st, sws, src_row);
   if (rc) return rc;
   return xmli_gemm_ln_tail((const float*)pre, ln_pos_g, ln_pos_b, y, rows, hidden, dt, st);
 }
```
